# Robotmurlock/Deepwalk-and-Node2vec

Measured on AMD Instinct MI355X. Metric: positive-pairs/s + random-walks/s, 1M-node d=128 k=5, 1/2/4/8 MI355X, higher is better.
Workload: dtype fp32

## Files before the change

deepwalk-and-node2vec_amd/csrc/dw_abi.cpp:

```cpp
#include <stdarg.h>
#include <string.h>

#include "dw_common.h"

namespace dw {

static thread_local char g_err[512] = "";
static thread_local const dw_step_scalars *g_step = nullptr;
static thread_local bool g_step_has_host = false;
static thread_local int64_t g_step_host = 0;

const dw_step_scalars *bound_step_scalars() { return g_step; }

int bound_step_rel(int64_t step, const dw_step_scalars **dyn, int32_t *delta, const char *what) {
    *dyn = g_step;
    *delta = 0;
    if (!g_step) return DW_OK;
    if (!g_step_has_host) {
        set_error("%s: a dw_step_scalars block is bound without its host step "
                  "(dw_step_scalars_bind_at)", what);
        return DW_E_INVALID_ARG;
    }
    const int64_t d = step - g_step_host;
    if (d < -0x7FFFFFFF || d > 0x7FFFFFFF) {
        set_error("%s: step %lld is too far from the bound block's host step %lld", what,
                  (long long)step, (long long)g_step_host);
        return DW_E_INVALID_ARG;
    }
    *delta = static_cast<int32_t>(d);
    return DW_OK;
}

void set_error(const char *fmt, ...) {
    va_list ap;
    va_start(ap, fmt);
    vsnprintf(g_err, sizeof(g_err), fmt, ap);
    va_end(ap);
}

}

extern "C" {

const char *dw_last_error_string(void) { return dw::g_err; }

int dw_abi_version(void) { return 29; }

#ifndef DW_BUILD_ID
#define DW_BUILD_ID "unknown"
#endif
const char *dw_build_id(void) { return DW_BUILD_ID; }

int dw_step_scalars_bind(const dw_step_scalars *dev) {
    dw::g_step = dev;
    dw::g_step_has_host = false;
    return DW_OK;
}

int dw_step_scalars_bind_at(const dw_step_scalars *dev, int64_t host_step) {
    dw::g_step = dev;
    dw::g_step_has_host = dev != nullptr;
    dw::g_step_host = host_step;
    return DW_OK;
}

int dw_device_sync(void *stream) {
    hipError_t e = hipStreamSynchronize(dw::as_stream(stream));
    if (e != hipSuccess) {
        dw::set_error("hipStreamSynchronize: %s", hipGetErrorString(e));
        return DW_E_HIP;
    }
    return DW_OK;
}

}
```

deepwalk-and-node2vec_amd/csrc/dw_sgns.hip:

```cpp
#include <stdlib.h>

#include <cmath>
#include <mutex>
#include <unordered_map>
#include <vector>

#include <rocprim/block/block_radix_sort.hpp>
#include <rocprim/block/block_scan.hpp>
#include <rocprim/device/device_radix_sort.hpp>
#include <rocprim/device/device_scan.hpp>
#include <rocprim/device/device_select.hpp>

#include "dw_common.h"

namespace {

constexpr int WAVE = 64;
constexpr int WAVES_PER_BLOCK = 4;
constexpr int CHUNK = 12;
constexpr int TMAX = 256;
constexpr int GCH = 512;
constexpr int GU = 8;
constexpr uint32_t TAG_SGNS = 0x53470000u;

__device__ __forceinline__ float sigmoidf(float x) { return 1.0f / (1.0f + expf(-x)); }

using dw::row_coef;

__device__ void flush_loss(double *acc, float p, float n, float r, float pr) {
    __shared__ float s_loss[WAVES_PER_BLOCK][4];
    p = dw::wave_sum(p);
    n = dw::wave_sum(n);
    r = dw::wave_sum(r);
    pr = dw::wave_sum(pr);
    const int lane = threadIdx.x & (WAVE - 1), wv = threadIdx.x / WAVE;
    if (lane == 0) {
        s_loss[wv][0] = p;
        s_loss[wv][1] = n;
        s_loss[wv][2] = r;
        s_loss[wv][3] = pr;
    }
    __syncthreads();
    if (threadIdx.x < 4) {
        double t = 0.0;
        for (int w = 0; w < WAVES_PER_BLOCK; ++w) t += s_loss[w][threadIdx.x];
        if (t != 0.0) atomicAdd(acc + threadIdx.x, t);
    }
}

__device__ __forceinline__ float pooled(const int64_t *__restrict__ inputs, int64_t b, int32_t P,
                                        const float *__restrict__ w_in, int32_t d, int e) {
    if (P == 1) return w_in[inputs[b] * d + e];
    float h = 0.f;
    for (int p = 0; p < P; ++p) h += w_in[inputs[b * P + p] * d + e];
    return h / static_cast<float>(P);
}

__device__ __forceinline__ bool inputs_ok(const int64_t *__restrict__ inputs, int64_t b,
                                          int32_t P, int64_t V) {
    bool ok = true;
    for (int p = 0; p < P; ++p) {
        const int64_t c = inputs[b * P + p];
        ok = ok && c >= 0 && c < V;
    }
    return ok;
}

struct SgnsArgs {
    const int32_t *walks;
    int32_t L, R;
    const int64_t *inputs;
    int32_t n_in;
    const int64_t *targets;
    int64_t batch;
    int32_t C;
    int32_t K;
    int64_t V;
    int32_t d;
    const float *w_in, *w_out;
    float *g_in, *g_out;
    const int64_t *noise;
    uint32_t k0, k1;
    uint64_t noise_offset;
    float scale;
    double *loss_acc;
    int32_t *status;
    uint32_t *rec_key;
    uint64_t *rec_val;
    int32_t owner, n_owners;
    int32_t own_shift;
    uint32_t *rec_counts;
    uint32_t *count_out;
    int64_t region;
    const uint32_t *place_rank = nullptr, *place_off = nullptr;
    const uint32_t *occ;
    int64_t occ_per_wave;
    const dw_step_scalars *dyn;
    dw::Fixed fx_in{};
};

#ifndef DW_NOISE_ROUNDS
#define DW_NOISE_ROUNDS 10
#endif
__device__ __forceinline__ dw::U4 noise_pair(const SgnsArgs &a, int64_t b, int m) {
    const uint64_t g = (a.dyn ? a.dyn->noise_offset : a.noise_offset) + static_cast<uint64_t>(b);
    return dw::philox<DW_NOISE_ROUNDS>(
        dw::U4{static_cast<uint32_t>(g), static_cast<uint32_t>(g >> 32), static_cast<uint32_t>(m),
               TAG_SGNS},
        a.k0, a.k1);
}

__device__ __forceinline__ int64_t noise_id(const SgnsArgs &a, int64_t b, int j, int k) {
    if (a.noise) return a.noise[(b * a.C + j) * a.K + k];
    const int n = j * a.K + k;
    const dw::U4 r = noise_pair(a, b, n >> 1);
    const uint64_t V = static_cast<uint64_t>(a.V);
    return static_cast<int64_t>((n & 1) ? dw::bounded64(r.z, r.w, V) : dw::bounded64(r.x, r.y, V));
}

__device__ __forceinline__ uint64_t pack_record(float coef, int64_t centre) {
    return (static_cast<uint64_t>(__float_as_uint(coef)) << 32) |
           static_cast<uint32_t>(centre);
}

template <bool FROM_WALKS>
__device__ __forceinline__ int64_t row_id(const SgnsArgs &a, int64_t b, const int32_t *walk,
                                          int64_t i, int t) {
    const int rows_per_ctx = 1 + a.K;
    const int j = t / rows_per_ctx, k = t - j * rows_per_ctx - 1;
    if (k < 0) {
        if (FROM_WALKS) return walk[(j < a.R) ? (i - a.R + j) : (i + 1 + (j - a.R))];
        return a.targets[b * a.C + j];
    }
    return noise_id(a, b, j, k);
}

template <int VPL, bool MASKED, bool FROM_WALKS, bool RECORDS, int CH, bool EXACT = false>
__global__ void __launch_bounds__(WAVES_PER_BLOCK *WAVE) k_sgns(SgnsArgs a) {
    static_assert(!EXACT || RECORDS, "the exact form writes records");
    bool range = false;
    const int lane = threadIdx.x & (WAVE - 1);
    const int wv = threadIdx.x / WAVE;
    const int64_t n_waves = (int64_t)gridDim.x * WAVES_PER_BLOCK;
    const int rows_per_ctx = 1 + a.K;
    const int n_rows = a.C * rows_per_ctx;

    bool live[VPL];
#pragma unroll
    for (int m = 0; m < VPL; ++m) live[m] = !MASKED || (lane + WAVE * m < a.d);

    float acc_pos = 0.f, acc_neg = 0.f, acc_rec = 0.f, acc_prec = 0.f;

    for (int64_t b = (int64_t)blockIdx.x * WAVES_PER_BLOCK + wv; b < a.batch; b += n_waves) {
        const int32_t *walk = nullptr;
        int64_t i = 0, cid;
        if (FROM_WALKS) {
            const int64_t per = a.L - 2 * a.R;
            const int64_t w = b / per;
            i = a.R + (b - w * per);
            walk = a.walks + w * a.L;
            cid = walk[i];
        } else {
            cid = a.inputs[b * a.n_in];
        }
        const bool pool = !FROM_WALKS && a.n_in > 1;
        const bool centre_ok =
            pool ? inputs_ok(a.inputs, b, a.n_in, a.V) : (cid >= 0 && cid < a.V);
        if (!centre_ok) {
            if (lane == 0) dw::status_or(a.status, DW_S_BAD_INDEX);
            if (RECORDS) {
                for (int t = lane; t < n_rows; t += WAVE) {
                    a.rec_key[b * n_rows + t] = 0u;
                    a.rec_val[b * n_rows + t] = 0ull;
                }
            }
            continue;
        }
        float c[VPL], gc[VPL];
        int64_t gx[VPL];
        const float *crow = a.w_in + cid * a.d + lane;
#pragma unroll
        for (int m = 0; m < VPL; ++m) {
            c[m] = !live[m] ? 0.f
                   : pool   ? pooled(a.inputs, b, a.n_in, a.w_in, a.d, lane + WAVE * m)
                            : crow[WAVE * m];
            gc[m] = 0.f;
            gx[m] = 0;
        }
        for (int g0 = 0; g0 < n_rows; g0 += WAVE) {
            const int g_rows = (n_rows - g0 < WAVE) ? n_rows - g0 : WAVE;
            const int t = g0 + lane;
            int32_t my_id = 0;
            bool my_ok = false;
            const bool my_pos = (t % rows_per_ctx) == 0;
            if (lane < g_rows) {
                const int64_t id = row_id<FROM_WALKS>(a, b, walk, i, t);
                my_ok = id >= 0 && id < a.V;
                if (!my_ok) dw::status_or(a.status, DW_S_BAD_INDEX);
                my_id = my_ok ? static_cast<int32_t>(id) : 0;
            }
            float my_coef = 0.f;
            for (int r0 = 0; r0 < g_rows; r0 += CH) {
                int32_t id[CH];
                float o[CH][VPL], dot[CH];
#pragma unroll
                for (int u = 0; u < CH; ++u) {
                    const int src = (r0 + u < g_rows) ? r0 + u : 0;
                    id[u] = __builtin_amdgcn_readlane(my_id, src);
                }
#pragma unroll
                for (int u = 0; u < CH; ++u) {
                    const bool in = r0 + u < g_rows;
                    const float *row = a.w_out + static_cast<int64_t>(id[u]) * a.d + lane;
#pragma unroll
                    for (int m = 0; m < VPL; ++m) o[u][m] = (in && live[m]) ? row[WAVE * m] : 0.f;
                }
#pragma unroll
                for (int u = 0; u < CH; ++u) {
                    float s = 0.f;
#pragma unroll
                    for (int m = 0; m < VPL; ++m) s += c[m] * o[u][m];
                    dot[u] = s;
                }
#pragma unroll
                for (int off = 32; off >= 1; off >>= 1) {
#pragma unroll
                    for (int u = 0; u < CH; ++u) dot[u] += __shfl_xor(dot[u], off, WAVE);
                }
                float x = 0.f;
#pragma unroll
                for (int u = 0; u < CH; ++u)
                    if (lane == r0 + u) x = dot[u];
                const bool mine = lane >= r0 && lane < r0 + CH && lane < g_rows && my_ok;
                float coef = 0.f;
                if (mine) {
                    coef = row_coef(x, my_pos, a.scale, acc_pos, acc_neg, acc_rec, acc_prec);
                    my_coef = coef;
                }
#pragma unroll
                for (int u = 0; u < CH; ++u) {
                    if (r0 + u >= g_rows) continue;
                    const float gs =
                        __int_as_float(__builtin_amdgcn_readlane(__float_as_int(coef), r0 + u));
#pragma unroll
                    for (int m = 0; m < VPL; ++m) {
                        if constexpr (EXACT)
                            gx[m] += dw::to_fixed(gs * o[u][m], a.fx_in.fs, range);
                        else
                            gc[m] += gs * o[u][m];
                    }
                    if (!RECORDS && gs != 0.f) {
                        float *grow = a.g_out + static_cast<int64_t>(id[u]) * a.d + lane;
#pragma unroll
                        for (int m = 0; m < VPL; ++m)
                            if (live[m]) atomicAdd(grow + WAVE * m, gs * c[m]);
                    }
                }
            }
            if (RECORDS && lane < g_rows) {
                a.rec_key[b * n_rows + t] = static_cast<uint32_t>(my_id);
                a.rec_val[b * n_rows + t] = pack_record(my_ok ? my_coef : 0.f, cid);
            }
        }
        if (pool) {
            for (int p = 0; p < a.n_in; ++p) {
                float *grow = a.g_in + a.inputs[b * a.n_in + p] * a.d + lane;
#pragma unroll
                for (int m = 0; m < VPL; ++m)
                    if (live[m]) atomicAdd(grow + WAVE * m, gc[m] / static_cast<float>(a.n_in));
            }
        } else if constexpr (EXACT) {
            int64_t *gxrow = a.fx_in.acc + cid * a.d + lane;
#pragma unroll
            for (int m = 0; m < VPL; ++m)
                if (live[m]) dw::fixed_add(gxrow + WAVE * m, gx[m]);
        } else {
            float *gcrow = a.g_in + cid * a.d + lane;
#pragma unroll
            for (int m = 0; m < VPL; ++m)
                if (live[m]) atomicAdd(gcrow + WAVE * m, gc[m]);
        }
    }
    if constexpr (EXACT)
        if (__ballot(range) && lane == 0) dw::status_or(a.status, DW_S_FIXED_RANGE);

    if (a.loss_acc) flush_loss(a.loss_acc, acc_pos, acc_neg, acc_rec, acc_prec);
}

constexpr int G16_TMAX = 64;
#ifndef G16_MIN_WAVES
#define G16_MIN_WAVES 4
#endif

template <int N>
__device__ __forceinline__ float row_ror(float x) {
    return __int_as_float(
        __builtin_amdgcn_update_dpp(0, __float_as_int(x), 0x120 + N, 0xF, 0xF, false));
}

__device__ __forceinline__ float row_sum16(float x) {
    x += row_ror<8>(x);
    x += row_ror<4>(x);
    x += row_ror<2>(x);
    x += row_ror<1>(x);
    return x;
}

template <int F4, bool FROM_WALKS, int CHR, bool OWNER, bool EXACT = false, bool COEFIN = false>
__global__ void __launch_bounds__(WAVES_PER_BLOCK *WAVE, CHR >= 8 ? 3 : G16_MIN_WAVES)
    k_sgns_g16(SgnsArgs a) {
    static_assert(!COEFIN || OWNER, "the coefficients-in form is the owner path's");
    constexpr int D = 64 * F4;
    __shared__ int32_t s_id[WAVES_PER_BLOCK][4][G16_TMAX];
    __shared__ float s_coef[WAVES_PER_BLOCK][4][G16_TMAX];
    __shared__ uint8_t s_t[WAVES_PER_BLOCK][4][OWNER ? G16_TMAX : 1];
    __shared__ float4 s_g[WAVES_PER_BLOCK][4][EXACT ? 1 : 16 * F4];
    __shared__ int64_t s_gx[WAVES_PER_BLOCK][EXACT ? D : 1];
    bool range = false;
    uint32_t tmax = 0u;
    const int lane = threadIdx.x & (WAVE - 1);
    const int wv = threadIdx.x / WAVE;
    const int q = lane >> 4, gl = lane & 15;
    const int rows_per_ctx = 1 + a.K;
    const int T = a.C * rows_per_ctx;
    const int64_t n_slots = (int64_t)gridDim.x * WAVES_PER_BLOCK * 4;
    float acc_pos = 0.f, acc_neg = 0.f, acc_rec = 0.f, acc_prec = 0.f;
    int64_t filled = 0;
    const int64_t gw = (int64_t)blockIdx.x * WAVES_PER_BLOCK + wv;
    int64_t o_end = a.batch, step = n_slots, base0 = gw * 4;
    if constexpr (OWNER) {
        base0 = gw * a.occ_per_wave;
        o_end = base0 + a.occ_per_wave < a.batch ? base0 + a.occ_per_wave : a.batch;
        step = 4;
    }
    int32_t pend_c = -1;
    float pend[F4];
#pragma unroll
    for (int f = 0; f < F4; ++f) pend[f] = 0.f;

    for (int64_t base = base0; base < o_end; base += step) {
        const int64_t jb = base + q;
        const int64_t b0 =
            OWNER ? (jb < o_end ? (a.occ ? static_cast<int64_t>(a.occ[jb]) : jb) : 0) : jb;
        const bool bad_b = OWNER && jb < o_end && (b0 < 0 || b0 >= a.batch);
        if (bad_b && gl == 0) dw::status_or(a.status, DW_S_BAD_INDEX);
        const bool active = jb < o_end && !bad_b;
        const int64_t b = bad_b ? 0 : b0;
        const int32_t *walk = nullptr;
        int64_t i = 0, cid = -1;
        if (active) {
            if (FROM_WALKS) {
                const int64_t per = a.L - 2 * a.R;
                const int64_t w = b / per;
                i = a.R + (b - w * per);
                walk = a.walks + w * a.L;
                cid = walk[i];
            } else {
                cid = a.inputs[b];
            }
        }
        const bool ok_c = active && cid >= 0 && cid < a.V;
        if (active && !ok_c && gl == 0) dw::status_or(a.status, DW_S_BAD_INDEX);
        int n_own = T;
        if constexpr (OWNER) {
            int32_t *stage = reinterpret_cast<int32_t *>(&s_coef[wv][q][0]);
            for (int t = gl; t < T; t += 16) stage[t] = -1;
            if (ok_c) {
                const int n_neg = a.C * a.K;
                auto put = [&](int n, int64_t r) {
                    const int jn = n / a.K;
                    const int t = jn * rows_per_ctx + 1 + (n - jn * a.K);
                    if (r >= 0 && r < a.V)
                        stage[t] = static_cast<int32_t>(r);
                    else
                        dw::status_or(a.status, DW_S_BAD_INDEX);
                };
                for (int j = gl; j < a.C; j += 16) {
                    const int64_t r = row_id<FROM_WALKS>(a, b, walk, i, j * rows_per_ctx);
                    if (r >= 0 && r < a.V)
                        stage[j * rows_per_ctx] = static_cast<int32_t>(r);
                    else
                        dw::status_or(a.status, DW_S_BAD_INDEX);
                }
                if (a.noise) {
                    for (int n = gl; n < n_neg; n += 16) put(n, a.noise[b * n_neg + n]);
                } else {
                    const uint64_t Vu = static_cast<uint64_t>(a.V);
#pragma unroll 2
                    for (int m = gl; 2 * m < n_neg; m += 16) {
                        const dw::U4 r = noise_pair(a, b, m);
                        put(2 * m, static_cast<int64_t>(dw::bounded64(r.x, r.y, Vu)));
                        if (2 * m + 1 < n_neg)
                            put(2 * m + 1, static_cast<int64_t>(dw::bounded64(r.z, r.w, Vu)));
                    }
                }
            }
            dw::wave_lds_sync();
            n_own = 0;
#pragma unroll
            for (int k = 0; k < G16_TMAX / 16; ++k) {
                const int t = gl + 16 * k;
                const int32_t id = t < T ? stage[t] : -1;
                const int32_t lrow = a.own_shift >= 0 ? (id >> a.own_shift) : id / a.n_owners;
                const int32_t orow = id - lrow * a.n_owners;
                const bool own = (id >= 0 && orow == a.owner) ||
                                 (a.n_owners == 1 && active && t < T);
                const uint32_t grp =
                    static_cast<uint32_t>(__ballot(own) >> (16 * q)) & 0xFFFFu;
                if (own) {
                    const int pos = n_own + __popc(grp & ((1u << gl) - 1u));
                    s_id[wv][q][pos] = lrow;
                    s_t[wv][q][pos] = static_cast<uint8_t>(t);
                }
                n_own += __popc(grp);
            }
        } else {
#pragma unroll 2
            for (int k = 0; k < G16_TMAX / 16; ++k) {
                const int t = gl + 16 * k;
                int32_t id = -1;
                if (t < T && ok_c) {
                    const int64_t r = row_id<FROM_WALKS>(a, b, walk, i, t);
                    if (r >= 0 && r < a.V)
                        id = static_cast<int32_t>(r);
                    else
                        dw::status_or(a.status, DW_S_BAD_INDEX);
                }
                if (t < T) {
                    s_id[wv][q][t] = id;
                    s_coef[wv][q][t] = 0.f;
                }
            }
        }
        int n_loop = T;
        if constexpr (OWNER) {
            const int c0 = __builtin_amdgcn_readlane(n_own, 0);
            const int c1 = __builtin_amdgcn_readlane(n_own, 16);
            const int c2 = __builtin_amdgcn_readlane(n_own, 32);
            const int c3 = __builtin_amdgcn_readlane(n_own, 48);
            n_loop = max(max(c0, c1), max(c2, c3));
        }
        float4 c4[F4], g4[F4];
        int64_t gx[EXACT ? 4 * F4 : 1];
        const float *crow = a.w_in + (ok_c ? cid : 0) * D + 4 * gl;
#pragma unroll
        for (int f = 0; f < F4; ++f) {
            c4[f] = ok_c ? *reinterpret_cast<const float4 *>(crow + 64 * f)
                         : make_float4(0.f, 0.f, 0.f, 0.f);
            g4[f] = make_float4(0.f, 0.f, 0.f, 0.f);
        }
#pragma unroll
        for (int k = 0; k < (EXACT ? 4 * F4 : 1); ++k) gx[k] = 0;
        dw::wave_lds_sync();
        auto load_chunk = [&](float4(&o4)[CHR][F4], int32_t(&rid)[CHR], int t0) {
#pragma unroll
            for (int u = 0; u < CHR; ++u) {
                const int t = t0 + u;
                rid[u] = (t < n_own) ? s_id[wv][q][t] : -1;
                const int64_t at = rid[u] < 0 ? 0 : static_cast<int64_t>(rid[u]);
                const float *row = a.w_out + at * D + 4 * gl;
#pragma unroll
                for (int f = 0; f < F4; ++f)
                    o4[u][f] = rid[u] >= 0 ? *reinterpret_cast<const float4 *>(row + 64 * f)
                                           : make_float4(0.f, 0.f, 0.f, 0.f);
            }
        };
        auto compute_chunk = [&](const float4(&o4)[CHR][F4], const int32_t(&rid)[CHR],
                                 int t0) {
            float dot[CHR];
            if constexpr (!COEFIN) {
#pragma unroll
                for (int u = 0; u < CHR; ++u) {
                    float p = 0.f;
#pragma unroll
                    for (int f = 0; f < F4; ++f) {
                        p = fmaf(c4[f].x, o4[u][f].x, p);
                        p = fmaf(c4[f].y, o4[u][f].y, p);
                        p = fmaf(c4[f].z, o4[u][f].z, p);
                        p = fmaf(c4[f].w, o4[u][f].w, p);
                    }
                    dot[u] = row_sum16(p);
                }
            }
            float x = 0.f;
            int32_t xid = -1;
#pragma unroll
            for (int u = 0; u < CHR; ++u)
                if (gl == u) {
                    if constexpr (!COEFIN) x = dot[u];
                    xid = rid[u];
                }
            float coef = 0.f;
            const int t = t0 + gl;
            if (gl < CHR && t < n_own && xid >= 0) {
                const int slot = OWNER ? static_cast<int>(s_t[wv][q][t]) : t;
                if constexpr (COEFIN) {
                    coef = reinterpret_cast<const float *>(a.rec_val)[b * T + slot];
                } else {
                    coef = row_coef(x, (slot % rows_per_ctx) == 0, a.scale, acc_pos, acc_neg,
                                    acc_rec, acc_prec);
                    s_coef[wv][q][t] = coef;
                }
            }
#pragma unroll
            for (int u = 0; u < CHR; ++u) {
                const float cu = __shfl(coef, (q << 4) | u, WAVE);
                if constexpr (EXACT) {
                    const double fs = a.fx_in.fs;
#pragma unroll
                    for (int f = 0; f < F4; ++f) {
                        const float t0 = cu * o4[u][f].x, t1 = cu * o4[u][f].y;
                        const float t2 = cu * o4[u][f].z, t3 = cu * o4[u][f].w;
                        gx[4 * f + 0] += dw::fixed_bits(t0, fs);
                        gx[4 * f + 1] += dw::fixed_bits(t1, fs);
                        gx[4 * f + 2] += dw::fixed_bits(t2, fs);
                        gx[4 * f + 3] += dw::fixed_bits(t3, fs);
                        tmax = dw::fixed_track(dw::fixed_track(tmax, t0), t1);
                        tmax = dw::fixed_track(dw::fixed_track(tmax, t2), t3);
                    }
                    continue;
                }
#pragma unroll
                for (int f = 0; f < F4; ++f) {
                    g4[f].x = fmaf(cu, o4[u][f].x, g4[f].x);
                    g4[f].y = fmaf(cu, o4[u][f].y, g4[f].y);
                    g4[f].z = fmaf(cu, o4[u][f].z, g4[f].z);
                    g4[f].w = fmaf(cu, o4[u][f].w, g4[f].w);
                }
            }
        };
        for (int t0 = 0; t0 < n_loop; t0 += CHR) {
            float4 o4[CHR][F4];
            int32_t rid[CHR];
            load_chunk(o4, rid, t0);
            compute_chunk(o4, rid, t0);
        }
        if constexpr (EXACT) {
            const int64_t nt = static_cast<int64_t>((n_loop + CHR - 1) / CHR) * CHR;
#pragma unroll
            for (int k = 0; k < 4 * F4; ++k) gx[k] = dw::fixed_finish(gx[k], nt);
        }
        if constexpr (!EXACT) {
#pragma unroll
            for (int f = 0; f < F4; ++f) s_g[wv][q][gl + 16 * f] = g4[f];
        }
        dw::wave_lds_sync();
        if constexpr (COEFIN) {
        } else if constexpr (OWNER) {
            const int c0 = __builtin_amdgcn_readlane(n_own, 0);
            const int c1 = __builtin_amdgcn_readlane(n_own, 16);
            const int c2 = __builtin_amdgcn_readlane(n_own, 32);
            const int c3 = __builtin_amdgcn_readlane(n_own, 48);
            const int64_t at = ((int64_t)blockIdx.x * WAVES_PER_BLOCK + wv) * a.region + filled +
                               (q == 0 ? 0 : q == 1 ? c0 : q == 2 ? c0 + c1 : c0 + c1 + c2);
#pragma unroll
            for (int k = 0; k < G16_TMAX / 16; ++k) {
                const int tt = gl + 16 * k;
                if (tt < n_own) {
                    const int32_t id = s_id[wv][q][tt];
                    if (a.place_off) {
                        if (id >= 0) {
                            const uint32_t pos = a.place_off[id] +
                                                 a.place_rank[b * T + s_t[wv][q][tt]];
                            a.rec_key[pos] = static_cast<uint32_t>(id);
                            a.rec_val[pos] = pack_record(s_coef[wv][q][tt], ok_c ? cid : 0);
                        }
                    } else {
                        a.rec_key[at + tt] = static_cast<uint32_t>(id < 0 ? 0 : id);
                        a.rec_val[at + tt] = pack_record(id < 0 ? 0.f : s_coef[wv][q][tt],
                                                         ok_c ? cid : 0);
                    }
                }
            }
            filled += c0 + c1 + c2 + c3;
        } else if (active) {
#pragma unroll
            for (int k = 0; k < G16_TMAX / 16; ++k) {
                const int tt = gl + 16 * k;
                if (tt < T) {
                    const int32_t id = s_id[wv][q][tt];
                    a.rec_key[b * T + tt] = static_cast<uint32_t>(id < 0 ? 0 : id);
                    a.rec_val[b * T + tt] = pack_record(s_coef[wv][q][tt], ok_c ? cid : 0);
                }
            }
        }
        if constexpr (EXACT) {
            const int32_t cq_self = (ok_c && n_own > 0) ? static_cast<int32_t>(cid) : -1;
#pragma unroll
            for (int qq = 0; qq < 4; ++qq) {
                const int32_t cq = __builtin_amdgcn_readlane(cq_self, qq * 16);
                if (cq < 0) continue;
                if (q == qq) {
#pragma unroll
                    for (int f = 0; f < F4; ++f)
#pragma unroll
                        for (int k = 0; k < 4; ++k) s_gx[wv][64 * f + 4 * gl + k] = gx[4 * f + k];
                }
                dw::wave_lds_sync();
                int64_t *dst = a.fx_in.acc + static_cast<int64_t>(cq) * D + lane;
#pragma unroll
                for (int f = 0; f < F4; ++f) dw::fixed_add(dst + 64 * f, s_gx[wv][lane + 64 * f]);
                dw::wave_lds_sync();
            }
            dw::wave_lds_sync();
            continue;
        }
        const float *sg_flat = reinterpret_cast<const float *>(&s_g[wv][0][0]);
#pragma unroll
        for (int qq = 0; qq < 4; ++qq) {
            const int32_t cq = __builtin_amdgcn_readlane(
                ok_c && n_own > 0 ? static_cast<int32_t>(cid) : -1, qq * 16);
            if constexpr (OWNER) {
                if (cq < 0) continue;
                if (cq != pend_c) {
                    if (pend_c >= 0) {
                        float *dst = a.g_in + static_cast<int64_t>(pend_c) * D + lane;
#pragma unroll
                        for (int f = 0; f < F4; ++f) atomicAdd(dst + 64 * f, pend[f]);
                    }
                    pend_c = cq;
#pragma unroll
                    for (int f = 0; f < F4; ++f) pend[f] = 0.f;
                }
#pragma unroll
                for (int f = 0; f < F4; ++f)
                    pend[f] += sg_flat[qq * 16 * F4 * 4 + ((lane >> 2) + 16 * f) * 4 + (lane & 3)];
                continue;
            }
            if (cq >= 0) {
                float *dst = a.g_in + static_cast<int64_t>(cq) * D;
#pragma unroll
                for (int e0 = 0; e0 < D; e0 += WAVE) {
                    const int e = e0 + lane;
                    const int f = e >> 6, g = (e & 63) >> 2, comp = e & 3;
                    atomicAdd(dst + e, sg_flat[qq * 16 * F4 * 4 + (g + 16 * f) * 4 + comp]);
                }
            }
        }
        dw::wave_lds_sync();
    }
    if constexpr (EXACT) {
        range = range || dw::fixed_range(tmax, a.fx_in.fs);
        if (__ballot(range) && lane == 0) dw::status_or(a.status, DW_S_FIXED_RANGE);
    }
    if constexpr (OWNER) {
        if (!EXACT && pend_c >= 0) {
            float *dst = a.g_in + static_cast<int64_t>(pend_c) * D + lane;
#pragma unroll
            for (int f = 0; f < F4; ++f) atomicAdd(dst + 64 * f, pend[f]);
        }
        if (!COEFIN && lane == 0) a.rec_counts[gw] = static_cast<uint32_t>(filled);
        if (!COEFIN && a.count_out && blockIdx.x == 0 && threadIdx.x == 0)
            *a.count_out = static_cast<uint32_t>(a.batch * T);
    }
    if (a.loss_acc) flush_loss(a.loss_acc, acc_pos, acc_neg, acc_rec, acc_prec);
}

struct OutAdam {
    float *p, *m, *v;
    uint8_t *flags;
    dw::AdamScalars s;
    int32_t *last = nullptr;
    const float *hist = nullptr;
    int32_t step = 0;
    const dw_step_scalars *dyn = nullptr;
    int32_t step_delta = 0;
    bool p_current = false;
    bool betas_const = false;
    uint32_t *counts = nullptr;
    uint8_t *pend = nullptr;
};

template <int VPL, bool MASKED>
__device__ __forceinline__ void lazy_row_step(const OutAdam &oa, int32_t step, uint32_t row,
                                              int32_t d, int lane, const float (&g)[VPL]) {
    const int32_t from = __builtin_amdgcn_readfirstlane(oa.last[row]);
    const bool pd = oa.pend && __builtin_amdgcn_readfirstlane(oa.pend[row]) != 0;
    const int64_t o = static_cast<int64_t>(row) * d + lane;
    float pp[VPL], mm[VPL], vv[VPL], gg[VPL];
#pragma unroll
    for (int m = 0; m < VPL; ++m) {
        const bool live = !MASKED || lane + WAVE * m < d;
        const int64_t i = o + WAVE * m;
        pp[m] = live ? oa.p[i] : 0.f;
        mm[m] = live ? oa.m[i] : 0.f;
        vv[m] = live ? oa.v[i] : 0.f;
        gg[m] = g[m];
    }
    if (oa.p_current) {
        if (oa.betas_const) {
            const float *h = oa.hist + 8 * static_cast<int64_t>(step);
            const float w1 = h[0], b2 = h[1];
            for (int32_t t = from + 1; t < step; ++t) {
#pragma unroll
                for (int m = 0; m < VPL; ++m) {
#pragma clang fp contract(off)
                    mm[m] = fmaf(w1, -mm[m], mm[m]);
                    vv[m] = vv[m] * b2;
                }
            }
        } else {
            for (int32_t t = from + 1; t < step; ++t) {
                const float *h = oa.hist + 8 * static_cast<int64_t>(t);
                const float w1 = h[0], b2 = h[1];
#pragma unroll
                for (int m = 0; m < VPL; ++m) {
#pragma clang fp contract(off)
                    mm[m] = fmaf(w1, -mm[m], mm[m]);
                    vv[m] = vv[m] * b2;
                }
            }
        }
    } else {
        const int32_t box_from = dw::hist_box_from(oa.hist);
        if (pd) dw::settle_pending(pp, mm, vv, oa.hist, from, box_from);
        dw::replay_g0(pp, mm, vv, oa.hist, from, step - 1, box_from);
    }
    const dw::AdamScalars h = dw::hist_at(oa.hist, step);
#pragma unroll
    for (int m = 0; m < VPL; ++m) {
        if (MASKED && lane + WAVE * m >= d) continue;
        if (oa.pend)
            dw::adam_mv(pp[m], gg[m], mm[m], vv[m], h);
        else
            dw::adam_elem(pp[m], gg[m], mm[m], vv[m], h);
        const int64_t i = o + WAVE * m;
        oa.p[i] = pp[m];
        oa.m[i] = mm[m];
        oa.v[i] = vv[m];
    }
    if (lane == 0) {
        oa.last[row] = step;
        if (oa.counts) oa.counts[row] = 0u;
        if (oa.pend && !pd) oa.pend[row] = 1;
    }
}

template <int VPL, bool MASKED, bool ADAM, bool EXACT = false>
__global__ void __launch_bounds__(WAVES_PER_BLOCK *WAVE)
    k_rec_gather(const uint32_t *__restrict__ keys, const uint64_t *__restrict__ vals,
                 int64_t n_rec, const float *__restrict__ w_in, float *__restrict__ g_out,
                 int32_t d, OutAdam oa, const int64_t *__restrict__ range, int32_t gch,
                 dw::Fixed fo, int32_t *status) {
    bool fx_range = false;
    uint32_t fx_tmax = 0u;
    const int lane = threadIdx.x & (WAVE - 1);
    const int wv = __builtin_amdgcn_readfirstlane(threadIdx.x / WAVE);
    const int64_t lo = range ? range[0] : 0;
    const int64_t hi = range ? range[1] : n_rec;
    const int64_t n_chunks = (hi - lo + gch - 1) / gch;
    const dw::AdamScalars sc = ADAM ? dw::step_adam(oa.dyn, oa.s) : oa.s;
    const int32_t lstep = dw::eff_step(oa.dyn, oa.step_delta, oa.step);
    const int64_t n_waves = (int64_t)gridDim.x * WAVES_PER_BLOCK;
    bool live[VPL];
#pragma unroll
    for (int m = 0; m < VPL; ++m) live[m] = !MASKED || (lane + WAVE * m < d);

    for (int64_t ch = (int64_t)blockIdx.x * WAVES_PER_BLOCK + wv; ch < n_chunks; ch += n_waves) {
        const int64_t e0 = lo + ch * gch;
        const int64_t e1 = (e0 + gch < hi) ? e0 + gch : hi;
        const uint32_t before = e0 > lo ? keys[e0 - 1] : 0xFFFFFFFFu;
        const uint32_t after = e1 < hi ? keys[e1] : 0xFFFFFFFFu;
        const uint32_t last = keys[e1 - 1];
        uint32_t cur = keys[e0];
        float g[VPL];
        int64_t gx[VPL];
#pragma unroll
        for (int m = 0; m < VPL; ++m) {
            g[m] = 0.f;
            gx[m] = 0;
        }

        int64_t nt = 0;
        auto flush = [&](uint32_t row) {
            float *dst = g_out + static_cast<int64_t>(row) * d + lane;
            if constexpr (EXACT) {
#pragma unroll
                for (int m = 0; m < VPL; ++m) gx[m] = dw::fixed_finish(gx[m], nt);
                if (row == before || row == after) {
                    int64_t *acc = fo.acc + static_cast<int64_t>(row) * d + lane;
#pragma unroll
                    for (int m = 0; m < VPL; ++m)
                        if (live[m]) dw::fixed_add(acc + WAVE * m, gx[m]);
                    return;
                }
#pragma unroll
                for (int m = 0; m < VPL; ++m) g[m] = dw::from_fixed(gx[m], fo.fi);
            }
            if (row != before && row != after) {
                if (ADAM && oa.last) {
                    lazy_row_step<VPL, MASKED>(oa, lstep, row, d, lane, g);
                } else if (ADAM) {
                    const int64_t o = static_cast<int64_t>(row) * d + lane;
#pragma unroll
                    for (int m = 0; m < VPL; ++m) {
                        if (!live[m]) continue;
                        const int64_t i = o + WAVE * m;
                        float pp = oa.p[i], gg = g[m], mm = oa.m[i], vv = oa.v[i];
                        dw::adam_elem(pp, gg, mm, vv, sc);
                        oa.p[i] = pp;
                        oa.m[i] = mm;
                        oa.v[i] = vv;
                    }
                    if (lane == 0) oa.flags[row] = 1;
                } else {
#pragma unroll
                    for (int m = 0; m < VPL; ++m)
                        if (live[m]) dst[WAVE * m] += g[m];
                }
            } else {
#pragma unroll
                for (int m = 0; m < VPL; ++m)
                    if (live[m]) atomicAdd(dst + WAVE * m, g[m]);
            }
        };

        for (int64_t e = e0; e < e1; e += GU) {
            uint32_t k[GU];
            float coef[GU];
            float x[GU][VPL];
#pragma unroll
            for (int u = 0; u < GU; ++u) {
                const bool in = e + u < e1;
                const uint64_t v = in ? vals[e + u] : 0ull;
                k[u] = in ? keys[e + u] : last;
                coef[u] = in ? __uint_as_float(static_cast<uint32_t>(v >> 32)) : 0.f;
                const float *src = w_in + static_cast<int64_t>(static_cast<uint32_t>(v)) * d + lane;
#pragma unroll
                for (int m = 0; m < VPL; ++m) x[u][m] = (in && live[m]) ? src[WAVE * m] : 0.f;
            }
#pragma unroll
            for (int u = 0; u < GU; ++u) {
                if (k[u] != cur) {
                    flush(cur);
                    cur = k[u];
                    nt = 0;
#pragma unroll
                    for (int m = 0; m < VPL; ++m) {
                        g[m] = 0.f;
                        gx[m] = 0;
                    }
                }
                ++nt;
#pragma unroll
                for (int m = 0; m < VPL; ++m) {
                    if constexpr (EXACT) {
                        const float t = coef[u] * x[u][m];
                        gx[m] += dw::fixed_bits(t, fo.fs);
                        fx_tmax = dw::fixed_track(fx_tmax, t);
                    } else {
                        g[m] += coef[u] * x[u][m];
                    }
                }
            }
        }
        flush(cur);
    }
    if constexpr (EXACT) {
        fx_range = fx_range || dw::fixed_range(fx_tmax, fo.fs);
        if (__ballot(fx_range) && lane == 0) dw::status_or(status, DW_S_FIXED_RANGE);
    }
}

__global__ void __launch_bounds__(WAVES_PER_BLOCK *WAVE)
    k_fixed_boundary(const uint32_t *__restrict__ keys, int64_t n_rec, int32_t gch,
                     const int64_t *__restrict__ range, dw::Fixed fo, float *__restrict__ g_out,
                     int32_t d) {
    const int lane = threadIdx.x & (WAVE - 1);
    const int64_t lo = range ? range[0] : 0;
    const int64_t hi = range ? range[1] : n_rec;
    const int64_t n_chunks = (hi - lo + gch - 1) / gch;
    const int64_t n_waves = (int64_t)gridDim.x * WAVES_PER_BLOCK;
    for (int64_t ch = (int64_t)blockIdx.x * WAVES_PER_BLOCK + threadIdx.x / WAVE; ch < n_chunks;
         ch += n_waves) {
        const int64_t e0 = lo + ch * gch;
        const int64_t e1 = (e0 + gch < hi) ? e0 + gch : hi;
        const uint32_t first = keys[e0], last = keys[e1 - 1];
        const bool a = e0 > lo && keys[e0 - 1] == first;
        const bool b = e1 < hi && keys[e1] == last;
        for (int k = 0; k < 2; ++k) {
            if (!(k == 0 ? a : b)) continue;
            const int64_t o = static_cast<int64_t>(k == 0 ? first : last) * d;
            for (int e = lane; e < d; e += WAVE) {
                const unsigned long long v =
                    atomicExch(reinterpret_cast<unsigned long long *>(fo.acc + o + e), 0ull);
                if (v) atomicAdd(g_out + o + e, dw::from_fixed(static_cast<int64_t>(v), fo.fi));
            }
        }
    }
}

template <bool FROM_WALKS>
__global__ void __launch_bounds__(WAVES_PER_BLOCK *WAVE) k_fixed_centres(SgnsArgs a) {
    const int lane = threadIdx.x & (WAVE - 1);
    const int64_t n_waves = (int64_t)gridDim.x * WAVES_PER_BLOCK;
    for (int64_t b = (int64_t)blockIdx.x * WAVES_PER_BLOCK + threadIdx.x / WAVE; b < a.batch;
         b += n_waves) {
        int64_t cid;
        if (FROM_WALKS) {
            const int64_t per = a.L - 2 * a.R;
            const int64_t w = b / per;
            cid = a.walks[w * a.L + a.R + (b - w * per)];
        } else {
            cid = a.inputs[b];
        }
        if (cid < 0 || cid >= a.V) continue;
        const int64_t o = cid * a.d;
        for (int e = lane; e < a.d; e += WAVE) {
            const unsigned long long v =
                atomicExch(reinterpret_cast<unsigned long long *>(a.fx_in.acc + o + e), 0ull);
            if (v) atomicAdd(a.g_in + o + e, dw::from_fixed(static_cast<int64_t>(v), a.fx_in.fi));
        }
    }
}

__global__ void k_fixed_dense(int64_t *__restrict__ acc, float *__restrict__ g, int64_t n,
                              double fi, int32_t accumulate) {
    const int64_t stride = (int64_t)gridDim.x * blockDim.x;
    for (int64_t i = blockIdx.x * (int64_t)blockDim.x + threadIdx.x; i < n; i += stride) {
        const int64_t v = acc[i];
        if (v) acc[i] = 0;
        const float f = dw::from_fixed(v, fi);
        if (accumulate) {
            if (v) g[i] += f;
        } else {
            g[i] = f;
        }
    }
}

int end_bit_for(int64_t V) {
    int bits = 1;
    while (bits < 32 && (static_cast<uint64_t>(V - 1) >> bits) != 0) ++bits;
    return bits;
}

constexpr int MAX_PIECES = 1024;
constexpr int MAX_OWNER_WAVES = 1 << 16;

struct Workspace {
    uint32_t *k0, *k1;
    uint64_t *v0, *v1;
    int64_t *bounds;
    uint32_t *count;
    uint32_t *wave_counts;
    int64_t *wave_offsets;
    void *cub;
    size_t cub_bytes;
    size_t total;
};

inline size_t align256(size_t x) { return (x + 255) & ~size_t(255); }

using RecordSortConfig = rocprim::radix_sort_config<
    rocprim::default_config, rocprim::default_config,
    rocprim::radix_sort_onesweep_config<rocprim::kernel_config<1024, 16>,
                                        rocprim::kernel_config<1024, 16>, 11,
                                        rocprim::block_radix_rank_algorithm::match>,
    0>;
using SmallSortConfig = rocprim::radix_sort_config<
    rocprim::default_config, rocprim::default_config,
    rocprim::radix_sort_onesweep_config<rocprim::kernel_config<256, 8>,
                                        rocprim::kernel_config<256, 8>, 8,
                                        rocprim::block_radix_rank_algorithm::match>,
    128 * 1024>;
constexpr uint32_t SMALL_SORT_MAX = 4u << 20;
using Small11SortConfig = rocprim::radix_sort_config<
    rocprim::default_config, rocprim::default_config,
    rocprim::radix_sort_onesweep_config<rocprim::kernel_config<1024, 4>,
                                        rocprim::kernel_config<1024, 4>, 11,
                                        rocprim::block_radix_rank_algorithm::match>,
    0>;

template <class K, class Vt>
hipError_t sort_pairs(void *tmp, size_t &bytes, rocprim::double_buffer<K> &kb,
                      rocprim::double_buffer<Vt> &vb, uint32_t n, int end_bit, hipStream_t st) {
    if (tmp == nullptr) {
        size_t a = 0, b = 0, c = 0;
        hipError_t e = rocprim::radix_sort_pairs<RecordSortConfig>(nullptr, a, kb, vb, n, 0,
                                                                   end_bit, st);
// ... 23 lines not shown
        dw::set_error("dw_sgns: sort size query failed: %s", hipGetErrorString(e));
        return DW_E_HIP;
    }
    const size_t kbytes = align256((size_t)n_rec * 4), vbytes = align256((size_t)n_rec * 8);
    char *p = static_cast<char *>(base);
    ws->k0 = reinterpret_cast<uint32_t *>(p);
    ws->k1 = reinterpret_cast<uint32_t *>(p + kbytes);
    ws->v0 = reinterpret_cast<uint64_t *>(p + 2 * kbytes);
    ws->v1 = reinterpret_cast<uint64_t *>(p + 2 * kbytes + vbytes);
    const size_t wbytes = align256(sizeof(uint32_t) * MAX_OWNER_WAVES) +
                          align256(sizeof(int64_t) * MAX_OWNER_WAVES);
    const size_t bbytes = align256(sizeof(int64_t) * (MAX_PIECES + 1)) + 256 + wbytes;
    char *q = p + 2 * kbytes + 2 * vbytes;
    ws->bounds = reinterpret_cast<int64_t *>(q);
    q += align256(sizeof(int64_t) * (MAX_PIECES + 1));
    ws->count = reinterpret_cast<uint32_t *>(q);
    q += 256;
    ws->wave_counts = reinterpret_cast<uint32_t *>(q);
    q += align256(sizeof(uint32_t) * MAX_OWNER_WAVES);
    ws->wave_offsets = reinterpret_cast<int64_t *>(q);
    ws->cub = p + 2 * kbytes + 2 * vbytes + bbytes;
    ws->cub_bytes = cub_bytes;
    ws->total = 2 * kbytes + 2 * vbytes + bbytes + align256(cub_bytes);
    return DW_OK;
}

int64_t grid_cap(int per_cu) {
    static int n_cu[64] = {0};
    int dev = 0;
    if (hipGetDevice(&dev) != hipSuccess || dev < 0 || dev >= 64) return 65536;
    if (n_cu[dev] == 0) {
        int v = 0;
        if (hipDeviceGetAttribute(&v, hipDeviceAttributeMultiprocessorCount, dev) != hipSuccess ||
            v <= 0)
            v = 256;
        n_cu[dev] = v;
    }
    return (int64_t)n_cu[dev] * per_cu;
}

struct ExactEntry {
    int64_t *acc;
    int64_t n;
    int32_t frac, flags;
};
std::mutex g_exact_mu;
std::unordered_map<const float *, ExactEntry> g_exact;

int exact_of(const float *g, int64_t need, dw::Fixed *fx, int32_t *flags, const char *who) {
    *fx = dw::Fixed{};
    if (flags) *flags = 0;
    if (!g) return DW_OK;
    std::lock_guard<std::mutex> lk(g_exact_mu);
    const auto it = g_exact.find(g);
    if (it == g_exact.end()) return DW_OK;
    DW_REQUIRE(it->second.n >= need, "%s: the registered accumulator holds %lld elements, the "
               "launch needs %lld", who, (long long)it->second.n, (long long)need);
    *fx = dw::Fixed{it->second.acc, ldexp(1.0, it->second.frac), ldexp(1.0, -it->second.frac)};
    if (flags) *flags = it->second.flags;
    return DW_OK;
}

}

int dw::exact_lookup(const float *g, dw::Fixed *fx, int64_t *n, int32_t *flags) {
    *fx = dw::Fixed{};
    *n = 0;
    *flags = 0;
    if (!g) return 0;
    std::lock_guard<std::mutex> lk(g_exact_mu);
    const auto it = g_exact.find(g);
    if (it == g_exact.end()) return 0;
    *fx = dw::Fixed{it->second.acc, ldexp(1.0, it->second.frac), ldexp(1.0, -it->second.frac)};
    *n = it->second.n;
    *flags = it->second.flags;
    return 1;
}

namespace {

template <bool FROM_WALKS, bool RECORDS>
int launch_pass1(const SgnsArgs &a, hipStream_t st) {
    int64_t blocks = (a.batch + WAVES_PER_BLOCK - 1) / WAVES_PER_BLOCK;
    if (blocks > grid_cap(8)) blocks = grid_cap(8);
    if (blocks < 1) blocks = 1;
    const dim3 g((unsigned)blocks), bl(WAVES_PER_BLOCK * WAVE);
    const bool exact = a.fx_in.acc != nullptr;
    DW_REQUIRE(!exact || RECORDS, "dw_sgns: the deterministic mode needs the records (sorted) "
               "output-table path");
    DW_REQUIRE(!exact || FROM_WALKS || a.n_in == 1,
               "dw_sgns: the deterministic mode does not cover pooled (CBOW) inputs");
#define DW_SGNS_CASE(VPL)                                                                    \
    if (a.d <= 64 * VPL) {                                                                    \
        const bool full = a.d == 64 * VPL;                                                    \
        if (exact && RECORDS && full)                                                         \
            hipLaunchKernelGGL((k_sgns<VPL, false, FROM_WALKS, RECORDS, CHUNK, RECORDS>), g,  \
                               bl, 0, st, a);                                                 \
        else if (exact && RECORDS)                                                            \
            hipLaunchKernelGGL((k_sgns<VPL, true, FROM_WALKS, RECORDS, CHUNK, RECORDS>), g,   \
                               bl, 0, st, a);                                                 \
        else if (full)                                                                        \
            hipLaunchKernelGGL((k_sgns<VPL, false, FROM_WALKS, RECORDS, CHUNK>), g, bl, 0, st, \
                               a);                                                            \
        else                                                                                  \
            hipLaunchKernelGGL((k_sgns<VPL, true, FROM_WALKS, RECORDS, CHUNK>), g, bl, 0, st, \
                               a);                                                            \
        DW_LAUNCH_CHECK("dw_sgns");                                                           \
        return DW_OK;                                                                         \
    }
    DW_SGNS_CASE(1)
    DW_SGNS_CASE(2)
    DW_SGNS_CASE(4)
    DW_SGNS_CASE(8)
#undef DW_SGNS_CASE
    dw::set_error("dw_sgns: dim %d > 512 is not supported", a.d);
    return DW_E_UNSUPPORTED;
}

template <bool FROM_WALKS, bool OWNER = false, bool COEFIN = false>
int launch_pass1_g16(const SgnsArgs &a, hipStream_t st) {
    const int64_t T = (int64_t)a.C * (1 + a.K);
    if (a.d % 64 != 0 || a.d > 512 || T > G16_TMAX) return DW_E_UNSUPPORTED;
    int64_t blocks = (a.batch + 4 * WAVES_PER_BLOCK - 1) / (4 * WAVES_PER_BLOCK);
    if (blocks > grid_cap(8)) blocks = grid_cap(8);
    if (blocks < 1) blocks = 1;
    const dim3 g((unsigned)blocks), bl(WAVES_PER_BLOCK * WAVE);
    if constexpr (COEFIN) {
        switch ((a.d / 64) * 2 + (a.fx_in.acc ? 1 : 0)) {
            case 2: hipLaunchKernelGGL((k_sgns_g16<1, FROM_WALKS, 8, true, false, true>), g, bl, 0, st, a); break;
            case 3: hipLaunchKernelGGL((k_sgns_g16<1, FROM_WALKS, 8, true, true, true>), g, bl, 0, st, a); break;
            case 4: hipLaunchKernelGGL((k_sgns_g16<2, FROM_WALKS, 4, true, false, true>), g, bl, 0, st, a); break;
            case 5: hipLaunchKernelGGL((k_sgns_g16<2, FROM_WALKS, 4, true, true, true>), g, bl, 0, st, a); break;
            case 8: hipLaunchKernelGGL((k_sgns_g16<4, FROM_WALKS, 2, true, false, true>), g, bl, 0, st, a); break;
            case 9: hipLaunchKernelGGL((k_sgns_g16<4, FROM_WALKS, 2, true, true, true>), g, bl, 0, st, a); break;
            case 16: hipLaunchKernelGGL((k_sgns_g16<8, FROM_WALKS, 1, true, false, true>), g, bl, 0, st, a); break;
            case 17: hipLaunchKernelGGL((k_sgns_g16<8, FROM_WALKS, 1, true, true, true>), g, bl, 0, st, a); break;
            default:
                dw::set_error("dw_sgns: the coefficient-input pass 1 needs d in {64, 128, 256, 512}, got %d", a.d);
                return DW_E_UNSUPPORTED;
        }
        DW_LAUNCH_CHECK("dw_sgns/g16_coefin");
        return DW_OK;
    }
    if (a.fx_in.acc) {
        switch (a.d / 64) {
            case 1: hipLaunchKernelGGL((k_sgns_g16<1, FROM_WALKS, 8, OWNER, true>), g, bl, 0, st, a); break;
            case 2: hipLaunchKernelGGL((k_sgns_g16<2, FROM_WALKS, 4, OWNER, true>), g, bl, 0, st, a); break;
            case 4: hipLaunchKernelGGL((k_sgns_g16<4, FROM_WALKS, 2, OWNER, true>), g, bl, 0, st, a); break;
            case 8: hipLaunchKernelGGL((k_sgns_g16<8, FROM_WALKS, 1, OWNER, true>), g, bl, 0, st, a); break;
            default: return DW_E_UNSUPPORTED;
        }
        DW_LAUNCH_CHECK("dw_sgns/g16");
        return DW_OK;
    }
    switch (a.d / 64) {
        case 1: hipLaunchKernelGGL((k_sgns_g16<1, FROM_WALKS, 8, OWNER>), g, bl, 0, st, a); break;
        case 2: hipLaunchKernelGGL((k_sgns_g16<2, FROM_WALKS, 4, OWNER>), g, bl, 0, st, a); break;
        case 4: hipLaunchKernelGGL((k_sgns_g16<4, FROM_WALKS, 2, OWNER>), g, bl, 0, st, a); break;
        case 8: hipLaunchKernelGGL((k_sgns_g16<8, FROM_WALKS, 1, OWNER>), g, bl, 0, st, a); break;
        default: return DW_E_UNSUPPORTED;
    }
    DW_LAUNCH_CHECK("dw_sgns/g16");
    return DW_OK;
}

template <int VPL, bool MASKED>
__global__ void __launch_bounds__(256)
    k_adam_rest(int64_t n_rows, int32_t d, uint8_t *__restrict__ flags,
                float *__restrict__ g, OutAdam oa) {
    const int lane = threadIdx.x & (WAVE - 1);
    const int64_t n_waves = (int64_t)gridDim.x * (blockDim.x / WAVE);
    const dw::AdamScalars sc = dw::step_adam(oa.dyn, oa.s);
    for (int64_t base = (blockIdx.x * (int64_t)(blockDim.x / WAVE) + threadIdx.x / WAVE) * WAVE;
         base < n_rows; base += n_waves * WAVE) {
        const int64_t r = base + lane;
        const bool in = r < n_rows;
        const uint8_t f = in ? flags[r] : 1;
        if (in && f != 0) flags[r] = 0;
        unsigned long long todo = __ballot(in && f == 0);
        while (todo) {
            const int l0 = __ffsll(static_cast<long long>(todo)) - 1;
            todo &= todo - 1ull;
            const bool two = todo != 0ull;
            const int l1 = two ? __ffsll(static_cast<long long>(todo)) - 1 : l0;
            if (two) todo &= todo - 1ull;
            const int64_t o0 = (base + l0) * d + lane, o1 = (base + l1) * d + lane;
            float pp[2][VPL], gg[2][VPL], mm[2][VPL], vv[2][VPL];
#pragma unroll
            for (int m = 0; m < VPL; ++m) {
                if (MASKED && lane + WAVE * m >= d) continue;
                const int64_t i0 = o0 + WAVE * m, i1 = o1 + WAVE * m;
                pp[0][m] = oa.p[i0]; gg[0][m] = g[i0]; mm[0][m] = oa.m[i0]; vv[0][m] = oa.v[i0];
                pp[1][m] = oa.p[i1]; gg[1][m] = g[i1]; mm[1][m] = oa.m[i1]; vv[1][m] = oa.v[i1];
            }
#pragma unroll
            for (int k = 0; k < 2; ++k) {
                if (k == 1 && !two) break;
                const int64_t o = k ? o1 : o0;
#pragma unroll
                for (int m = 0; m < VPL; ++m) {
                    if (MASKED && lane + WAVE * m >= d) continue;
                    const int64_t i = o + WAVE * m;
                    dw::adam_elem(pp[k][m], gg[k][m], mm[k][m], vv[k][m], sc);
                    oa.p[i] = pp[k][m];
                    oa.m[i] = mm[k][m];
                    oa.v[i] = vv[k][m];
                    if (__float_as_uint(gg[k][m]) != 0u) g[i] = 0.f;
                }
            }
        }
    }
}

template <int VPL, bool MASKED>
__global__ void __launch_bounds__(WAVES_PER_BLOCK *WAVE)
    k_lazy_boundary(const uint32_t *__restrict__ keys, int64_t n_rec, int32_t gch,
                    float *__restrict__ g_out, int32_t d, OutAdam oa,
                    const int64_t *__restrict__ range) {
    const int lane = threadIdx.x & (WAVE - 1);
    if (range) n_rec = range[1];
    const int64_t n_chunks = (n_rec + gch - 1) / gch;
    const int64_t n_waves = (int64_t)gridDim.x * WAVES_PER_BLOCK;
    for (int64_t ch = (int64_t)blockIdx.x * WAVES_PER_BLOCK + threadIdx.x / WAVE; ch < n_chunks;
         ch += n_waves) {
        const int64_t e0 = ch * gch;
        const int64_t e1 = (e0 + gch < n_rec) ? e0 + gch : n_rec;
        const uint32_t row = keys[e1 - 1];
        if (e1 >= n_rec || keys[e1] != row) continue;
        if (keys[e0] == row && e0 > 0 && keys[e0 - 1] == row) continue;
        float g[VPL];
        const int64_t o = static_cast<int64_t>(row) * d + lane;
#pragma unroll
        for (int m = 0; m < VPL; ++m) {
            g[m] = 0.f;
            if (MASKED && lane + WAVE * m >= d) continue;
            g[m] = g_out[o + WAVE * m];
            g_out[o + WAVE * m] = 0.f;
        }
        lazy_row_step<VPL, MASKED>(oa, dw::eff_step(oa.dyn, oa.step_delta, oa.step), row, d,
                                   lane, g);
    }
}

template <int VPL>
void launch_boundary(hipStream_t st, const uint32_t *keys, int64_t n_rec, int32_t gch,
                     float *g_out, int32_t d, const OutAdam &oa, const int64_t *range) {
    int64_t blocks = ((n_rec + gch - 1) / gch + WAVES_PER_BLOCK - 1) / WAVES_PER_BLOCK;
    if (blocks < 1) blocks = 1;
    if (blocks > 65536) blocks = 65536;
    if (d == 64 * VPL)
        hipLaunchKernelGGL((k_lazy_boundary<VPL, false>), dim3((unsigned)blocks),
                           dim3(WAVES_PER_BLOCK * WAVE), 0, st, keys, n_rec, gch, g_out, d, oa,
                           range);
    else
        hipLaunchKernelGGL((k_lazy_boundary<VPL, true>), dim3((unsigned)blocks),
                           dim3(WAVES_PER_BLOCK * WAVE), 0, st, keys, n_rec, gch, g_out, d, oa,
                           range);
}

constexpr int OUT_ROWS_WAVES = 7;
template <int F4, bool EXACT = false>
__global__ void __launch_bounds__(WAVES_PER_BLOCK *WAVE, F4 <= 2 ? OUT_ROWS_WAVES : 2)
    k_out_rows(SgnsArgs a, const uint32_t *__restrict__ keys, const uint64_t *__restrict__ vals,
               const int64_t *__restrict__ range, int32_t gch, OutAdam oa,
               float *__restrict__ coef_slot, dw::Fixed fo, const uint32_t *__restrict__ off) {
    constexpr int D = 64 * F4;
    constexpr int BR = WAVES_PER_BLOCK * WAVE;
    bool fx_range = false;
    uint32_t fx_tmax = 0u;
    constexpr int RU = 4;
    __shared__ uint32_t s_key[BR], s_slot[BR];
    __shared__ int32_t s_cid[BR];
    __shared__ uint16_t s_rs[BR + 1];
    __shared__ int32_t s_wrows[WAVES_PER_BLOCK];
    __shared__ int32_t s_next;
    __shared__ float4 s_p[WAVES_PER_BLOCK][D / 4];
    __shared__ float4 s_c[WAVES_PER_BLOCK][RU][D / 4];
    __shared__ uint32_t s_ovs[WAVES_PER_BLOCK][WAVE];
    __shared__ int32_t s_ovc[WAVES_PER_BLOCK][WAVE];
    const int lane = threadIdx.x & (WAVE - 1);
    const int wv = __builtin_amdgcn_readfirstlane(threadIdx.x / WAVE);
    const int q = lane >> 4, gl = lane & 15;
    const uint64_t lt = (1ull << lane) - 1ull;
    const int64_t n_rec = range[1];
    const int32_t br_len = WAVES_PER_BLOCK * gch;
    const int64_t n_ranges = (n_rec + br_len - 1) / br_len;
    const int32_t step = dw::eff_step(oa.dyn, oa.step_delta, oa.step);
    const dw::AdamScalars hs = dw::hist_at(oa.hist, step);
    const int32_t box_from = dw::hist_box_from(oa.hist);
    const int T = a.C * (1 + a.K), rpc = 1 + a.K;
    const int64_t per = a.L - 2 * a.R;
    float *sp = reinterpret_cast<float *>(&s_p[wv][0]);
    float acc_pos = 0.f, acc_neg = 0.f, acc_rec = 0.f, acc_prec = 0.f;

    for (int64_t br = blockIdx.x; br < n_ranges; br += gridDim.x) {
        const int64_t r0 = br * br_len;
        const int n_blk = static_cast<int>(n_rec - r0 < br_len ? n_rec - r0 : br_len);
        const uint32_t after = r0 + n_blk < n_rec ? keys[r0 + n_blk] : 0xFFFFFFFFu;
        {
            const int i = WAVE * wv + lane;
            const bool in = i < n_blk;
            const uint32_t key = in ? keys[r0 + i] : 0xFFFFFFFFu;
            const uint32_t prev = lane > 0 ? 0u
                                  : i == 0 ? (r0 > 0 ? keys[r0 - 1] : 0xFFFFFFFFu)
                                           : (in ? keys[r0 + i - 1] : 0u);
            const uint64_t rec = in ? vals[r0 + i] : 0xFFFFFFFF00000000ull;
// ... 27 lines not shown
        float np[F4], nm[F4], nv[F4];
        int32_t nlast = 0;
        uint32_t npend = 0;
        auto prefetch = [&](int k) {
            const uint32_t r = s_key[s_rs[k]];
            const int64_t o = static_cast<int64_t>(r) * D + lane;
            nlast = oa.last[r];
            npend = oa.pend[r];
#pragma unroll
            for (int f = 0; f < F4; ++f) {
                np[f] = oa.p[o + 64 * f];
                nm[f] = oa.m[o + 64 * f];
                nv[f] = oa.v[o + 64 * f];
            }
        };
        int k = take();
        if (k < nrows) prefetch(k);
        while (k < nrows) {
            const int rs = s_rs[k], re = s_rs[k + 1];
            const uint32_t row = s_key[rs];
            const int64_t ro = static_cast<int64_t>(row) * D + lane;
            const bool glob = re == n_blk && after == row;
            const int cnt = glob ? static_cast<int>(off[row + 1] - static_cast<uint32_t>(r0 + rs))
                                 : re - rs;
            auto window = [&](int j) {
                const uint64_t rec = j + lane < cnt ? vals[r0 + rs + j + lane]
                                                    : 0xFFFFFFFF00000000ull;
                s_ovs[wv][lane] = static_cast<uint32_t>(rec);
                s_ovc[wv][lane] = static_cast<int32_t>(rec >> 32);
                dw::wave_lds_sync();
            };
            if (glob) window(0);
            const uint32_t *Ls = glob ? &s_ovs[wv][0] : &s_slot[rs];
            const int32_t *Lc = glob ? &s_ovc[wv][0] : &s_cid[rs];
            const int msk = glob ? WAVE - 1 : 0x7FFFFFFF;
            float p[F4], m[F4], v[F4], g[F4];
            int64_t gx[EXACT ? F4 : 1];
#pragma unroll
            for (int f = 0; f < F4; ++f) {
                p[f] = np[f];
                m[f] = nm[f];
                v[f] = nv[f];
                g[f] = 0.f;
            }
#pragma unroll
            for (int f = 0; f < (EXACT ? F4 : 1); ++f) gx[f] = 0;
            const int32_t from = __builtin_amdgcn_readfirstlane(nlast);
            const bool pd = __builtin_amdgcn_readfirstlane(npend) != 0;
            __builtin_amdgcn_s_waitcnt(0x0F70);
            float4 c4[F4];
            {
                const int32_t cid = q < cnt ? Lc[q] : -1;
                const bool ok = cid >= 0 && cid < a.V;
                const float *crow = a.w_in + static_cast<int64_t>(ok ? cid : 0) * D + 4 * gl;
#pragma unroll
                for (int f = 0; f < F4; ++f)
                    c4[f] = ok ? *reinterpret_cast<const float4 *>(crow + 64 * f)
                               : make_float4(0.f, 0.f, 0.f, 0.f);
            }
            const int kn = take();
            prefetch(kn < nrows ? kn : k);
            if (pd) dw::settle_pending(p, m, v, oa.hist, from, box_from);
            dw::replay_g0(p, m, v, oa.hist, from, step - 1, box_from);
#pragma unroll
            for (int f = 0; f < F4; ++f) sp[lane + 64 * f] = p[f];
            dw::wave_lds_sync();
            for (int j0 = 0; j0 < cnt; j0 += RU) {
                const bool in = j0 + q < cnt;
                if (glob && j0 > 0 && (j0 & (WAVE - 1)) == 0) window(j0);
                const int l = in ? (j0 & msk) + q : 0;
                const uint32_t spx = Ls[l];
                const uint32_t slot = spx & 0x7FFFFFFFu;
                const bool pos = (spx >> 31) != 0u;
                const int32_t cid = in ? Lc[l] : -1;
                const bool ok = in && cid >= 0 && cid < a.V;
                if (j0 > 0) {
                    const float *crow = a.w_in + static_cast<int64_t>(ok ? cid : 0) * D + 4 * gl;
#pragma unroll
                    for (int f = 0; f < F4; ++f)
                        c4[f] = ok ? *reinterpret_cast<const float4 *>(crow + 64 * f)
                                   : make_float4(0.f, 0.f, 0.f, 0.f);
                }
                float pr = 0.f;
#pragma unroll
                for (int f = 0; f < F4; ++f) {
                    const float4 of = s_p[wv][gl + 16 * f];
                    pr = fmaf(c4[f].x, of.x, pr);
                    pr = fmaf(c4[f].y, of.y, pr);
                    pr = fmaf(c4[f].z, of.z, pr);
                    pr = fmaf(c4[f].w, of.w, pr);
                    s_c[wv][q][gl + 16 * f] = c4[f];
                }
                const float x = row_sum16(pr);
                float coef = 0.f;
                if (ok && gl == 0)
                    coef = row_coef(x, pos, a.scale, acc_pos, acc_neg, acc_rec, acc_prec);
                if (in && gl == 0) coef_slot[slot] = coef;
                dw::wave_lds_sync();
#pragma unroll
                for (int u = 0; u < RU; ++u) {
                    if (j0 + u >= cnt) break;
                    const float cu = __shfl(coef, u << 4, WAVE);
                    const float *cr = reinterpret_cast<const float *>(&s_c[wv][u][0]);
                    if constexpr (EXACT) {
#pragma unroll
                        for (int f = 0; f < F4; ++f) {
                            const float t = cu * cr[lane + 64 * f];
                            gx[f] += dw::fixed_bits(t, fo.fs);
                            fx_tmax = dw::fixed_track(fx_tmax, t);
                        }
                    } else {
#pragma unroll
                        for (int f = 0; f < F4; ++f) g[f] += cu * cr[lane + 64 * f];
                    }
                }
                dw::wave_lds_sync();
            }
            if constexpr (EXACT) {
#pragma unroll
                for (int f = 0; f < F4; ++f) {
                    gx[f] = dw::fixed_finish(gx[f], cnt);
                    g[f] = dw::from_fixed(gx[f], fo.fi);
                }
            }
            {
#pragma unroll
                for (int f = 0; f < F4; ++f) {
                    dw::adam_mv(p[f], g[f], m[f], v[f], hs);
                    oa.p[ro + 64 * f] = p[f];
                    oa.m[ro + 64 * f] = m[f];
                    oa.v[ro + 64 * f] = v[f];
                }
                if (lane == 0) {
                    oa.last[row] = step;
                    if (!pd) oa.pend[row] = 1;
                    if (oa.counts) oa.counts[row] = 0u;
                }
            }
            k = kn;
        }
        __syncthreads();
    }
    if constexpr (EXACT) {
        fx_range = fx_range || dw::fixed_range(fx_tmax, fo.fs);
        if (__ballot(fx_range) && lane == 0) dw::status_or(a.status, DW_S_FIXED_RANGE);
    }
    if (a.loss_acc) flush_loss(a.loss_acc, acc_pos, acc_neg, acc_rec, acc_prec);
}

template <int VPL, bool EXACT>
void launch_gather_fx(dim3 g, dim3 bl, hipStream_t st, const uint32_t *keys,
                      const uint64_t *vals, int64_t n_rec, const float *w_in, float *g_out,
                      int32_t d, const OutAdam *oa, const int64_t *range, int32_t gch,
                      const dw::Fixed &fo, int32_t *status) {
    const bool full = d == 64 * VPL;
    if (oa) {
        if (full)
            hipLaunchKernelGGL((k_rec_gather<VPL, false, true, EXACT>), g, bl, 0, st, keys, vals,
                               n_rec, w_in, g_out, d, *oa, range, gch, fo, status);
        else
            hipLaunchKernelGGL((k_rec_gather<VPL, true, true, EXACT>), g, bl, 0, st, keys, vals,
                               n_rec, w_in, g_out, d, *oa, range, gch, fo, status);
    } else {
        if (full)
            hipLaunchKernelGGL((k_rec_gather<VPL, false, false, EXACT>), g, bl, 0, st, keys,
                               vals, n_rec, w_in, g_out, d, OutAdam{}, range, gch, fo, status);
        else
            hipLaunchKernelGGL((k_rec_gather<VPL, true, false, EXACT>), g, bl, 0, st, keys, vals,
                               n_rec, w_in, g_out, d, OutAdam{}, range, gch, fo, status);
    }
}

template <int VPL>
void launch_gather(dim3 g, dim3 bl, hipStream_t st, const uint32_t *keys, const uint64_t *vals,
                   int64_t n_rec, const float *w_in, float *g_out, int32_t d,
                   const OutAdam *oa, const int64_t *range, int32_t gch, const dw::Fixed &fo,
                   int32_t *status) {
    if (fo.acc)
        launch_gather_fx<VPL, true>(g, bl, st, keys, vals, n_rec, w_in, g_out, d, oa, range, gch,
                                    fo, status);
    else
        launch_gather_fx<VPL, false>(g, bl, st, keys, vals, n_rec, w_in, g_out, d, oa, range,
                                     gch, fo, status);
}

template <int VPL>
void launch_rest(hipStream_t st, int64_t V, int32_t d, float *g_out, const OutAdam &oa) {
    int64_t rb = (V + 255) / 256;
    if (rb > grid_cap(8)) rb = grid_cap(8);
    if (rb < 1) rb = 1;
    if (d == 64 * VPL)
        hipLaunchKernelGGL((k_adam_rest<VPL, false>), dim3((unsigned)rb), dim3(256), 0, st, V, d,
                           oa.flags, g_out, oa);
    else
        hipLaunchKernelGGL((k_adam_rest<VPL, true>), dim3((unsigned)rb), dim3(256), 0, st, V, d,
                           oa.flags, g_out, oa);
}

int launch_pass2(const uint32_t *keys, const uint64_t *vals, int64_t n_rec, const float *w_in,
                 float *g_out, int32_t d, const OutAdam *oa, int64_t V, hipStream_t st,
                 const int64_t *range = nullptr, double share = 1.0, int32_t *status = nullptr) {
    dw::Fixed fo;
    {
        const int rc = exact_of(g_out, V * d, &fo, nullptr, "dw_sgns pass 2");
        if (rc != DW_OK) return rc;
    }
    int32_t gch = GCH;
    {
        const int64_t want = grid_cap(16);
        while (gch > 32 && (n_rec + gch - 1) / gch < want) gch >>= 1;
    }
    const int64_t n_chunks = (n_rec + gch - 1) / gch;
    int64_t blocks = (int64_t)((double)(n_chunks + WAVES_PER_BLOCK - 1) / WAVES_PER_BLOCK * share);
    if (blocks < 1) blocks = 1;
    if (blocks > 65536) blocks = 65536;
    const dim3 g((unsigned)blocks), bl(WAVES_PER_BLOCK * WAVE);
    if (d <= 64) launch_gather<1>(g, bl, st, keys, vals, n_rec, w_in, g_out, d, oa, range, gch, fo, status);
    else if (d <= 128) launch_gather<2>(g, bl, st, keys, vals, n_rec, w_in, g_out, d, oa, range, gch, fo, status);
    else if (d <= 256) launch_gather<4>(g, bl, st, keys, vals, n_rec, w_in, g_out, d, oa, range, gch, fo, status);
    else if (d <= 512) launch_gather<8>(g, bl, st, keys, vals, n_rec, w_in, g_out, d, oa, range, gch, fo, status);
    else return DW_E_UNSUPPORTED;
    DW_LAUNCH_CHECK("dw_sgns/gather");
    if (fo.acc && n_rec > 0) {
        hipLaunchKernelGGL(k_fixed_boundary, g, bl, 0, st, keys, n_rec, gch, range, fo, g_out, d);
        DW_LAUNCH_CHECK("dw_sgns/fixed_boundary");
    }
    if (oa && oa->last) {
        if (n_rec > 0) {
            if (d <= 64) launch_boundary<1>(st, keys, n_rec, gch, g_out, d, *oa, range);
            else if (d <= 128) launch_boundary<2>(st, keys, n_rec, gch, g_out, d, *oa, range);
            else if (d <= 256) launch_boundary<4>(st, keys, n_rec, gch, g_out, d, *oa, range);
            else launch_boundary<8>(st, keys, n_rec, gch, g_out, d, *oa, range);
            DW_LAUNCH_CHECK("dw_sgns/lazy_boundary");
        }
    } else if (oa) {
        if (d <= 64) launch_rest<1>(st, V, d, g_out, *oa);
        else if (d <= 128) launch_rest<2>(st, V, d, g_out, *oa);
        else if (d <= 256) launch_rest<4>(st, V, d, g_out, *oa);
        else launch_rest<8>(st, V, d, g_out, *oa);
        DW_LAUNCH_CHECK("dw_sgns/adam_rest");
    }
    return DW_OK;
}

struct PhaseTimer {
    static constexpr size_t MAX_CALLS = 4096;
    bool on = false;
    size_t calls = 0;
    std::vector<hipEvent_t> ev;
    bool active() const { return on && calls < MAX_CALLS; }
    void mark(int slot, hipStream_t st) {
        if (!active()) return;
        const size_t i = 4 * calls + slot;
        while (ev.size() <= i) {
            hipEvent_t e;
            if (hipEventCreate(&e) != hipSuccess) {
                on = false;
                return;
            }
            ev.push_back(e);
        }
        (void)hipEventRecord(ev[i], st);
        if (slot == 3) ++calls;
    }
};
PhaseTimer g_timer;

template <bool FROM_WALKS>
int launch_sgns_impl(SgnsArgs a, void *workspace, size_t workspace_bytes, int phase,
                     hipStream_t st, const OutAdam *oa);

template <bool FROM_WALKS>
int launch_sgns(SgnsArgs a, void *workspace, size_t workspace_bytes, int phase, hipStream_t st,
                const OutAdam *oa = nullptr) {
    if (phase != 2) g_timer.mark(0, st);
    const int rc = launch_sgns_impl<FROM_WALKS>(a, workspace, workspace_bytes, phase, st, oa);
    if (rc != DW_OK) {
        if (g_timer.active()) g_timer.on = false;
        return rc;
    }
    if (phase != 1) g_timer.mark(3, st);
    return DW_OK;
}

template <bool FROM_WALKS>
int launch_sgns_impl(SgnsArgs a, void *workspace, size_t workspace_bytes, int phase,
                     hipStream_t st, const OutAdam *oa) {
    const bool do1 = phase != 2, do2 = phase != 1;
    if (a.batch == 0 && do2 && oa) {
        if (do1) g_timer.mark(1, st);
        g_timer.mark(2, st);
        return launch_pass2(nullptr, nullptr, 0, a.w_in, a.g_out, a.d, oa, a.V, st);
    }
    if (a.batch == 0 || workspace == nullptr) {
        if (do1 && a.batch > 0) {
            dw::Fixed f0;
            int rc0 = exact_of(a.g_in, 0, &f0, nullptr, "dw_sgns");
            if (rc0 == DW_OK) rc0 = exact_of(a.g_out, 0, &f0, nullptr, "dw_sgns");
            if (rc0 != DW_OK) return rc0;
            DW_REQUIRE(!f0.acc, "dw_sgns: the deterministic mode needs the records (sorted) "
                       "output-table path (a workspace)");
            const int rc = launch_pass1<FROM_WALKS, false>(a, st);
            if (rc != DW_OK) return rc;
        }
        if (do1) g_timer.mark(1, st);
        if (do2) g_timer.mark(2, st);
        return DW_OK;
    }
    const int64_t T = (int64_t)a.C * (1 + a.K);
    DW_REQUIRE(T <= TMAX, "dw_sgns: records mode needs 2R(1+K) <= %d (got %lld)", TMAX,
               (long long)T);
    DW_REQUIRE(a.V <= 0x7FFFFFFF, "dw_sgns: records mode needs vocab_size < 2^31");
    const int64_t n_rec = a.batch * T;
    DW_REQUIRE(n_rec < 0x7FFFFFFF, "dw_sgns: records mode needs batch*2R(1+K) < 2^31");
    Workspace ws;
    int rc = plan_workspace(n_rec, a.V, workspace, &ws, st);
    if (rc != DW_OK) return rc;
    DW_REQUIRE(workspace_bytes >= ws.total, "dw_sgns: workspace too small (%zu < %zu)",
               workspace_bytes, ws.total);
    if (do1) {
        a.rec_key = ws.k0;
        a.rec_val = ws.v0;
        int32_t fl = 0;
        rc = exact_of(a.g_in, a.V * a.d, &a.fx_in, &fl, "dw_sgns pass 1");
        if (rc != DW_OK) return rc;
        rc = launch_pass1_g16<FROM_WALKS>(a, st);
        if (rc == DW_E_UNSUPPORTED) rc = launch_pass1<FROM_WALKS, true>(a, st);
        if (rc != DW_OK) return rc;
        if (a.fx_in.acc && !(fl & (DW_EXACT_DEFER | DW_EXACT_ADAM))) {
            int64_t cb = (a.batch + WAVES_PER_BLOCK - 1) / WAVES_PER_BLOCK;
            if (cb > grid_cap(8)) cb = grid_cap(8);
            hipLaunchKernelGGL(k_fixed_centres<FROM_WALKS>, dim3((unsigned)cb),
                               dim3(WAVES_PER_BLOCK * WAVE), 0, st, a);
            DW_LAUNCH_CHECK("dw_sgns/fixed_centres");
        }
        g_timer.mark(1, st);
    }
    if (!do2) return DW_OK;
    rocprim::double_buffer<uint32_t> kb(ws.k0, ws.k1);
    rocprim::double_buffer<uint64_t> vb(ws.v0, ws.v1);
    size_t cub_bytes = ws.cub_bytes;
    hipError_t e = sort_pairs(ws.cub, cub_bytes, kb, vb, static_cast<uint32_t>(n_rec),
                              end_bit_for(a.V), st);
    if (e != hipSuccess) {
        dw::set_error("dw_sgns: records sort failed: %s", hipGetErrorString(e));
        return DW_E_HIP;
    }
    g_timer.mark(2, st);
    return launch_pass2(kb.current(), vb.current(), n_rec, a.w_in, a.g_out, a.d, oa, a.V, st,
                        nullptr, 1.0, a.status);
}

__global__ void k_piece_bounds(const uint32_t *__restrict__ keys, int64_t n_rec, int32_t n_pieces,
                               int64_t piece_rows, int64_t *__restrict__ bounds) {
    const int p = blockIdx.x * blockDim.x + threadIdx.x;
    if (p > n_pieces) return;
    if (p == n_pieces) {
        bounds[p] = n_rec;
        return;
    }
    const uint64_t target = static_cast<uint64_t>(p) * static_cast<uint64_t>(piece_rows);
    int64_t lo = 0, hi = n_rec;
    while (lo < hi) {
        const int64_t mid = (lo + hi) >> 1;
        if (static_cast<uint64_t>(keys[mid]) < target) lo = mid + 1;
        else hi = mid;
    }
    bounds[p] = lo;
}

std::mutex g_sorted_mu;
std::unordered_map<const void *, bool> g_sorted_in_k1;

int launch_pieces(SgnsArgs a, void *workspace, size_t workspace_bytes, int piece, int n_pieces,
                  int64_t piece_rows, hipStream_t st) {
    DW_REQUIRE(workspace != nullptr, "dw_sgns_walks_phase2_piece: needs the records workspace");
    DW_REQUIRE(n_pieces >= 1 && n_pieces <= MAX_PIECES && piece >= -1 && piece < n_pieces,
               "dw_sgns_walks_phase2_piece: piece %d of %d (at most %d pieces)", piece, n_pieces,
               MAX_PIECES);
    DW_REQUIRE(piece_rows >= 1 && piece_rows * (int64_t)n_pieces >= a.V,
               "dw_sgns_walks_phase2_piece: %d pieces of %lld rows do not cover %lld rows",
               n_pieces, (long long)piece_rows, (long long)a.V);
    const int64_t T = (int64_t)a.C * (1 + a.K);
    DW_REQUIRE(T <= TMAX && a.V <= 0x7FFFFFFF, "dw_sgns_walks_phase2_piece: records mode limits");
    const int64_t n_rec = a.batch * T;
    DW_REQUIRE(n_rec < 0x7FFFFFFF, "dw_sgns_walks_phase2_piece: too many records");
    Workspace ws;
    int rc = plan_workspace(n_rec > 0 ? n_rec : 1, a.V, workspace, &ws, st);
    if (rc != DW_OK) return rc;
    DW_REQUIRE(workspace_bytes >= ws.total, "dw_sgns: workspace too small (%zu < %zu)",
               workspace_bytes, ws.total);
    if (piece == -1) {
        bool in_k1 = false;
        if (n_rec > 0) {
            rocprim::double_buffer<uint32_t> kb(ws.k0, ws.k1);
            rocprim::double_buffer<uint64_t> vb(ws.v0, ws.v1);
            size_t cub_bytes = ws.cub_bytes;
            hipError_t e = sort_pairs(ws.cub, cub_bytes, kb, vb, static_cast<uint32_t>(n_rec),
                                      end_bit_for(a.V), st);
            if (e != hipSuccess) {
                dw::set_error("dw_sgns: records sort failed: %s", hipGetErrorString(e));
                return DW_E_HIP;
            }
            in_k1 = kb.current() == ws.k1;
        }
        {
            std::lock_guard<std::mutex> lk(g_sorted_mu);
            g_sorted_in_k1[workspace] = in_k1;
        }
        hipLaunchKernelGGL(k_piece_bounds, dim3((n_pieces + 256) / 256), dim3(256), 0, st,
                           in_k1 ? ws.k1 : ws.k0, n_rec, n_pieces, piece_rows, ws.bounds);
        DW_LAUNCH_CHECK("dw_sgns/piece_bounds");
        g_timer.mark(2, st);
        return DW_OK;
    }
    bool in_k1;
    {
        std::lock_guard<std::mutex> lk(g_sorted_mu);
        auto it = g_sorted_in_k1.find(workspace);
        DW_REQUIRE(it != g_sorted_in_k1.end(),
                   "dw_sgns_walks_phase2_piece: piece %d before the sort call (piece -1)", piece);
        in_k1 = it->second;
    }
    if (n_rec > 0) {
        rc = launch_pass2(in_k1 ? ws.k1 : ws.k0, in_k1 ? ws.v1 : ws.v0, n_rec, a.w_in, a.g_out,
                          a.d, nullptr, a.V, st, ws.bounds + piece, 2.0 / n_pieces);
        if (rc != DW_OK) return rc;
    }
    if (piece == n_pieces - 1) g_timer.mark(3, st);
    return DW_OK;
}

struct OwnerLayout {
    int64_t blocks, n_waves, region, total;
};

OwnerLayout owner_layout(int64_t n_centres, int64_t T) {
    OwnerLayout l;
    l.blocks = (n_centres + 4 * WAVES_PER_BLOCK - 1) / (4 * WAVES_PER_BLOCK);
    if (l.blocks > grid_cap(8)) l.blocks = grid_cap(8);
    if (l.blocks < 1) l.blocks = 1;
    l.n_waves = l.blocks * WAVES_PER_BLOCK;
    const int64_t per_sweep = l.n_waves * 4;
    const int64_t iters = (n_centres + per_sweep - 1) / per_sweep;
    l.region = iters * 4 * T;
    l.total = l.n_waves * l.region;
    return l;
}

__global__ void __launch_bounds__(1024)
    k_wave_scan(const uint32_t *__restrict__ counts, int64_t n, int64_t *__restrict__ offsets,
                uint32_t *__restrict__ count) {
    __shared__ int64_t part[1024];
    const int t = threadIdx.x;
    const int64_t per = (n + 1023) / 1024;
    const int64_t lo = t * per, hi = lo + per < n ? lo + per : n;
    int64_t sum = 0;
    for (int64_t i = lo; i < hi; ++i) sum += counts[i];
    part[t] = sum;
    __syncthreads();
    for (int off = 1; off < 1024; off <<= 1) {
        const int64_t v = t >= off ? part[t - off] : 0;
        __syncthreads();
        part[t] += v;
        __syncthreads();
    }
    int64_t run = part[t] - sum;
    for (int64_t i = lo; i < hi; ++i) {
        offsets[i] = run;
        run += counts[i];
    }
    if (t == 1023) *count = static_cast<uint32_t>(part[1023]);
}

__global__ void __launch_bounds__(256)
    k_rec_compact(const uint32_t *__restrict__ counts, const int64_t *__restrict__ offsets,
                  int64_t n_waves, int64_t region, const uint32_t *__restrict__ k_src,
                  const uint64_t *__restrict__ v_src, uint32_t *__restrict__ k_dst,
                  uint64_t *__restrict__ v_dst) {
    for (int64_t g = blockIdx.x; g < n_waves; g += gridDim.x) {
        const int64_t n = counts[g], src = g * region, dst = offsets[g];
        for (int64_t i = threadIdx.x; i < n; i += blockDim.x) {
            k_dst[dst + i] = k_src[src + i];
            v_dst[dst + i] = v_src[src + i];
        }
    }
}

__global__ void __launch_bounds__(256)
    k_rec_pad(const uint32_t *__restrict__ count, int64_t bound, uint32_t *__restrict__ keys,
              uint64_t *__restrict__ vals, int64_t *__restrict__ range) {
    const int64_t n = *count;
    if (blockIdx.x == 0 && threadIdx.x == 0) {
        range[0] = 0;
        range[1] = n < bound ? n : bound;
    }
    for (int64_t i = n + blockIdx.x * (int64_t)blockDim.x + threadIdx.x; i < bound;
         i += (int64_t)gridDim.x * blockDim.x) {
        keys[i] = 0xFFFFFFFFu;
        vals[i] = 0ull;
    }
}

__global__ void __launch_bounds__(256)
    k_occ_keys(const int32_t *__restrict__ walks, int64_t n_centres, int32_t L, int32_t R,
               uint32_t *__restrict__ keys, uint32_t *__restrict__ vals) {
    const int64_t per = L - 2 * R;
    for (int64_t b = blockIdx.x * (int64_t)blockDim.x + threadIdx.x; b < n_centres;
         b += (int64_t)gridDim.x * blockDim.x) {
        const int64_t w = b / per;
        keys[b] = static_cast<uint32_t>(walks[w * L + R + (b - w * per)]);
        vals[b] = static_cast<uint32_t>(b);
    }
}

constexpr int OCC_SMALL_THREADS = 1024, OCC_SMALL_IPT = 8;
constexpr int64_t OCC_SMALL_MAX = (int64_t)OCC_SMALL_THREADS * OCC_SMALL_IPT;

__global__ void __launch_bounds__(OCC_SMALL_THREADS)
    k_occ_small(const int32_t *__restrict__ walks, int64_t n_centres, int32_t L, int32_t R,
                int32_t end_bit, uint32_t *__restrict__ keys_out, uint32_t *__restrict__ vals_out,
                uint32_t *__restrict__ touched, int64_t *__restrict__ n_touched) {
    using Sort = rocprim::block_radix_sort<uint32_t, OCC_SMALL_THREADS, OCC_SMALL_IPT, uint32_t>;
    using Scan = rocprim::block_scan<uint32_t, OCC_SMALL_THREADS>;
    __shared__ typename Sort::storage_type s_sort;
    __shared__ typename Scan::storage_type s_scan;
    __shared__ uint32_t s_last[OCC_SMALL_THREADS];
    const int t = threadIdx.x;
    const int64_t per = L - 2 * R;
    uint32_t k[OCC_SMALL_IPT], v[OCC_SMALL_IPT];
#pragma unroll
    for (int i = 0; i < OCC_SMALL_IPT; ++i) {
        const int64_t b = (int64_t)t * OCC_SMALL_IPT + i;
        if (b < n_centres) {
            const int64_t w = b / per;
            k[i] = static_cast<uint32_t>(walks[w * L + R + (b - w * per)]);
            v[i] = static_cast<uint32_t>(b);
        } else {
            k[i] = 0xFFFFFFFFu;
            v[i] = 0xFFFFFFFFu;
        }
    }
    Sort().sort(k, v, s_sort, 0, end_bit);
#pragma unroll
    for (int i = 0; i < OCC_SMALL_IPT; ++i) {
        const int64_t b = (int64_t)t * OCC_SMALL_IPT + i;
        if (b < n_centres) {
            keys_out[b] = k[i];
            vals_out[b] = v[i];
        }
    }
    if (!touched) return;
    s_last[t] = k[OCC_SMALL_IPT - 1];
    __syncthreads();
    uint32_t prev = t > 0 ? s_last[t - 1] : 0u;
    bool f[OCC_SMALL_IPT];
    uint32_t cnt = 0;
#pragma unroll
    for (int i = 0; i < OCC_SMALL_IPT; ++i) {
        const int64_t b = (int64_t)t * OCC_SMALL_IPT + i;
        f[i] = b < n_centres && (b == 0 || k[i] != prev);
        prev = k[i];
        cnt += f[i] ? 1u : 0u;
    }
    uint32_t off = 0, total = 0;
    Scan().exclusive_scan(cnt, off, 0u, total, s_scan);
#pragma unroll
    for (int i = 0; i < OCC_SMALL_IPT; ++i)
        if (f[i]) touched[off++] = k[i];
    if (t == 0) *n_touched = static_cast<int64_t>(total);
}

struct OccSpace {
    uint32_t *k0, *k1, *v0, *v1;
    void *tmp;
    size_t tmp_bytes, total;
};

int plan_occ(int64_t n_centres, int64_t V, void *base, OccSpace *o, hipStream_t st) {
// ... 635 lines not shown
                   n_rows && hist && status,
               "dw_sgns_owner_out_catch_up: null pointer");
    DW_REQUIRE((flags & ~7) == 0, "dw_sgns_owner_out_catch_up: flags must be a set of 1 | 2 | 4");
    const bool place = (flags & 1) != 0, p_only = (flags & 2) != 0;
    const bool rows_major = (flags & 4) != 0;
    DW_REQUIRE(!place || counts, "dw_sgns_owner_out_catch_up: placing needs the row counts");
    DW_REQUIRE(!rows_major || place, "dw_sgns_owner_out_catch_up: the rows-major step places "
               "the records (flags & 1)");
    hipStream_t st = dw::as_stream(stream);
    const dw_step_scalars *dyn = nullptr;
    int32_t delta = 0;
    int rc = dw::bound_step_rel(step, &dyn, &delta, "dw_sgns_owner_out_catch_up");
    if (rc != DW_OK) return rc;
    SgnsArgs a = base_args(vocab_size, dim, neg_samples, nullptr, w_out_local, nullptr, nullptr,
                           noise, seed, noise_offset, 0.f, nullptr, status);
    a.walks = walks;
    a.L = walk_length;
    a.R = context_radius;
    a.batch = n_walks * (walk_length - 2 * context_radius);
    a.C = 2 * context_radius;
    a.owner = owner;
    a.n_owners = n_owners;
    if (!(flags & 4) && hipMemsetAsync(n_rows, 0, sizeof(int64_t), st) != hipSuccess) {
        dw::set_error("dw_sgns_owner_out_catch_up: counter reset failed");
        return DW_E_HIP;
    }
    const int64_t T = (int64_t)a.C * (1 + a.K);
    Workspace ws;
    OwnerLayout lay;
    PlaceSpace pl{};
    if (place) {
        rc = owner_workspace(a.batch, T, local_rows, workspace, workspace_bytes, &ws, &lay, st,
                             "dw_sgns_owner_out_catch_up", vocab_size, nullptr, &pl);
        if (rc != DW_OK) return rc;
    }
    const int64_t ctile = (int64_t)WAVES_PER_BLOCK * (rows_major ? 1 : CLAIM_TRIPS);
    int64_t blocks = (a.batch + ctile - 1) / ctile;
    if (blocks > grid_cap(8)) blocks = grid_cap(8);
    if (blocks < 1) blocks = 1;
    if (rows_major)
        hipLaunchKernelGGL(k_out_claim<false>, dim3((unsigned)blocks),
                           dim3(WAVES_PER_BLOCK * WAVE), 0, st, a, claim, step, delta, rows_buf,
                           reinterpret_cast<unsigned long long *>(n_rows), counts, pl.rank,
                           ws.k0);
    else
        hipLaunchKernelGGL(k_out_claim<true>, dim3((unsigned)blocks),
                           dim3(WAVES_PER_BLOCK * WAVE), 0, st, a, claim, step, delta, rows_buf,
                           reinterpret_cast<unsigned long long *>(n_rows),
                           place ? counts : nullptr, place ? pl.rank : nullptr, nullptr);
    DW_LAUNCH_CHECK("dw_sgns_owner_out_catch_up/claim");
    if (place) {
        const int64_t nb = (local_rows + PLACE_TILE - 1) / PLACE_TILE;
        DW_REQUIRE(pl.tmp_bytes >= (size_t)nb * 4, "dw_sgns_owner_out_catch_up: scan scratch");
        uint32_t *sums = static_cast<uint32_t *>(pl.tmp);
        hipLaunchKernelGGL(k_place_sums, dim3((unsigned)nb), dim3(256), 0, st, counts, local_rows,
                           sums);
        hipLaunchKernelGGL(k_place_scan, dim3((unsigned)nb), dim3(256), 0, st, counts, local_rows,
                           sums, pl.off, ws.bounds);
        DW_LAUNCH_CHECK("dw_sgns_owner_out_catch_up/place");
    }
    if (rows_major) {
        int64_t pb = (a.batch * T + 255) / 256;
        if (pb > grid_cap(8)) pb = grid_cap(8);
        if (pb < 1) pb = 1;
        hipLaunchKernelGGL(k_place_slots, dim3((unsigned)pb), dim3(256), 0, st, a.batch * T,
                           ws.k0, pl.rank, pl.off, ws.k1, ws.v1, walks, walk_length,
                           context_radius, static_cast<int32_t>(T), 1 + neg_samples);
        DW_LAUNCH_CHECK("dw_sgns_owner_out_catch_up/place_slots");
        return DW_OK;
    }
    const int64_t n_max = std::min<int64_t>(local_rows, a.batch * T);
    return dw::adam_rows_launch(w_out_local, m_out, v_out, last_step, nullptr, local_rows, dim,
                                rows_buf,
                                n_rows, n_max, nullptr, hist, step - 1, p_only, st);
}

int dw_exact_register(const float *grad, int64_t *acc, int64_t n_elems, int32_t frac,
                      int32_t flags) {
    DW_REQUIRE(grad && acc && n_elems >= 0, "dw_exact_register: bad arguments");
    DW_REQUIRE(frac >= 0 && frac <= 62, "dw_exact_register: frac %d outside [0, 62]", frac);
    DW_REQUIRE((flags & ~(DW_EXACT_DEFER | DW_EXACT_ADAM)) == 0,
               "dw_exact_register: unknown flags %d", flags);
    std::lock_guard<std::mutex> lk(g_exact_mu);
    g_exact[grad] = ExactEntry{acc, n_elems, frac, flags};
    return DW_OK;
}

int dw_exact_unregister(const float *grad) {
    std::lock_guard<std::mutex> lk(g_exact_mu);
    g_exact.erase(grad);
    return DW_OK;
}

int32_t dw_exact_frac_bits(double scale) {
    const double a = fabs(scale);
    if (!(a > 0.0) || !std::isfinite(a)) return 40;
    int f = 32 + static_cast<int>(ceil(-log2(a)));
    return f < 16 ? 16 : (f > 62 ? 62 : f);
}

int dw_fixed_to_float(int64_t *acc, float *grad, int64_t n, int32_t frac, int32_t accumulate,
                      void *stream) {
    DW_REQUIRE(n >= 0 && frac >= 0 && frac <= 62, "dw_fixed_to_float: bad arguments");
    if (n == 0) return DW_OK;
    DW_REQUIRE(acc && grad, "dw_fixed_to_float: null pointer");
    int64_t blocks = (n + 255) / 256;
    if (blocks > grid_cap(8)) blocks = grid_cap(8);
    hipLaunchKernelGGL(k_fixed_dense, dim3((unsigned)blocks), dim3(256), 0, dw::as_stream(stream),
                       acc, grad, n, ldexp(1.0, -frac), accumulate);
    DW_LAUNCH_CHECK("dw_fixed_to_float");
    return DW_OK;
}

int dw_sgns_timing(int32_t enable) {
    g_timer.on = enable != 0;
    if (enable) g_timer.calls = 0;
    return DW_OK;
}

int dw_sgns_phase_ms(double *ms, int64_t *n_calls) {
    DW_REQUIRE(ms && n_calls, "dw_sgns_phase_ms: null pointer");
    ms[0] = ms[1] = ms[2] = 0.0;
    *n_calls = static_cast<int64_t>(g_timer.calls);
    if (g_timer.calls == 0) return DW_OK;
    hipError_t e = hipEventSynchronize(g_timer.ev[4 * g_timer.calls - 1]);
    for (size_t c = 0; c < g_timer.calls && e == hipSuccess; ++c) {
        for (int k = 0; k < 3 && e == hipSuccess; ++k) {
            float t = 0.f;
            e = hipEventElapsedTime(&t, g_timer.ev[4 * c + k], g_timer.ev[4 * c + k + 1]);
            ms[k] += t;
        }
    }
    if (e != hipSuccess) {
        dw::set_error("dw_sgns_phase_ms: %s", hipGetErrorString(e));
        return DW_E_HIP;
    }
    for (int k = 0; k < 3; ++k) ms[k] /= static_cast<double>(g_timer.calls);
    return DW_OK;
}

int dw_sgns_workspace_bytes(int64_t n_centres, int32_t n_ctx, int32_t neg_samples,
                            int64_t vocab_size, size_t *bytes) {
    DW_REQUIRE(bytes, "dw_sgns_workspace_bytes: bytes is null");
    DW_REQUIRE(n_centres >= 0 && n_ctx >= 1 && neg_samples >= 0 && vocab_size >= 1,
               "dw_sgns_workspace_bytes: bad sizes");
    const int64_t n_rec = n_centres * n_ctx * (1 + (int64_t)neg_samples);
    DW_REQUIRE(n_rec < 0x7FFFFFFF, "dw_sgns_workspace_bytes: too many records");
    Workspace ws;
    char dummy;
    int rc = plan_workspace(n_rec > 0 ? n_rec : 1, vocab_size, &dummy, &ws, nullptr);
    if (rc != DW_OK) return rc;
    *bytes = ws.total;
    return DW_OK;
}

namespace {
int sgns_walks(int phase, const int32_t *walks, int64_t n_walks, int32_t walk_length,
               int32_t context_radius, int32_t neg_samples, int64_t vocab_size, int32_t dim,
               const float *w_in, const float *w_out, float *g_in, float *g_out,
               const int64_t *noise, uint64_t seed, uint64_t noise_offset, float grad_scale,
               double *loss_acc, int32_t *status, void *workspace, size_t workspace_bytes,
               void *stream) {
    DW_REQUIRE(phase >= 0 && phase <= 2, "dw_sgns_walks_phase: phase must be 0, 1 or 2");
    DW_REQUIRE(context_radius >= 1, "dw_sgns_walks: context_radius must be >= 1");
    DW_REQUIRE(walk_length >= 2 * context_radius + 1,
               "dw_sgns_walks: walk_length %d < 2R+1 (Text is too short!)", walk_length);
    DW_REQUIRE(neg_samples >= 0 && dim >= 1 && vocab_size >= 1 && n_walks >= 0,
               "dw_sgns_walks: bad sizes");
    DW_REQUIRE(walks && w_in && w_out && g_in && g_out && status, "dw_sgns_walks: null pointer");
    SgnsArgs a = base_args(vocab_size, dim, neg_samples, w_in, w_out, g_in, g_out, noise, seed,
                           noise_offset, grad_scale, loss_acc, status);
    a.walks = walks;
    a.L = walk_length;
    a.R = context_radius;
    a.batch = n_walks * (walk_length - 2 * context_radius);
    a.C = 2 * context_radius;
    return launch_sgns<true>(a, workspace, workspace_bytes, phase, dw::as_stream(stream));
}
}

int dw_sgns_walks(const int32_t *walks, int64_t n_walks, int32_t walk_length,
                  int32_t context_radius, int32_t neg_samples, int64_t vocab_size, int32_t dim,
                  const float *w_in, const float *w_out, float *g_in, float *g_out,
                  const int64_t *noise, uint64_t seed, uint64_t noise_offset, float grad_scale,
                  double *loss_acc, int32_t *status, void *workspace, size_t workspace_bytes,
                  void *stream) {
    return sgns_walks(0, walks, n_walks, walk_length, context_radius, neg_samples, vocab_size,
                      dim, w_in, w_out, g_in, g_out, noise, seed, noise_offset, grad_scale,
                      loss_acc, status, workspace, workspace_bytes, stream);
}

int dw_sgns_walks_phase2_adam(const int32_t *walks, int64_t n_walks, int32_t walk_length,
                              int32_t context_radius, int32_t neg_samples, int64_t vocab_size,
                              int32_t dim, const float *w_in, float *w_out, float *g_out,
                              float *m_out, float *v_out, uint8_t *row_flags,
                              float one_minus_beta1, float beta2, float one_minus_beta2,
                              float bias_correction2_sqrt, float neg_step_size, float eps,
                              float weight_decay, int32_t *status, void *workspace,
                              size_t workspace_bytes, void *stream) {
    DW_REQUIRE(workspace && m_out && v_out && row_flags && w_out && g_out,
               "dw_sgns_walks_phase2_adam: needs the records workspace and the Adam state");
    DW_REQUIRE(bias_correction2_sqrt > 0.f, "dw_sgns_walks_phase2_adam: bad Adam scalars");
    DW_REQUIRE(context_radius >= 1 && walk_length >= 2 * context_radius + 1 && n_walks >= 0 &&
                   dim >= 1 && vocab_size >= 1 && neg_samples >= 0,
               "dw_sgns_walks_phase2_adam: bad sizes");
    DW_REQUIRE(walks && w_in && status, "dw_sgns_walks_phase2_adam: null pointer");
    SgnsArgs a = base_args(vocab_size, dim, neg_samples, w_in, w_out, nullptr, g_out, nullptr,
                           0, 0, 1.f, nullptr, status);
    a.walks = walks;
    a.L = walk_length;
    a.R = context_radius;
    a.batch = n_walks * (walk_length - 2 * context_radius);
    a.C = 2 * context_radius;
    OutAdam oa{w_out, m_out, v_out, row_flags,
               dw::AdamScalars{one_minus_beta1, beta2, one_minus_beta2, bias_correction2_sqrt,
                               neg_step_size, eps, weight_decay,
                               bias_correction2_sqrt > 0.f ? 1.0f / bias_correction2_sqrt : 0.f}};
    oa.dyn = dw::bound_step_scalars();
    return launch_sgns<true>(a, workspace, workspace_bytes, 2, dw::as_stream(stream), &oa);
}

int dw_sgns_walks_phase2_piece(int32_t piece, int32_t n_pieces, int64_t piece_rows,
                               const int32_t *walks, int64_t n_walks, int32_t walk_length,
                               int32_t context_radius, int32_t neg_samples, int64_t vocab_size,
                               int32_t dim, const float *w_in, float *g_out, int32_t *status,
                               void *workspace, size_t workspace_bytes, void *stream) {
    DW_REQUIRE(context_radius >= 1 && walk_length >= 2 * context_radius + 1 && n_walks >= 0 &&
                   dim >= 1 && vocab_size >= 1 && neg_samples >= 0,
               "dw_sgns_walks_phase2_piece: bad sizes");
    DW_REQUIRE(walks && w_in && g_out && status, "dw_sgns_walks_phase2_piece: null pointer");
    SgnsArgs a = base_args(vocab_size, dim, neg_samples, w_in, nullptr, nullptr, g_out, nullptr,
                           0, 0, 1.f, nullptr, status);
    a.walks = walks;
    a.L = walk_length;
    a.R = context_radius;
    a.batch = n_walks * (walk_length - 2 * context_radius);
    a.C = 2 * context_radius;
    return launch_pieces(a, workspace, workspace_bytes, piece, n_pieces, piece_rows,
                         dw::as_stream(stream));
}

int dw_sgns_walks_phase(int32_t phase, const int32_t *walks, int64_t n_walks,
                        int32_t walk_length, int32_t context_radius, int32_t neg_samples,
                        int64_t vocab_size, int32_t dim, const float *w_in, const float *w_out,
                        float *g_in, float *g_out, const int64_t *noise, uint64_t seed,
                        uint64_t noise_offset, float grad_scale, double *loss_acc,
                        int32_t *status, void *workspace, size_t workspace_bytes,
                        void *stream) {
    return sgns_walks(phase, walks, n_walks, walk_length, context_radius, neg_samples,
                      vocab_size, dim, w_in, w_out, g_in, g_out, noise, seed, noise_offset,
                      grad_scale, loss_acc, status, workspace, workspace_bytes, stream);
}

int dw_sgns_owner_workspace_bytes(int64_t n_centres, int32_t n_ctx, int32_t neg_samples,
                                  int64_t vocab_size, int64_t local_rows, size_t *bytes) {
    DW_REQUIRE(bytes, "dw_sgns_owner_workspace_bytes: bytes is null");
    DW_REQUIRE(n_centres >= 0 && n_ctx >= 1 && neg_samples >= 0 && local_rows >= 1 &&
                   vocab_size >= 1,
               "dw_sgns_owner_workspace_bytes: bad sizes");
    const OwnerLayout lay = owner_layout(n_centres, (int64_t)n_ctx * (1 + neg_samples));
    DW_REQUIRE(lay.total < 0x7FFFFFFF, "dw_sgns_owner_workspace_bytes: too many records");
    Workspace ws;
    OccSpace occ;
    PlaceSpace pl;
    char dummy;
    int rc = plan_workspace(lay.total > 0 ? lay.total : 1, local_rows, &dummy, &ws, nullptr);
    if (rc != DW_OK) return rc;
    rc = plan_place(n_centres * (int64_t)n_ctx * (1 + neg_samples), local_rows, &dummy, &pl,
                    nullptr);
    if (rc != DW_OK) return rc;
    rc = plan_occ(n_centres > 0 ? n_centres : 1, vocab_size, &dummy, &occ, nullptr);
    if (rc != DW_OK) return rc;
    *bytes = ws.total + pl.total + occ.total;
    return DW_OK;
}

int dw_sgns_owner_prepare(const int32_t *walks, int64_t n_walks, int32_t walk_length,
                          int32_t context_radius, int32_t neg_samples, int64_t vocab_size,
                          int64_t local_rows, uint32_t *touched, int64_t *n_touched,
                          void *workspace, size_t workspace_bytes, void *stream) {
    DW_REQUIRE(context_radius >= 1 && walk_length >= 2 * context_radius + 1 && n_walks >= 0 &&
                   vocab_size >= 1 && local_rows >= 1 && neg_samples >= 0,
               "dw_sgns_owner_prepare: bad sizes");
    DW_REQUIRE((walks || n_walks == 0) && (!touched || n_touched),
               "dw_sgns_owner_prepare: null pointer");
    SgnsArgs a = base_args(vocab_size, 64, neg_samples, nullptr, nullptr, nullptr, nullptr,
                           nullptr, 0, 0, 1.f, nullptr, nullptr);
    a.walks = walks;
    a.L = walk_length;
    a.R = context_radius;
    a.batch = n_walks * (walk_length - 2 * context_radius);
    a.C = 2 * context_radius;
    return launch_owner_prepare(a, local_rows, touched, n_touched, workspace, workspace_bytes,
                                dw::as_stream(stream));
}

int dw_sgns_owner_touch_claim(const int32_t *walks, int64_t n_walks, int32_t walk_length,
                              int32_t context_radius, int64_t vocab_size, int32_t *claim,
                              int32_t step, uint32_t *touched, int64_t *n_touched,
                              uint32_t *fresh, int64_t *n_fresh, int32_t flags, void *stream) {
    DW_REQUIRE(context_radius >= 1 && walk_length >= 2 * context_radius + 1 && n_walks >= 0 &&
                   vocab_size >= 1 && step >= 1,
               "dw_sgns_owner_touch_claim: bad sizes");
    DW_REQUIRE(claim && touched && n_touched && (walks || n_walks == 0) && (!fresh || n_fresh),
               "dw_sgns_owner_touch_claim: null pointer");
    const hipStream_t st = dw::as_stream(stream);
// ... 348 lines not shown
```

deepwalk-and-node2vec_amd/shallow_encoders/_native.py:

```python
import ctypes
import os
import threading
from typing import Optional

import torch

LIB_PATH = os.environ.get(
    'DW_LIB_PATH', os.path.join(os.path.dirname(os.path.abspath(__file__)), '_lib', 'libdw_hip.so'))

DW_OK = 0
DW_E_INVALID_ARG = -1
DW_E_HIP = -2
DW_E_UNSUPPORTED = -3

DW_S_ISOLATED_NODE = 1
DW_S_ZERO_WEIGHT = 2
DW_S_REJECTION_CAP = 4
DW_S_BAD_CSR = 8
DW_S_BAD_INDEX = 16
DW_S_RECORDS_FULL = 32
DW_S_DUP_NEIGHBOR = 64
DW_S_FIXED_RANGE = 128
DW_S_BAD_TEXT = 256
DW_EXACT_DEFER = 1
DW_EXACT_ADAM = 2

DW_METHOD_DEEPWALK = 0
DW_METHOD_NODE2VEC = 1

ABI_VERSION = 29

_p = ctypes.c_void_p
_i32 = ctypes.c_int32
_i64 = ctypes.c_int64
_u64 = ctypes.c_uint64
_f32 = ctypes.c_float
_f64 = ctypes.c_double
_szp = ctypes.POINTER(ctypes.c_size_t)

SIGNATURES = {
    'dw_last_error_string': (ctypes.c_char_p, []),
    'dw_abi_version': (ctypes.c_int, []),
    'dw_build_id': (ctypes.c_char_p, []),
    'dw_device_sync': (ctypes.c_int, [_p]),
    'dw_stream_copy': (ctypes.c_int, [_p, _p, _i64, _p]),
    'dw_host_shuffle': (ctypes.c_int, [_p, _p, _i64]),
    'dw_mt_jump_table': (ctypes.c_int, [_i64, _i64, _p, _p, _i64]),
    'dw_mt_uniforms': (ctypes.c_int, [_p, _i32, _i64, _p, _p, _i64, _p, _p, _i64, _p, _i64,
                                      _p]),
    'dw_mt_workspace_words': (ctypes.c_int64, [_i64]),
    'dw_mt_draw': (ctypes.c_int, [_i32, _p, _i32, _i64, _p, _u64, _p, _i64, _p, _p, _i64, _p,
                                  _i64, _p]),
    'dw_csr_validate': (ctypes.c_int, [_p, _p, _i64, _i64, _p, _p]),
    'dw_csr_sort_copy': (ctypes.c_int, [_p, _p, _i64, _i64, _p, _p, _szp, _p]),
    'dw_csr_check_simple': (ctypes.c_int, [_p, _p, _i64, _i64, _p, _p]),
    'dw_adj_hash_offsets': (ctypes.c_int, [_p, _i64, _p, _p, _szp, _p]),
    'dw_adj_hash_build': (ctypes.c_int, [_p, _p, _i64, _p, _i64, _p, _p, _p]),
    'dw_alias_build': (ctypes.c_int, [_p, _p, _i64, _i64, _p, _p, _p, _p, _p, _p]),
    'dw_ingest_workspace_bytes': (ctypes.c_int, [_i32, _i64, _i64, _szp]),
    'dw_rmat_edges': (ctypes.c_int, [_i32, _i64, _p, _p, _u64, _u64, _f64, _f64, _f64, _p, _p, _p,
                                     ctypes.c_size_t, _p]),
    'dw_graph_isolated': (ctypes.c_int, [_p, _i64, _i64, _p, _p, _p, _p, ctypes.c_size_t, _p]),
    'dw_csr_from_edges': (ctypes.c_int, [_p, _i64, _i64, _p, _p, _p, _p, ctypes.c_size_t, _p]),
    'dw_edgelist_workspace_bytes': (ctypes.c_int, [_i64, _i64, _szp]),
    'dw_edgelist_parse': (ctypes.c_int, [_p, _i64, _i64, _p, _p, _i64, _p, _p, _p, _p,
                                         ctypes.c_size_t, _p]),
    'dw_edges_canonical': (ctypes.c_int, [_p, _p, _p, _i64, _i32, _p, _p, _p, _p, _p, _p,
                                          ctypes.c_size_t, _p]),
    'dw_csr_from_edges_loops': (ctypes.c_int, [_p, _p, _i64, _i64, _p, _p, _p, _p, _p,
                                               ctypes.c_size_t, _p]),
    'dw_walk_replay': (ctypes.c_int, [_p, _p, _p, _p, _i64, _p, _i64, _i32, _i32, _f64, _f64,
                                      _p, _p, _p, _p]),
    'dw_walk_fast': (ctypes.c_int, [_p, _p, _p, _p, _p, _i64, _p, _i64, _i32, _i32, _f64, _f64,
                                    _u64, _u64, _p, _p, _p]),
    'dw_walk_fast_indexed': (ctypes.c_int, [_p, _p, _p, _p, _p, _p, _p, _i64, _p, _i64, _i32,
                                            _i32, _f64, _f64, _u64, _u64, _p, _p, _p]),
    'dw_walk_fast_counted': (ctypes.c_int, [_p, _p, _p, _p, _p, _p, _i64, _p, _i64, _i32, _f64,
                                            _f64, _u64, _u64, _p, _p, _p, _p]),
    'dw_walk_fast_positions': (ctypes.c_int, [_p, _p, _p, _i64, _p, _i64, _i32, _f64, _f64,
                                              _u64, _u64, _p, _p, _p, _p]),
    'dw_edges_inline_build': (ctypes.c_int, [_p, _p, _i64, _i64, _p, _p]),
    'dw_sgns_walks': (ctypes.c_int, [_p, _i64, _i32, _i32, _i32, _i64, _i32, _p, _p, _p, _p,
                                     _p, _u64, _u64, _f32, _p, _p, _p, ctypes.c_size_t, _p]),
    'dw_sgns_walks_phase': (ctypes.c_int, [_i32, _p, _i64, _i32, _i32, _i32, _i64, _i32, _p, _p,
                                           _p, _p, _p, _u64, _u64, _f32, _p, _p, _p,
                                           ctypes.c_size_t, _p]),
    'dw_sgns_walks_phase2_piece': (ctypes.c_int, [_i32, _i32, _i64, _p, _i64, _i32, _i32, _i32,
                                                   _i64, _i32, _p, _p, _p, _p, ctypes.c_size_t,
                                                   _p]),
    'dw_sgns_owner_workspace_bytes': (ctypes.c_int, [_i64, _i32, _i32, _i64, _i64, _szp]),
    'dw_sgns_owner_prepare': (ctypes.c_int, [_p, _i64, _i32, _i32, _i32, _i64, _i64, _p, _p,
                                             _p, ctypes.c_size_t, _p]),
    'dw_sgns_owner_pass1': (ctypes.c_int, [_p, _i64, _i32, _i32, _i32, _i64, _i32, _i32, _i32,
                                           _i64, _i32, _p, _p, _p, _p, _u64, _u64, _f32, _p, _p,
                                           _p, ctypes.c_size_t, _p]),
    'dw_sgns_owner_touch_claim': (ctypes.c_int, [_p, _i64, _i32, _i32, _i64, _p, _i32, _p, _p,
                                                 _p, _p, _i32, _p]),
    'dw_adam_rows': (ctypes.c_int, [_p, _p, _p, _p, _p, _i64, _i32, _p, _p, _i64, _p, _i32, _p,
                                    _i32, _p]),
    'dw_rows_gather': (ctypes.c_int, [_p, _i64, _i32, _p, _p, _i64, _p, _i32, _p]),
    'dw_sgns_owner_pass2': (ctypes.c_int, [_i64, _i32, _i32, _i32, _i64, _i32, _p, _p, _p, _p, _p,
                                           _p, _f32, _f32, _f32, _f32, _f32, _f32, _f32, _p, _p,
                                           ctypes.c_size_t, _p, _p]),
    'dw_sgns_owner_out_catch_up': (ctypes.c_int, [_p, _i64, _i32, _i32, _i32, _i64, _i32, _i32,
                                                  _i32, _i64, _p, _u64, _u64, _p, _p, _p, _p, _p,
                                                  _p, _p, _p, _p, _i32, _i32, _p, _p,
                                                  ctypes.c_size_t, _p]),
    'dw_sgns_owner_pass2_lazy': (ctypes.c_int, [_i64, _i32, _i32, _i32, _i64, _i32, _p, _p, _p,
                                                _p, _p, _p, _p, _i32, _i32, _p, _p, _p,
                                                ctypes.c_size_t, _p, _p]),
    'dw_sgns_owner_out_rows': (ctypes.c_int, [_p, _i64, _i32, _i32, _i32, _i64, _i32, _i32, _i32,
                                              _i64, _p, _u64, _u64, _f32, _p, _p, _p, _p, _p, _p,
                                              _p, _p, _p, _i32, _p, _p, _p,
                                              ctypes.c_size_t, _p]),
    'dw_sgns_walks_phase2_adam': (ctypes.c_int, [_p, _i64, _i32, _i32, _i32, _i64, _i32, _p, _p,
                                                 _p, _p, _p, _p, _f32, _f32, _f32, _f32, _f32,
                                                 _f32, _f32, _p, _p, ctypes.c_size_t, _p]),
    'dw_sgns_walks_shared': (ctypes.c_int, [_p, _i64, _i32, _i32, _i32, _i32, _i64, _i32, _p, _p,
                                            _p, _p, _p, _f32, _p, _p, _p]),
    'dw_sgns_pairs': (ctypes.c_int, [_p, _p, _i64, _i32, _i32, _i64, _i32, _p, _p, _p, _p,
                                     _p, _u64, _u64, _f32, _p, _p, _p, ctypes.c_size_t, _p]),
    'dw_sgns_workspace_bytes': (ctypes.c_int, [_i64, _i32, _i32, _i64, _szp]),
    'dw_sgns_pooled_pairs': (ctypes.c_int, [_p, _i32, _p, _i64, _i32, _i32, _i64, _i32, _p, _p,
                                            _p, _p, _p, _u64, _u64, _f32, _p, _p, _p]),
    'dw_sgns_noise': (ctypes.c_int, [_i64, _i32, _i32, _i64, _u64, _u64, _p, _p]),
    'dw_noise_alias_build': (ctypes.c_int, [_p, _i64, _p]),
    'dw_sgns_noise_alias': (ctypes.c_int, [_i64, _i32, _i32, _i64, _p, _u64, _u64, _p, _p]),
    'dw_negative_edges': (ctypes.c_int, [_p, _p, _i64, _i64, _i64, _u64, _u64, _p, _p, _p]),
    'dw_edge_features': (ctypes.c_int, [_p, _i64, _i32, _i32, _p, _i64, _p, _p, _p]),
    'dw_edge_logreg_workspace_bytes': (ctypes.c_int, [_i64, _i32, _szp]),
    'dw_edge_logreg': (ctypes.c_int, [_p, _i64, _i32, _i32, _p, _p, _i64, _p, _p, _p,
                                      ctypes.c_size_t, _p, _p]),
    'dw_embedding_renorm_workspace_bytes': (ctypes.c_int, [_i64, _i64, _szp]),
    'dw_embedding_renorm': (ctypes.c_int, [_p, _i64, _i32, _p, _i64, _f64, _p, ctypes.c_size_t,
                                           _p, _p]),
    'dw_pooled_logits': (ctypes.c_int, [_p, _i32, _p, _i64, _i32, _i64, _i32, _p, _p, _i32, _p,
                                        _p, _p]),
    'dw_pooled_logits_backward': (ctypes.c_int, [_p, _i32, _p, _i64, _i32, _i64, _i32, _p, _p,
                                                 _p, _p, _p, _p, _p]),
    'dw_sgns_timing': (ctypes.c_int, [_i32]),
    'dw_sgns_phase_ms': (ctypes.c_int, [ctypes.POINTER(ctypes.c_double),
                                        ctypes.POINTER(ctypes.c_int64)]),
    'dw_skipgram_logits': (ctypes.c_int, [_p, _p, _i64, _i32, _i64, _i32, _p, _p, _i32, _p, _p,
                                          _p]),
    'dw_skipgram_logits_backward': (ctypes.c_int, [_p, _p, _i64, _i32, _i64, _i32, _p, _p, _p,
                                                   _p, _p, _p, _p]),
    'dw_adam_dense': (ctypes.c_int, [_p, _p, _p, _p, _i64, _f32, _f32, _f32, _f32, _f32, _f32,
                                     _f32, _i32, _p]),
    'dw_adam_dense_to': (ctypes.c_int, [_p, _p, _p, _p, _p, _i64, _f32, _f32, _f32, _f32, _f32,
                                         _f32, _f32, _i32, _i64, _p]),
    'dw_sgd_dense': (ctypes.c_int, [_p, _p, _p, _i64, _f32, _f32, _f32, _f32, _i32, _i32, _i32,
                                    _p]),
    'dw_sgd_rows': (ctypes.c_int, [_p, _p, _i64, _i32, _p, _i32, _i64, _p, _f32, _p, _p]),
    'dw_scale': (ctypes.c_int, [_p, _i64, _f32, _p, _p]),
    'dw_step_scalars_bind': (ctypes.c_int, [_p]),
    'dw_step_scalars_bind_at': (ctypes.c_int, [_p, _i64]),
    'dw_step_scalars_advance': (ctypes.c_int, [_p, _p, _i64, _u64, _u64, _p, _p, _i64, _p,
                                               _i64, _p]),
    'dw_step_starts': (ctypes.c_int, [_p, _p, _i64, _p, _i64, _p]),
    'dw_walk_replay_inline': (ctypes.c_int, [_p, _p, _i64, _p, _i64, _i32, _p, _p, _p, _p]),
    'dw_walk_replay_indexed': (ctypes.c_int, [_p, _p, _p, _p, _p, _p, _p, _p, _i64, _p, _i64,
                                              _p, _i64, _i32, _f64, _f64, _p, _p, _p, _p, _p]),
    'dw_edge_common_counts': (ctypes.c_int, [_p, _p, _p, _p, _p, _p, _p, _i64, _i64, _i64, _p,
                                             _p]),
    'dw_hub_bitmaps': (ctypes.c_int, [_p, _p, _i64, _p, _i64, _i64, _p, _p]),
    'dw_n2v_edge_offsets': (ctypes.c_int, [_p, _p, _p, _i64, _p, _p, _p, _szp, _p]),
    'dw_n2v_edge_index_build': (ctypes.c_int, [_p, _p, _p, _p, _p, _p, _p, _i64, _p, _p, _p,
                                               _i64, _i64, _i64, _i64, _i64, _i64, _p, _p, _p,
                                               _p, _szp, _p, _p]),
    'dw_n2v_edge_records': (ctypes.c_int, [_p, _p, _p, _p, _p, _i64, _p, _p]),
    'dw_exact_register': (ctypes.c_int, [_p, _p, _i64, _i32, _i32]),
    'dw_exact_unregister': (ctypes.c_int, [_p]),
    'dw_exact_frac_bits': (ctypes.c_int32, [_f64]),
    'dw_fixed_to_float': (ctypes.c_int, [_p, _p, _i64, _i32, _i32, _p]),
    'dw_walk_replay_positions': (ctypes.c_int, [_p, _p, _p, _i64, _p, _i64, _i32, _f64, _f64,
                                                _p, _p, _p, _p, _p]),
    'dw_adj_hash_positions': (ctypes.c_int, [_p, _p, _i64, _p, _p, _i64, _p, _p, _p]),
    'dw_step_scalars_expand': (ctypes.c_int, [_p, _p, _i64, _p, _i64, _u64, _u64, _p, _p, _i64,
                                              _p, _i64, _p]),
}


class NativeLibraryError(RuntimeError):
    """libdw_hip.so is missing or failed to load (build it with __graft_entry__.build())."""


class DWError(RuntimeError):
    """A libdw_hip entry point returned a negative DW_E_* code."""


_lock = threading.Lock()
_lib: Optional[ctypes.CDLL] = None


def load() -> ctypes.CDLL:
    global _lib
    if _lib is not None:
        return _lib
    with _lock:
        if _lib is not None:
            return _lib
        if not os.path.exists(LIB_PATH):
            raise NativeLibraryError(
                f'HIP library not found at {LIB_PATH}; build it with '
                f'`python -c "import __graft_entry__ as g; g.build()"` (hipcc, gfx950)')
        try:
            lib = ctypes.CDLL(LIB_PATH)
        except OSError as exc:
            raise NativeLibraryError(f'cannot load {LIB_PATH}: {exc}') from exc
        for name, (res, args) in SIGNATURES.items():
            fn = getattr(lib, name)
            fn.restype = res
            fn.argtypes = args
        if lib.dw_abi_version() != ABI_VERSION:
            raise NativeLibraryError(
                f'ABI mismatch: library {lib.dw_abi_version()} != host {ABI_VERSION}; rebuild')
        _lib = lib
        return lib


def call(name: str, *args) -> None:
    lib = load()
    rc = getattr(lib, name)(*args)
    if rc != DW_OK:
        msg = lib.dw_last_error_string().decode(errors='replace')
        raise DWError(f'{name} failed ({rc}): {msg}')


def ptr(t: Optional[torch.Tensor]) -> Optional[int]:
    if t is None:
        return None
    if t.device.type != 'cuda':
        raise ValueError(f'libdw_hip needs device tensors, got a {t.device} tensor')
    if not t.is_contiguous():
        raise ValueError('libdw_hip needs contiguous tensors')
    return t.data_ptr()


def stream(device: Optional[torch.device] = None) -> int:
    return torch.cuda.current_stream(device).cuda_stream


def require_device(device) -> torch.device:
    if not torch.cuda.is_available():
        raise NativeLibraryError('no HIP device visible: the hot path runs only on MI355X '
                                 '(the CPU restatement lives in oracle/, used by tests only)')
    load()
    dev = torch.device(device) if device is not None else torch.device('cuda',
                                                                       torch.cuda.current_device())
    if dev.type != 'cuda':
        raise ValueError(f'expected a HIP device, got {dev}')
    return dev


def check_status(status: torch.Tensor, what: str) -> None:
    s = int(status.item())
    if s == 0:
        return
    if s & DW_S_ISOLATED_NODE:
        raise IndexError(f'{what}: Cannot choose from an empty sequence (walk reached a node '
                         f'without neighbours)')
    if s & DW_S_ZERO_WEIGHT:
        raise ZeroDivisionError(f'{what}: neighbour weights sum to zero')
    if s & DW_S_REJECTION_CAP:
        raise RuntimeError(f'{what}: node2vec rejection sampling exceeded its round cap')
    if s & DW_S_BAD_CSR:
        raise ValueError(f'{what}: malformed CSR graph')
    if s & DW_S_BAD_INDEX:
        raise IndexError(f'{what}: index out of range [0, vocab_size)')
    if s & DW_S_RECORDS_FULL:
        raise RuntimeError(f'{what}: SGNS records exceeded the workspace')
    if s & DW_S_DUP_NEIGHBOR:
        raise ValueError(f'{what}: a CSR row lists the same neighbour twice (the reference\'s '
                         f'networkx.Graph cannot hold a repeated edge)')
    if s & DW_S_FIXED_RANGE:
# ... 6 lines not shown
```

deepwalk-and-node2vec_amd/shallow_encoders/word2vec/graphed.py:

```python
from typing import Optional

import numpy as np
import torch

from shallow_encoders import _native
from shallow_encoders.word2vec.sharding import (OwnerLazyTables, ShardedTables, adam_scalars,
                                                hist_header, hist_row,
                                                owner_lazy_step, owner_lazy_steps,
                                                replicated_step)

_STEP_DTYPE = np.dtype([('walk_id0', '<u8'), ('noise_offset', '<u8'), ('step', '<i8'),
                        ('adam', '<f4', (8,))])


def adam_history(n_steps: int, lr: float, betas, eps: float, weight_decay: float) -> np.ndarray:
    h = np.zeros((n_steps + 1, 8), dtype=np.float32)
    for s in range(1, n_steps + 1):
        h[s] = hist_row(s, lr, betas, eps, weight_decay)
    h[0] = hist_header(h, n_steps)
    return h


class GraphedStep:

    def __init__(self, tables: ShardedTables, walker, epoch_starts: torch.Tensor, B: int,
                 context_radius: int, neg_samples: int, *, seed: int, grad_scale: float,
                 loss_acc: torch.Tensor, status: torch.Tensor, first_walk_id: int,
                 n_steps: int, noise_offset: Optional[int] = None, scatter: str = 'sorted',
                 unroll: int = 1):
        if tables.world != 1 or not tables.can_fuse_out_adam():
            raise ValueError('GraphedStep: one GPU, HIP Adam')
        if epoch_starts.dtype != torch.int32 or epoch_starts.device != tables.device:
            raise ValueError('GraphedStep: epoch_starts must be int32 on the tables\' device')
        if unroll < 1:
            raise ValueError('GraphedStep: unroll must be >= 1')
        if getattr(walker, '_rng', None) != 'philox':
            raise ValueError("GraphedStep: the walker must be a Philox walker (rng='philox'); "
                             "rng='python' draws its uniforms on the host")
        self.unroll = int(unroll)
        self.t, self.walker = tables, walker
        dev = tables.device
        L = walker.length
        R, K = int(context_radius), int(neg_samples)
        self.B, self.centres = int(B), int(B) * (L - 2 * R)
        self.status, self.loss_acc = status, loss_acc
        self.epoch_starts = epoch_starts
        self.walks = torch.empty((self.unroll * self.B, L), dtype=torch.int32, device=dev)
        self.starts = torch.empty(self.unroll * self.B, dtype=torch.int32, device=dev)
        s1 = tables.step_count + 1
        hist = adam_history(s1 + n_steps + 2, tables.lr, tables.betas, tables.eps,
                            tables.weight_decay)
        self.hist = torch.from_numpy(hist).to(dev)
        blk = np.zeros(1, dtype=_STEP_DTYPE)
        blk['walk_id0'] = first_walk_id
        blk['noise_offset'] = (first_walk_id * (L - 2 * R) if noise_offset is None
                               else noise_offset)
        blk['step'] = s1
        blk['adam'][0] = hist[s1]
        self.block = torch.from_numpy(np.frombuffer(blk.tobytes(), dtype=np.uint8).copy()).to(dev)
        self.step_blocks = torch.zeros(self.unroll * _STEP_DTYPE.itemsize, dtype=torch.uint8,
                                       device=dev)
        self._args = dict(seed=seed, grad_scale=grad_scale, scatter=scatter,
                          fuse_out_adam=scatter == 'sorted')
        self.R, self.K = R, K
        self.graphs = {}
        self._hist_rows = int(hist.shape[0])
        next_wid = walker._next_walk_id
        n_warm = min(self.B, int(epoch_starts.numel()))
        walker.walk_batch(epoch_starts[:n_warm], walk_id0=int(first_walk_id),
                          out=torch.empty((n_warm, L), dtype=torch.int32, device=dev),
                          check=False, status=torch.zeros(1, dtype=torch.int32, device=dev))
        walker._next_walk_id = next_wid
        from shallow_encoders.word2vec.sgns import _use_records, workspace_for
        if scatter == 'sorted' and _use_records(scatter, 2 * R, K, tables.V):
            workspace_for(self.centres, 2 * R, K, tables.V, dev)
        torch.cuda.synchronize(dev)
        self._flips = tables.overlap_in and self.unroll % 2 == 1
        n_graphs = 2 if self._flips else 1
        for _ in range(n_graphs):
            parity = tables._cur_in
            g = torch.cuda.CUDAGraph()
            try:
                with torch.cuda.graph(g, capture_error_mode='relaxed'):
                    self._body()
            finally:
                _native.call('dw_step_scalars_bind', None)
            self.graphs[parity] = g
        tables.step_count -= n_graphs * self.unroll
        walker._next_walk_id = next_wid
        torch.cuda.synchronize(dev)

    def _step_blk(self, k: int) -> int:
        return self.step_blocks.data_ptr() + k * _STEP_DTYPE.itemsize

    def _body(self) -> None:
        t, dev, B = self.t, self.t.device, self.B
        with torch.cuda.device(dev):
            _native.call('dw_step_scalars_expand', _native.ptr(self.block), self._step_blk(0),
                         self.unroll, _native.ptr(self.hist), self.hist.shape[0], B,
                         self.centres, _native.ptr(self.status), _native.ptr(self.epoch_starts),
                         self.epoch_starts.numel(), _native.ptr(self.starts), self.starts.numel(),
                         _native.stream(dev))
        _native.call('dw_step_scalars_bind', self._step_blk(0))
        self.walker.walk_batch(self.starts, walk_id0=0, out=self.walks, check=False,
                               status=self.status)
        for k in range(self.unroll):
            _native.call('dw_step_scalars_bind', self._step_blk(k))
            replicated_step(t, self.walks[k * B:(k + 1) * B], self.R, self.K, noise_offset=0,
                            loss_acc=self.loss_acc, status=self.status, **self._args)

    def replay(self) -> None:
        t = self.t
        if t.step_count + 1 + self.unroll >= self._hist_rows:
            raise RuntimeError(f'GraphedStep: the Adam-scalar history covers steps up to '
                               f'{self._hist_rows - 2}; build a new GraphedStep (n_steps) to go on')
        self.graphs[t._cur_in].replay()
        t.step_count += self.unroll
        if self._flips:
            t._next_in = 2 - t._cur_in
            t._cur_in = t._next_in

    def scalars(self) -> dict:
        b = np.frombuffer(self.block.cpu().numpy().tobytes(), dtype=_STEP_DTYPE)[0]
        return {'walk_id0': int(b['walk_id0']), 'noise_offset': int(b['noise_offset']),
                'step': int(b['step'])}


SIDE_FIRST_FROM = 2000


class GraphedOwnerStep:

    def __init__(self, tables: OwnerLazyTables, walker, epoch_starts: torch.Tensor, B: int,
                 context_radius: int, neg_samples: int, *, seed: int, grad_scale: float,
                 loss_acc: torch.Tensor, status: torch.Tensor, first_walk_id: int,
                 n_steps: int, unroll: int = 1):
        if not isinstance(tables, OwnerLazyTables) or tables.multi or tables.world != 1 \
                or not tables._hip():
            raise ValueError('GraphedOwnerStep: one GPU, OwnerLazyTables with the HIP Adam')
        if tables._touched is None or tables._G is None or tables.step_count < 1:
            raise ValueError('GraphedOwnerStep: run one eager owner_lazy_step at this batch shape '
                             'first (it allocates the buffers the capture reuses)')
        if epoch_starts.dtype != torch.int32 or epoch_starts.device != tables.device:
            raise ValueError('GraphedOwnerStep: epoch_starts must be int32 on the tables\' device')
        if unroll < 1:
            raise ValueError('GraphedOwnerStep: unroll must be >= 1')
        if getattr(walker, '_rng', None) != 'philox':
            raise ValueError("GraphedOwnerStep: the walker must be a Philox walker (rng='philox')")
        self.unroll = int(unroll)
        self.t, self.walker = tables, walker
        dev = tables.device
        L = walker.length
        R, K = int(context_radius), int(neg_samples)
        self.R, self.K = R, K
        self.B, self.centres = int(B), int(B) * (L - 2 * R)
        self.status, self.loss_acc, self.epoch_starts = status, loss_acc, epoch_starts
        self.seed, self.grad_scale = int(seed), float(grad_scale)
        self.walks = torch.empty((self.unroll * self.B, L), dtype=torch.int32, device=dev)
        self.starts = torch.empty(self.unroll * self.B, dtype=torch.int32, device=dev)
        s1 = tables.step_count + 1
        self._last = s1 + int(n_steps) + self.unroll
        tables.reserve_history(self._last)
        self._key = tables._hist_key
        hist = tables._hist
        self._hist_ptr = hist.data_ptr()
        blk = np.zeros(1, dtype=_STEP_DTYPE)
        blk['walk_id0'] = first_walk_id
        blk['noise_offset'] = first_walk_id * (L - 2 * R)
        blk['step'] = s1
        blk['adam'][0] = hist[s1].cpu().numpy()
        self.block = torch.from_numpy(np.frombuffer(blk.tobytes(), dtype=np.uint8).copy()).to(dev)
        self.step_blocks = torch.zeros(self.unroll * _STEP_DTYPE.itemsize, dtype=torch.uint8,
                                       device=dev)
        next_wid = walker._next_walk_id
        n_warm = min(self.B, int(epoch_starts.numel()))
        walker.walk_batch(epoch_starts[:n_warm], walk_id0=int(first_walk_id),
                          out=torch.empty((n_warm, L), dtype=torch.int32, device=dev),
                          check=False, status=torch.zeros(1, dtype=torch.int32, device=dev))
        walker._next_walk_id = next_wid
        torch.cuda.synchronize(dev)
        if tables.pipeline_ok(R, K):
            tables._pipe_alloc(self.B, L, R, K)
        steps0, lr0 = tables.step_count, len(tables._lr_hist)
        self.graph = torch.cuda.CUDAGraph()
        self.graph_late = None
        for late in ((False, True) if tables.pipeline_ok(R, K) else (False,)):
            g = torch.cuda.CUDAGraph() if late else self.graph
            try:
                with torch.cuda.graph(g, capture_error_mode='relaxed'):
                    self._body(side_first=late)
            finally:
                _native.call('dw_step_scalars_bind', None)
                tables.step_count = steps0
                del tables._lr_hist[lr0:]
                walker._next_walk_id = next_wid
            if late:
                self.graph_late = g
        torch.cuda.synchronize(dev)

    def _step_blk(self, k: int) -> int:
        return self.step_blocks.data_ptr() + k * _STEP_DTYPE.itemsize

    def _body(self, side_first: bool = False) -> None:
        t, dev, B = self.t, self.t.device, self.B
        with torch.cuda.device(dev):
            _native.call('dw_step_scalars_expand', _native.ptr(self.block), self._step_blk(0),
                         self.unroll, _native.ptr(t._hist), self._last + 1, B, self.centres,
                         _native.ptr(self.status), _native.ptr(self.epoch_starts),
                         self.epoch_starts.numel(), _native.ptr(self.starts), self.starts.numel(),
                         _native.stream(dev))
        _native.call('dw_step_scalars_bind', self._step_blk(0))
        self.walker.walk_batch(self.starts, walk_id0=0, out=self.walks, check=False,
                               status=self.status)
        steps0 = t.step_count

        def bind(k):
            _native.call('dw_step_scalars_bind_at', self._step_blk(k), steps0 + k + 1)
        owner_lazy_steps(t, [self.walks[k * B:(k + 1) * B] for k in range(self.unroll)], self.R,
                         self.K, seed=self.seed, noise_offsets=[0] * self.unroll,
                         grad_scale=self.grad_scale, loss_acc=self.loss_acc, status=self.status,
                         bind=bind, side_first=side_first)

    def replay(self) -> None:
        t = self.t
        if (t.lr, tuple(t.betas), t.eps, t.weight_decay) != self._key:
            raise RuntimeError('GraphedOwnerStep: the Adam hyper-parameters changed since the '
                               'capture; build a new GraphedOwnerStep')
        if t._hist.data_ptr() != self._hist_ptr:
# ... 191 lines not shown
```

deepwalk-and-node2vec_amd/shallow_encoders/word2vec/sgns.py:

```python
import math
from typing import Callable, Dict, Optional

import torch

RECORDS_MAX_ROWS = 256

from shallow_encoders import _native


def loss_terms(acc: torch.Tensor, n_terms: int, neg_samples: int) -> Dict[str, torch.Tensor]:
    m = float(max(n_terms, 1))
    pos = (acc[0] / m).float()
    neg = (acc[1] / m).float()
    out = {
        'loss': pos + neg,
        'positive-loss': pos,
        'negative-loss': neg,
        'recall': (acc[2] / m).float(),
        'precision': (1.0 - acc[3] / (m * max(neg_samples, 1))).float(),
    }
    return out


_WORKSPACES: Dict[torch.device, torch.Tensor] = {}


def _use_records(scatter: str, n_ctx: int, neg_samples: int, vocab_size: int) -> bool:
    return (scatter == 'sorted' and n_ctx * (1 + neg_samples) <= RECORDS_MAX_ROWS
            and vocab_size < 2 ** 31)


def workspace_for(n_centres: int, n_ctx: int, neg_samples: int, vocab_size: int,
                  device: torch.device, local_rows: Optional[int] = None,
                  slot: int = 0) -> torch.Tensor:
    import ctypes
    nbytes = ctypes.c_size_t(0)
    if local_rows is None:
        _native.call('dw_sgns_workspace_bytes', int(n_centres), int(n_ctx), int(neg_samples),
                     int(vocab_size), ctypes.byref(nbytes))
    else:
        _native.call('dw_sgns_owner_workspace_bytes', int(n_centres), int(n_ctx),
                     int(neg_samples), int(vocab_size), int(local_rows), ctypes.byref(nbytes))
    key = device if slot == 0 else (device, int(slot))
    ws = _WORKSPACES.get(key)
    if ws is None or ws.numel() < nbytes.value:
        _WORKSPACES.pop(key, None)
        ws = torch.empty(int(nbytes.value), dtype=torch.uint8, device=device)
        _WORKSPACES[key] = ws
    return ws


def sgns_accumulate(w_in: torch.Tensor, w_out: torch.Tensor, g_in: torch.Tensor,
                    g_out: torch.Tensor, neg_samples: int, *, walks: Optional[torch.Tensor] = None,
                    context_radius: int = 0, inputs: Optional[torch.Tensor] = None,
                    targets: Optional[torch.Tensor] = None, noise: Optional[torch.Tensor] = None,
                    seed: int = 0, noise_offset: int = 0, grad_scale: Optional[float] = None,
                    loss_acc: Optional[torch.Tensor] = None,
                    status: Optional[torch.Tensor] = None, scatter: str = 'sorted',
                    phase: int = 0, out_adam: Optional[dict] = None) -> torch.Tensor:
    dev = w_in.device
    V, d = w_in.shape
    if w_out.shape != (V, d) or g_in.shape != (V, d) or g_out.shape != (V, d):
        raise ValueError('embedding tables and gradients must all be (V, d)')
    for t in (w_in, w_out, g_in, g_out):
        if t.dtype != torch.float32:
            raise TypeError('embedding tables and gradients must be float32')
    if scatter not in ('sorted', 'atomic'):
        raise ValueError('scatter must be "sorted" or "atomic"')
    if loss_acc is None:
        loss_acc = torch.zeros(4, dtype=torch.float64, device=dev)
    if status is None:
        status = torch.zeros(1, dtype=torch.int32, device=dev)
    K = int(neg_samples)
    with torch.cuda.device(dev):
        s = _native.stream(dev)
        if walks is not None:
            if walks.dtype != torch.int32 or walks.dim() != 2:
                raise TypeError('walks must be int32 [n_walks, L]')
            n, L = walks.shape
            R = int(context_radius)
            n_centres = n * (L - 2 * R)
            C = 2 * R
            if noise is not None and noise.numel() != n_centres * C * K:
                raise ValueError('noise must have B\' * 2R * K entries')
            scale = 1.0 / max(n_centres * C, 1) if grad_scale is None else grad_scale
            ws = workspace_for(n_centres, C, K, V, dev) \
                if _use_records(scatter, C, K, V) else None
            if out_adam is not None:
                if phase != 2 or ws is None:
                    raise ValueError('out_adam fuses the output-table Adam into phase 2 of the '
                                     'records (sorted) path')
                _native.call('dw_sgns_walks_phase2_adam', _native.ptr(walks), n, L, R, K, V, d,
                             _native.ptr(w_in), _native.ptr(w_out), _native.ptr(g_out),
                             _native.ptr(out_adam['m']), _native.ptr(out_adam['v']),
                             _native.ptr(out_adam['flags']), *out_adam['scalars'],
                             _native.ptr(status), _native.ptr(ws), ws.numel(), s)
                return loss_acc
            _native.call('dw_sgns_walks_phase', int(phase), _native.ptr(walks), n, L, R, K, V, d,
                         _native.ptr(w_in), _native.ptr(w_out), _native.ptr(g_in),
                         _native.ptr(g_out), _native.ptr(noise), seed & 0xFFFFFFFFFFFFFFFF,
                         int(noise_offset), float(scale), _native.ptr(loss_acc),
                         _native.ptr(status), _native.ptr(ws), 0 if ws is None else ws.numel(), s)
        else:
            if inputs is None or targets is None:
                raise ValueError('give walks, or inputs and targets')
            if phase != 0:
                raise ValueError('the two-phase form takes walks')
            B, C = targets.shape
            P = 1 if inputs.dim() == 1 else inputs.shape[1]
            if inputs.numel() != B * P:
                raise ValueError('inputs and targets disagree on the batch size')
            if noise is not None and noise.numel() != B * C * K:
                raise ValueError('noise must have B * C * K entries')
            scale = 1.0 / max(B * C, 1) if grad_scale is None else grad_scale
            if P > 1:
                _native.call('dw_sgns_pooled_pairs', _native.ptr(inputs.contiguous()), P,
                             _native.ptr(targets.contiguous()), B, C, K, V, d, _native.ptr(w_in),
                             _native.ptr(w_out), _native.ptr(g_in), _native.ptr(g_out),
                             _native.ptr(noise), seed & 0xFFFFFFFFFFFFFFFF, int(noise_offset),
                             float(scale), _native.ptr(loss_acc), _native.ptr(status), s)
                return loss_acc
            inputs = inputs.reshape(-1)
            ws = workspace_for(B, C, K, V, dev) if _use_records(scatter, C, K, V) else None
            _native.call('dw_sgns_pairs', _native.ptr(inputs.contiguous()),
                         _native.ptr(targets.contiguous()), B, C, K, V, d, _native.ptr(w_in),
                         _native.ptr(w_out), _native.ptr(g_in), _native.ptr(g_out),
                         _native.ptr(noise), seed & 0xFFFFFFFFFFFFFFFF, int(noise_offset),
                         float(scale), _native.ptr(loss_acc), _native.ptr(status),
                         _native.ptr(ws), 0 if ws is None else ws.numel(), s)
    return loss_acc


def sgns_phase2_pieces(w_in: torch.Tensor, g_out: torch.Tensor, neg_samples: int, *,
                       walks: torch.Tensor, context_radius: int, n_pieces: int,
                       piece_rows: int, on_piece: Optional[Callable[[int], None]] = None,
                       status: Optional[torch.Tensor] = None, scatter: str = 'sorted') -> None:
    dev = w_in.device
    V, d = w_in.shape
    if g_out.shape != (V, d):
        raise ValueError('w_in and g_out must both be (V, d)')
    if walks.dtype != torch.int32 or walks.dim() != 2:
        raise TypeError('walks must be int32 [n_walks, L]')
    if n_pieces * piece_rows < V:
        raise ValueError('the pieces must cover every output row')
    n, L = walks.shape
    R, K = int(context_radius), int(neg_samples)
    C = 2 * R
    if not _use_records(scatter, C, K, V):
        for p in range(n_pieces):
            if on_piece is not None:
                on_piece(p)
        return
    if status is None:
        status = torch.zeros(1, dtype=torch.int32, device=dev)
    ws = workspace_for(n * (L - 2 * R), C, K, V, dev)
    with torch.cuda.device(dev):
        for p in range(-1, n_pieces):
            _native.call('dw_sgns_walks_phase2_piece', p, int(n_pieces), int(piece_rows),
                         _native.ptr(walks), n, L, R, K, V, d, _native.ptr(w_in),
                         _native.ptr(g_out), _native.ptr(status), _native.ptr(ws), ws.numel(),
                         _native.stream(dev))
            if p >= 0 and on_piece is not None:
                on_piece(p)


def device_noise(n_centres: int, n_ctx: int, neg_samples: int, vocab_size: int, seed: int,
                 noise_offset: int, device, out: Optional[torch.Tensor] = None) -> torch.Tensor:
    n = int(n_centres) * int(n_ctx) * int(neg_samples)
    if out is None:
        out = torch.empty((n_centres, n_ctx, neg_samples), dtype=torch.int64, device=device)
    elif out.dtype != torch.int64 or out.numel() != n or out.device.type != 'cuda':
        raise ValueError('device_noise: out must be an int64 device tensor of B * C * K elements')
    else:
        device = out.device
        out = out.view(n_centres, n_ctx, neg_samples)
    with torch.cuda.device(device):
        _native.call('dw_sgns_noise', int(n_centres), int(n_ctx), int(neg_samples),
                     int(vocab_size), seed & 0xFFFFFFFFFFFFFFFF, int(noise_offset),
                     _native.ptr(out), _native.stream(device))
    return out


SHARED_DIMS = (64, 128, 256)
SHARED_MAX_L = 128
SHARED_MAX_S = 128


def shared_shape_error(L: int, R: int, S: int, d: int, V: int) -> Optional[str]:
    if R < 1 or L < 2 * R + 1:
        return f'walk_length {L} < 2R+1 (R = {R})'
    if L > SHARED_MAX_L:
        return f'walk_length {L} > {SHARED_MAX_L}'
    if d not in SHARED_DIMS:
        return f'dim must be one of {SHARED_DIMS}, got {d}'
    if S % 32 or not 32 <= S <= SHARED_MAX_S:
        return f'shared_negatives must be a multiple of 32 in [32, {SHARED_MAX_S}], got {S}'
    if V >= 2 ** 31:
        return 'vocab_size must be < 2^31'
    return None


def sgns_shared_accumulate(w_in: torch.Tensor, w_out: torch.Tensor, g_in: torch.Tensor,
                           g_out: torch.Tensor, neg_samples: int, *, walks: torch.Tensor,
                           context_radius: int, shared_ids: torch.Tensor,
                           grad_scale: Optional[float] = None,
                           loss_acc: Optional[torch.Tensor] = None,
                           status: Optional[torch.Tensor] = None) -> torch.Tensor:
    dev = w_in.device
    V, d = w_in.shape
    if w_out.shape != (V, d) or g_in.shape != (V, d) or g_out.shape != (V, d):
        raise ValueError('embedding tables and gradients must all be (V, d)')
    for t in (w_in, w_out, g_in, g_out):
        if t.dtype != torch.float32:
            raise TypeError('embedding tables and gradients must be float32')
    if walks.dtype != torch.int32 or walks.dim() != 2:
        raise TypeError('walks must be int32 [n_walks, L]')
    n, L = walks.shape
    if shared_ids.dtype != torch.int64 or n == 0 or shared_ids.numel() % n:
        raise ValueError('shared_ids must be int64 with n_walks * S entries')
    S = shared_ids.numel() // n
    R, K = int(context_radius), int(neg_samples)
    scale = 1.0 / max(n * (L - 2 * R) * 2 * R, 1) if grad_scale is None else grad_scale
    if loss_acc is None:
        loss_acc = torch.zeros(4, dtype=torch.float64, device=dev)
    if status is None:
        status = torch.zeros(1, dtype=torch.int32, device=dev)
    with torch.cuda.device(dev):
        _native.call('dw_sgns_walks_shared', _native.ptr(walks), n, L, R, K, S, V, d,
                     _native.ptr(w_in), _native.ptr(w_out), _native.ptr(g_in), _native.ptr(g_out),
                     _native.ptr(shared_ids), float(scale), _native.ptr(loss_acc),
                     _native.ptr(status), _native.stream(dev))
    return loss_acc


def sgns_shared_bytes(n_walks: int, L: int, R: int, S: int, d: int) -> Dict[str, float]:
    rows = n_walks * ((L - 2 * R) + (L + S))
    return {'reads': rows * 4 * d + n_walks * (4 * L + 8 * S), 'l2_reads': rows * 4 * d,
            'atomics': rows * 8 * d, 'atomic_rows': rows * 4 * d}


def unigram_table_host(weights: torch.Tensor, power: float = 0.75) -> torch.Tensor:
    w = torch.as_tensor(weights).detach().double().cpu().reshape(-1).pow(float(power)).contiguous()
    table = torch.empty(w.numel(), dtype=torch.uint64)
    _native.call('dw_noise_alias_build', w.data_ptr(), int(w.numel()), table.data_ptr())
    return table


def unigram_table(weights: torch.Tensor, power: float = 0.75, device=None) -> torch.Tensor:
    if device is None and isinstance(weights, torch.Tensor) and weights.device.type == 'cuda':
        device = weights.device
    dev = _native.require_device(device)
    return unigram_table_host(weights, power).to(dev)


def unigram_noise(n_centres: int, n_ctx: int, neg_samples: int, table: torch.Tensor, seed: int,
                  noise_offset: int, device, out: Optional[torch.Tensor] = None) -> torch.Tensor:
    dev = table.device
    want = torch.device(device) if device is not None else dev
    if table.dtype != torch.uint64 or dev.type != 'cuda' or want.type != 'cuda' or \
            (want.index is not None and want.index != dev.index):
        raise ValueError('unigram_noise: table must be a uint64 tensor on the noise device')
    n = int(n_centres) * int(n_ctx) * int(neg_samples)
    if out is None:
        out = torch.empty((n_centres, n_ctx, neg_samples), dtype=torch.int64, device=dev)
    elif out.dtype != torch.int64 or out.numel() != n or out.device != dev:
        raise ValueError('unigram_noise: out must be an int64 device tensor of B * C * K elements')
    with torch.cuda.device(dev):
        _native.call('dw_sgns_noise_alias', int(n_centres), int(n_ctx), int(neg_samples),
                     int(table.numel()), _native.ptr(table), seed & 0xFFFFFFFFFFFFFFFF,
                     int(noise_offset), _native.ptr(out), _native.stream(dev))
    return out.view(n_centres, n_ctx, neg_samples)


_RENORM_WS: Dict[torch.device, torch.Tensor] = {}


def renorm_(weight: torch.Tensor, ids: torch.Tensor, max_norm: float,
            status: Optional[torch.Tensor] = None) -> None:
    import ctypes
    V, d = weight.shape
    ids = ids.reshape(-1).to(weight.device, torch.long).contiguous()
    n = ids.numel()
    if n == 0:
        return
    nbytes = ctypes.c_size_t(0)
    _native.call('dw_embedding_renorm_workspace_bytes', n, V, ctypes.byref(nbytes))
    ws = _RENORM_WS.get(weight.device)
    if ws is None or ws.numel() < nbytes.value:
        ws = torch.empty(int(nbytes.value), dtype=torch.uint8, device=weight.device)
        _RENORM_WS[weight.device] = ws
    st = torch.zeros(1, dtype=torch.int32, device=weight.device) if status is None else status
    with torch.cuda.device(weight.device):
        _native.call('dw_embedding_renorm', _native.ptr(weight.detach()), V, d, _native.ptr(ids),
                     n, float(max_norm), _native.ptr(ws), ws.numel(), _native.ptr(st),
                     _native.stream(weight.device))
    if status is None:
        _native.check_status(st, 'embedding renorm')


def sgns_phase_bytes(n_walks: int, L: int, R: int, K: int, d: int, V: int, scatter: str,
                     fused: bool = False) -> Dict[str, float]:
    centres = n_walks * (L - 2 * R)
    T = 2 * R * (1 + K)
    n_rec = centres * T
    if scatter != 'sorted':
        return {'pass1': centres * (4 * d * (1 + T) + 8 * d + 8 * d * T) + n_walks * L * 4,
                'sort': 0, 'pass2': 0}
    bits = max(1, math.ceil(math.log2(V)))
    touched = V * (1.0 - math.exp(-n_rec / V))
    return {'pass1': centres * (4 * d * (1 + T) + 8 * d + 12 * T) + n_walks * L * 4,
            'sort': n_rec * (4 + 24 * math.ceil(bits / 11)),
            'pass2': n_rec * (12 + 4 * d) + (V * d * 24 if fused else touched * 8 * d)}


def phase_timing(enable: bool) -> None:
    _native.call('dw_sgns_timing', 1 if enable else 0)


def phase_ms() -> Dict[str, float]:
    import ctypes
    ms = (ctypes.c_double * 3)()
    n = ctypes.c_int64(0)
    _native.call('dw_sgns_phase_ms', ms, ctypes.byref(n))
    return {'pass1': ms[0], 'sort': ms[1], 'pass2': ms[2], 'calls': int(n.value)}


class SGNSLoss(torch.autograd.Function):

    @staticmethod
    def forward(ctx, w_in, w_out, src, targets, noise, context_radius, neg_samples, seed,
                noise_offset):
        g_in = torch.zeros_like(w_in)
        g_out = torch.zeros_like(w_out)
        if targets is None:
            acc = sgns_accumulate(w_in.detach(), w_out.detach(), g_in, g_out, neg_samples,
                                  walks=src, context_radius=context_radius, noise=noise,
                                  seed=seed, noise_offset=noise_offset)
            n, L = src.shape
            n_terms = n * (L - 2 * context_radius) * 2 * context_radius
        else:
            acc = sgns_accumulate(w_in.detach(), w_out.detach(), g_in, g_out, neg_samples,
                                  inputs=src, targets=targets, noise=noise, seed=seed,
                                  noise_offset=noise_offset)
            n_terms = targets.numel()
        t = loss_terms(acc, n_terms, neg_samples)
        ctx.save_for_backward(g_in, g_out)
        others = (t['positive-loss'], t['negative-loss'], t['recall'], t['precision'])
        ctx.mark_non_differentiable(*others)
        return (t['loss'],) + others

    @staticmethod
    def backward(ctx, grad_loss, *unused):
        g_in, g_out = ctx.saved_tensors
        if grad_loss is not None:
            go = grad_loss.detach().float().contiguous()
            with torch.cuda.device(g_in.device):
                s = _native.stream(g_in.device)
                _native.call('dw_scale', _native.ptr(g_in), g_in.numel(), 1.0, _native.ptr(go), s)
                _native.call('dw_scale', _native.ptr(g_out), g_out.numel(), 1.0, _native.ptr(go),
                             s)
        return g_in, g_out, None, None, None, None, None, None, None


def sgns_owner_pass1(w_in: torch.Tensor, w_out_local: torch.Tensor, g_in: torch.Tensor,
                     neg_samples: int, *, walks: torch.Tensor, context_radius: int, owner: int,
                     n_owners: int, vocab_size: int, noise: Optional[torch.Tensor] = None,
                     seed: int = 0, noise_offset: int = 0, grad_scale: Optional[float] = None,
                     loss_acc: Optional[torch.Tensor] = None,
                     status: Optional[torch.Tensor] = None,
                     order_ready: bool = False, placed: bool = False,
                     coefficients_in: bool = False,
                     walk_order: bool = False,
                     workspace_slot: int = 0) -> Optional[torch.Tensor]:
    dev = w_in.device
    d = w_in.shape[1]
    local_rows = w_out_local.shape[0]
    if w_out_local.shape[1] != d or g_in.shape[1] != d or g_in.shape[0] < vocab_size \
            or w_in.shape[0] < vocab_size:
        raise ValueError('w_in / g_in must be (>= V, d) and w_out_local (local_rows, d)')
    if local_rows * n_owners < vocab_size:
        raise ValueError('the owners\' local rows do not cover the vocabulary')
    for t in (w_in, w_out_local, g_in):
        if t.dtype != torch.float32:
            raise TypeError('embedding tables and gradients must be float32')
    if walks.dtype != torch.int32 or walks.dim() != 2:
        raise TypeError('walks must be int32 [n_walks, L]')
    n, L = walks.shape
    R, K = int(context_radius), int(neg_samples)
    n_centres = n * (L - 2 * R)
    if noise is not None and noise.numel() != n_centres * 2 * R * K:
        raise ValueError('noise must have B\' * 2R * K entries')
    scale = 1.0 / max(n_centres * 2 * R, 1) if grad_scale is None else grad_scale
    if coefficients_in:
        if not placed:
            raise ValueError('coefficients_in needs the placed records (placed=True)')
        loss_acc = None
    elif walk_order:
        raise ValueError('walk_order is the coefficients_in form\'s')
    elif loss_acc is None:
        loss_acc = torch.zeros(4, dtype=torch.float64, device=dev)
    if status is None:
        status = torch.zeros(1, dtype=torch.int32, device=dev)
    ws = workspace_for(n_centres, 2 * R, K, vocab_size, dev, local_rows=local_rows,
                       slot=workspace_slot)
    with torch.cuda.device(dev):
        _native.call('dw_sgns_owner_pass1', _native.ptr(walks), n, L, R, K, int(vocab_size), d,
                     int(owner), int(n_owners), local_rows,
                     (1 if order_ready else 0) | (2 if placed else 0)
                     | (4 if coefficients_in else 0) | (8 if walk_order else 0),
                     _native.ptr(w_in), _native.ptr(w_out_local), _native.ptr(g_in),
                     _native.ptr(noise),
                     seed & 0xFFFFFFFFFFFFFFFF, int(noise_offset), float(scale),
                     _native.ptr(loss_acc), _native.ptr(status), _native.ptr(ws), ws.numel(),
                     _native.stream(dev))
    return loss_acc


def sgns_owner_prepare(walks: torch.Tensor, context_radius: int, neg_samples: int,
                       vocab_size: int, local_rows: int, *,
                       touched: Optional[torch.Tensor] = None,
                       n_touched: Optional[torch.Tensor] = None) -> None:
    dev = walks.device
    if walks.dtype != torch.int32 or walks.dim() != 2:
        raise TypeError('walks must be int32 [n_walks, L]')
    n, L = walks.shape
    R, K = int(context_radius), int(neg_samples)
    n_centres = n * (L - 2 * R)
    if touched is not None and (touched.numel() < n_centres or touched.dtype != torch.int32
                                or n_touched is None or n_touched.dtype != torch.int64):
        raise ValueError('touched must be int32 [>= n_centres] with an int64 n_touched')
    ws = workspace_for(n_centres, 2 * R, K, vocab_size, dev, local_rows=local_rows)
    with torch.cuda.device(dev):
        _native.call('dw_sgns_owner_prepare', _native.ptr(walks), n, L, R, K, int(vocab_size),
                     int(local_rows), _native.ptr(touched), _native.ptr(n_touched),
                     _native.ptr(ws), ws.numel(), _native.stream(dev))


def sgns_owner_pass2(w_in: torch.Tensor, w_out_local: torch.Tensor, g_out_local: torch.Tensor,
                     neg_samples: int, *, walks: torch.Tensor, context_radius: int,
                     out_adam: Optional[dict] = None,
                     status: Optional[torch.Tensor] = None,
                     read_count: bool = True) -> Optional[int]:
    import ctypes
    dev = w_in.device
    d = w_in.shape[1]
    local_rows = w_out_local.shape[0]
    if g_out_local.shape != w_out_local.shape or w_out_local.shape[1] != d:
        raise ValueError('w_out_local and g_out_local must both be (local_rows, d)')
    n, L = walks.shape
    R, K = int(context_radius), int(neg_samples)
    if status is None:
        status = torch.zeros(1, dtype=torch.int32, device=dev)
    ws = workspace_for(n * (L - 2 * R), 2 * R, K, w_in.shape[0], dev, local_rows=local_rows)
    n_rec = ctypes.c_int64(0)
    n_rec_p = ctypes.byref(n_rec) if read_count else None
    if out_adam is not None and 'last' in out_adam:
        with torch.cuda.device(dev):
            _native.call('dw_sgns_owner_pass2_lazy', n, L, R, K, local_rows, d, _native.ptr(w_in),
                         _native.ptr(w_out_local), _native.ptr(g_out_local),
                         _native.ptr(out_adam['m']), _native.ptr(out_adam['v']),
                         _native.ptr(out_adam['last']), _native.ptr(out_adam['hist']),
                         int(out_adam['step']), int(out_adam.get('flags', 0)),
# ... 18 lines not shown
```

include/dw_hip.h:

```cpp
#ifndef DW_HIP_H
#define DW_HIP_H

#include <stddef.h>
#include <stdint.h>

#ifdef __cplusplus
extern "C" {
#endif

#define DW_OK                0
#define DW_E_INVALID_ARG    -1
#define DW_E_HIP            -2
#define DW_E_UNSUPPORTED    -3

#define DW_S_ISOLATED_NODE   1
#define DW_S_ZERO_WEIGHT     2
#define DW_S_REJECTION_CAP   4
#define DW_S_BAD_CSR         8
#define DW_S_BAD_INDEX      16
#define DW_S_RECORDS_FULL   32
#define DW_S_DUP_NEIGHBOR   64
#define DW_S_FIXED_RANGE   128
#define DW_S_BAD_TEXT      256

// ... 152 lines not shown
                         int32_t *out, int32_t *status, void *stream);

int dw_walk_fast_counted(const int64_t *row_ptr, const int32_t *col, const int64_t *adj_off,
                         const int32_t *adj_hash, const uint32_t *prob_thr, const int32_t *alias,
                         int64_t n_rows, const int32_t *starts, int64_t n_walks,
                         int32_t walk_length, double p, double q, uint64_t seed,
                         uint64_t walk_id0, int32_t *out, int32_t *status,
                         uint64_t *counters, void *stream);

int dw_walk_fast_positions(const int64_t *row_ptr, const int32_t *n2v_rec, const uint8_t *n2v_pos,
                           int64_t n_rows, const int32_t *starts, int64_t n_walks,
                           int32_t walk_length, double p, double q, uint64_t seed,
                           uint64_t walk_id0, int32_t *out, int32_t *status, uint64_t *counters,
                           void *stream);

int dw_edges_inline_build(const int64_t *row_ptr, const int32_t *col, int64_t n_rows, int64_t nnz,
                          int32_t *edges, void *stream);


int dw_sgns_walks(const int32_t *walks, int64_t n_walks, int32_t walk_length,
                  int32_t context_radius, int32_t neg_samples, int64_t vocab_size, int32_t dim,
                  const float *w_in, const float *w_out, float *g_in, float *g_out,
                  const int64_t *noise, uint64_t seed, uint64_t noise_offset, float grad_scale,
                  double *loss_acc, int32_t *status, void *workspace, size_t workspace_bytes,
                  void *stream);

int dw_sgns_walks_phase(int32_t phase, const int32_t *walks, int64_t n_walks,
                        int32_t walk_length, int32_t context_radius, int32_t neg_samples,
                        int64_t vocab_size, int32_t dim, const float *w_in, const float *w_out,
                        float *g_in, float *g_out, const int64_t *noise, uint64_t seed,
                        uint64_t noise_offset, float grad_scale, double *loss_acc,
                        int32_t *status, void *workspace, size_t workspace_bytes,
                        void *stream);

int dw_sgns_walks_phase2_piece(int32_t piece, int32_t n_pieces, int64_t piece_rows,
                               const int32_t *walks, int64_t n_walks, int32_t walk_length,
                               int32_t context_radius, int32_t neg_samples, int64_t vocab_size,
                               int32_t dim, const float *w_in, float *g_out, int32_t *status,
                               void *workspace, size_t workspace_bytes, void *stream);

int dw_sgns_walks_phase2_adam(const int32_t *walks, int64_t n_walks, int32_t walk_length,
                              int32_t context_radius, int32_t neg_samples, int64_t vocab_size,
                              int32_t dim, const float *w_in, float *w_out, float *g_out,
                              float *m_out, float *v_out, uint8_t *row_flags,
                              float one_minus_beta1, float beta2, float one_minus_beta2,
                              float bias_correction2_sqrt, float neg_step_size, float eps,
                              float weight_decay, int32_t *status, void *workspace,
                              size_t workspace_bytes, void *stream);

int dw_sgns_owner_workspace_bytes(int64_t n_centres, int32_t n_ctx, int32_t neg_samples,
                                  int64_t vocab_size, int64_t local_rows, size_t *bytes);
int dw_sgns_owner_prepare(const int32_t *walks, int64_t n_walks, int32_t walk_length,
                          int32_t context_radius, int32_t neg_samples, int64_t vocab_size,
                          int64_t local_rows, uint32_t *touched, int64_t *n_touched,
                          void *workspace, size_t workspace_bytes, void *stream);
int dw_sgns_owner_pass1(const int32_t *walks, int64_t n_walks, int32_t walk_length,
                        int32_t context_radius, int32_t neg_samples, int64_t vocab_size,
                        int32_t dim, int32_t owner, int32_t n_owners, int64_t local_rows,
                        int32_t order_ready, const float *w_in, const float *w_out_local,
                        float *g_in,
                        const int64_t *noise, uint64_t seed, uint64_t noise_offset,
                        float grad_scale, double *loss_acc, int32_t *status, void *workspace,
                        size_t workspace_bytes, void *stream);
int dw_sgns_owner_pass2(int64_t n_walks, int32_t walk_length, int32_t context_radius,
                        int32_t neg_samples, int64_t local_rows, int32_t dim, const float *w_in,
                        float *w_out_local, float *g_out_local, float *m_out, float *v_out,
                        uint8_t *row_flags, float one_minus_beta1, float beta2,
                        float one_minus_beta2, float bias_correction2_sqrt, float neg_step_size,
                        float eps, float weight_decay, int32_t *status, void *workspace,
                        size_t workspace_bytes, int64_t *n_records, void *stream);

int dw_sgns_owner_out_catch_up(const int32_t *walks, int64_t n_walks, int32_t walk_length,
                               int32_t context_radius, int32_t neg_samples, int64_t vocab_size,
                               int32_t dim, int32_t owner, int32_t n_owners, int64_t local_rows,
                               const int64_t *noise, uint64_t seed, uint64_t noise_offset,
                               float *w_out_local, float *m_out, float *v_out,
                               int32_t *last_step, int32_t *claim, uint32_t *counts,
                               uint32_t *rows_buf, int64_t *n_rows, const float *hist,
                               int32_t step, int32_t flags, int32_t *status, void *workspace,
                               size_t workspace_bytes, void *stream);

int dw_sgns_owner_pass2_lazy(int64_t n_walks, int32_t walk_length, int32_t context_radius,
                             int32_t neg_samples, int64_t local_rows, int32_t dim,
                             const float *w_in, float *w_out_local, float *g_out_local,
                             float *m_out, float *v_out, int32_t *last_step, const float *hist,
                             int32_t step, int32_t flags, uint32_t *counts, int32_t *status,
                             void *workspace, size_t workspace_bytes, int64_t *n_records,
                             void *stream);

int dw_sgns_owner_touch_claim(const int32_t *walks, int64_t n_walks, int32_t walk_length,
                              int32_t context_radius, int64_t vocab_size, int32_t *claim,
                              int32_t step, uint32_t *touched, int64_t *n_touched,
                              uint32_t *fresh, int64_t *n_fresh, int32_t flags, void *stream);

int dw_sgns_owner_out_rows(const int32_t *walks, int64_t n_walks, int32_t walk_length,
                           int32_t context_radius, int32_t neg_samples, int64_t vocab_size,
                           int32_t dim, int32_t owner, int32_t n_owners, int64_t local_rows,
                           const int64_t *noise, uint64_t seed, uint64_t noise_offset,
                           float grad_scale, const float *w_in, float *w_out_local,
                           float *g_out_local, float *m_out, float *v_out, int32_t *last_step,
                           uint32_t *counts, uint8_t *pending, const float *hist,
                           int32_t step, double *loss_acc, int32_t *status,
                           void *workspace, size_t workspace_bytes, void *stream);

int dw_sgns_pairs(const int64_t *inputs, const int64_t *targets, int64_t batch, int32_t n_ctx,
                  int32_t neg_samples, int64_t vocab_size, int32_t dim,
                  const float *w_in, const float *w_out, float *g_in, float *g_out,
                  const int64_t *noise, uint64_t seed, uint64_t noise_offset, float grad_scale,
                  double *loss_acc, int32_t *status, void *workspace, size_t workspace_bytes,
                  void *stream);

int dw_sgns_pooled_pairs(const int64_t *inputs, int32_t n_in, const int64_t *targets,
                         int64_t batch, int32_t n_ctx, int32_t neg_samples, int64_t vocab_size,
                         int32_t dim, const float *w_in, const float *w_out, float *g_in,
                         float *g_out, const int64_t *noise, uint64_t seed,
                         uint64_t noise_offset, float grad_scale, double *loss_acc,
                         int32_t *status, void *stream);

int dw_sgns_walks_shared(const int32_t *walks, int64_t n_walks, int32_t walk_length,
                         int32_t context_radius, int32_t neg_samples, int32_t n_shared,
                         int64_t vocab_size, int32_t dim, const float *w_in, const float *w_out,
                         float *g_in, float *g_out, const int64_t *shared_ids, float grad_scale,
                         double *loss_acc, int32_t *status, void *stream);

int dw_sgns_noise(int64_t batch, int32_t n_ctx, int32_t neg_samples, int64_t vocab_size,
                  uint64_t seed, uint64_t noise_offset, int64_t *noise, void *stream);

int dw_noise_alias_build(const double *weights, int64_t V, uint64_t *table);
int dw_sgns_noise_alias(int64_t batch, int32_t n_ctx, int32_t neg_samples, int64_t vocab_size,
                        const uint64_t *table, uint64_t seed, uint64_t noise_offset,
                        int64_t *noise, void *stream);

int dw_negative_edges(const int64_t *row_ptr, const int32_t *col_sorted, int64_t n_rows,
                      int64_t first_node, int64_t n, uint64_t seed, uint64_t offset,
                      int64_t *pairs, int32_t *status, void *stream);

int dw_edge_features(const float *table, int64_t vocab_size, int32_t dim, int32_t op,
                     const int64_t *pairs, int64_t n, float *out, int32_t *status, void *stream);

int dw_edge_logreg_workspace_bytes(int64_t n, int32_t dim, size_t *bytes);
int dw_edge_logreg(const float *table, int64_t vocab_size, int32_t dim, int32_t op,
                   const int64_t *pairs, const uint8_t *labels, int64_t n, const double *coef,
                   double *out, void *workspace, size_t workspace_bytes, int32_t *status,
                   void *stream);

int dw_embedding_renorm_workspace_bytes(int64_t n_ids, int64_t vocab_size, size_t *bytes);
int dw_embedding_renorm(float *weight, int64_t vocab_size, int32_t dim, const int64_t *ids,
                        int64_t n_ids, double max_norm, void *workspace, size_t workspace_bytes,
                        int32_t *status, void *stream);

int dw_sgns_workspace_bytes(int64_t n_centres, int32_t n_ctx, int32_t neg_samples,
                            int64_t vocab_size, size_t *bytes);

int dw_sgns_timing(int32_t enable);
int dw_sgns_phase_ms(double *ms, int64_t *n_calls);

int dw_pooled_logits(const int64_t *inputs, int32_t n_in, const int64_t *outputs,
                     int64_t batch, int32_t n_out, int64_t vocab_size, int32_t dim,
                     const float *w_in, const float *w_out, int32_t proba, float *logits,
                     int32_t *status, void *stream);
int dw_pooled_logits_backward(const int64_t *inputs, int32_t n_in, const int64_t *outputs,
                              int64_t batch, int32_t n_out, int64_t vocab_size, int32_t dim,
                              const float *w_in, const float *w_out, const float *dlogits,
                              float *g_in, float *g_out, int32_t *status, void *stream);

int dw_skipgram_logits(const int64_t *inputs, const int64_t *outputs, int64_t batch,
                       int32_t n_out, int64_t vocab_size, int32_t dim, const float *w_in,
                       const float *w_out, int32_t proba, float *logits, int32_t *status,
                       void *stream);

int dw_skipgram_logits_backward(const int64_t *inputs, const int64_t *outputs, int64_t batch,
                                int32_t n_out, int64_t vocab_size, int32_t dim,
                                const float *w_in, const float *w_out, const float *dlogits,
                                float *g_in, float *g_out, int32_t *status, void *stream);

int dw_adam_dense(float *param, float *grad, float *exp_avg, float *exp_avg_sq, int64_t n_elem,
                  float one_minus_beta1, float beta2, float one_minus_beta2,
                  float bias_correction2_sqrt, float neg_step_size, float eps,
                  float weight_decay, int32_t zero_grad, void *stream);

int dw_adam_dense_to(const float *param_src, float *param_dst, float *grad, float *exp_avg,
                     float *exp_avg_sq, int64_t n_elem, float one_minus_beta1, float beta2,
                     float one_minus_beta2, float bias_correction2_sqrt, float neg_step_size,
                     float eps, float weight_decay, int32_t zero_grad, int64_t max_blocks,
                     void *stream);

int dw_sgd_dense(float *param, float *grad, float *momentum_buf, int64_t n_elem, float neg_lr,
                 float weight_decay, float momentum, float one_minus_dampening, int32_t nesterov,
                 int32_t first_step, int32_t zero_grad, void *stream);

int dw_sgd_rows(float *param, float *grad, int64_t n_table_rows, int32_t dim, const void *ids,
                int32_t id_bytes, int64_t n_ids, uint32_t *claim, float neg_lr, int32_t *status,
                void *stream);

int dw_adam_rows(float *param, float *exp_avg, float *exp_avg_sq, int32_t *last_step,
                 uint8_t *pending, int64_t n_table_rows, int32_t dim, const uint32_t *rows,
                 const int64_t *n_rows_dev, int64_t n_rows_max, float *grad_rows,
                 int32_t grad_by_row, const float *hist, int32_t step, void *stream);

int dw_rows_gather(float *table, int64_t n_table_rows, int32_t dim, const uint32_t *rows,
                   const int64_t *n_rows_dev, int64_t n_rows_max, float *out,
                   int32_t zero_source, void *stream);

int dw_scale(float *x, int64_t n_elem, float alpha, const float *alpha_dev, void *stream);

typedef struct dw_step_scalars {
    uint64_t walk_id0;
    uint64_t noise_offset;
    int64_t step;
    float adam[8];
} dw_step_scalars;

int dw_step_scalars_bind(const dw_step_scalars *dev);

int dw_step_scalars_bind_at(const dw_step_scalars *dev, int64_t host_step);

int dw_step_scalars_advance(dw_step_scalars *dev, const float *hist, int64_t hist_rows,
                            uint64_t walks_per_step, uint64_t centres_per_step, int32_t *status,
                            const int32_t *epoch_starts, int64_t n_epoch, int32_t *starts_out,
                            int64_t n, void *stream);

int dw_step_scalars_expand(dw_step_scalars *base, dw_step_scalars *steps, int64_t n_steps,
                           const float *hist, int64_t hist_rows, uint64_t walks_per_step,
                           uint64_t centres_per_step, int32_t *status,
                           const int32_t *epoch_starts, int64_t n_epoch, int32_t *starts_out,
                           int64_t n, void *stream);

int dw_step_starts(const dw_step_scalars *dev, const int32_t *epoch_starts, int64_t n_epoch,
                   int32_t *starts_out, int64_t n, void *stream);

#ifdef __cplusplus
}
#endif

#endif
```

Measured before the change: 849.6 million.

## Aggregate positive-pair gradients per walk position before the sorted scatter

In the from-walks records path, positive-pair coefficients are no longer emitted as one record per (centre, context) pair. A new per-walk kernel sums the coefficient-weighted input rows for every walk position into an aggregate buffer and emits a single record per position, flagged so the gather pass reads from that buffer. Negative samples still produce per-pair records. This cuts the number of records to sort and gather by roughly the 2R-fold positive pairs. The cost is an extra kernel, a walk-sized aggregate buffer of dimension d, and a larger workspace. It is enabled by default when 2R(L-2R) >= 2L, and disabled for exact-accumulation mode or via an env var.

Result: faster. 888.1 million (median of 6 runs) (+4.5%).

```diff
diff --git a/deepwalk-and-node2vec_amd/csrc/dw_abi.cpp b/deepwalk-and-node2vec_amd/csrc/dw_abi.cpp
--- a/deepwalk-and-node2vec_amd/csrc/dw_abi.cpp
+++ b/deepwalk-and-node2vec_amd/csrc/dw_abi.cpp
@@ -44,7 +44,7 @@
 
 const char *dw_last_error_string(void) { return dw::g_err; }
 
-int dw_abi_version(void) { return 29; }
+int dw_abi_version(void) { return 30; }
 
 #ifndef DW_BUILD_ID
 #define DW_BUILD_ID "unknown"
diff --git a/deepwalk-and-node2vec_amd/csrc/dw_sgns.hip b/deepwalk-and-node2vec_amd/csrc/dw_sgns.hip
--- a/deepwalk-and-node2vec_amd/csrc/dw_sgns.hip
+++ b/deepwalk-and-node2vec_amd/csrc/dw_sgns.hip
@@ -1,5 +1,6 @@
 #include <stdlib.h>
 
+#include <atomic>
 #include <cmath>
 #include <mutex>
 #include <unordered_map>
@@ -97,7 +98,11 @@
     int64_t occ_per_wave;
     const dw_step_scalars *dyn;
     dw::Fixed fx_in{};
+    float *coef_pos = nullptr;
+    float *agg = nullptr;
 };
+
+constexpr uint32_t AGG_BIT = 1u << 31;
 
 #ifndef DW_NOISE_ROUNDS
 #define DW_NOISE_ROUNDS 10
@@ -306,10 +311,12 @@
     return x;
 }
 
-template <int F4, bool FROM_WALKS, int CHR, bool OWNER, bool EXACT = false, bool COEFIN = false>
+template <int F4, bool FROM_WALKS, int CHR, bool OWNER, bool EXACT = false, bool COEFIN = false,
+          bool AGG = false>
 __global__ void __launch_bounds__(WAVES_PER_BLOCK *WAVE, CHR >= 8 ? 3 : G16_MIN_WAVES)
     k_sgns_g16(SgnsArgs a) {
     static_assert(!COEFIN || OWNER, "the coefficients-in form is the owner path's");
+    static_assert(!AGG || (FROM_WALKS && !OWNER && !EXACT), "aggregation: the float walks form");
     constexpr int D = 64 * F4;
     __shared__ int32_t s_id[WAVES_PER_BLOCK][4][G16_TMAX];
     __shared__ float s_coef[WAVES_PER_BLOCK][4][G16_TMAX];
@@ -579,6 +586,17 @@
                 const int tt = gl + 16 * k;
                 if (tt < T) {
                     const int32_t id = s_id[wv][q][tt];
+                    if constexpr (AGG) {
+                        const int j = tt / rows_per_ctx, k = tt - j * rows_per_ctx - 1;
+                        if (k < 0) {
+                            a.coef_pos[b * a.C + j] = s_coef[wv][q][tt];
+                        } else {
+                            const int64_t at = (b * a.C + j) * a.K + k;
+                            a.rec_key[at] = static_cast<uint32_t>(id < 0 ? 0 : id);
+                            a.rec_val[at] = pack_record(s_coef[wv][q][tt], ok_c ? cid : 0);
+                        }
+                        continue;
+                    }
                     a.rec_key[b * T + tt] = static_cast<uint32_t>(id < 0 ? 0 : id);
                     a.rec_val[b * T + tt] = pack_record(s_coef[wv][q][tt], ok_c ? cid : 0);
                 }
@@ -654,6 +672,74 @@
             *a.count_out = static_cast<uint32_t>(a.batch * T);
     }
     if (a.loss_acc) flush_loss(a.loss_acc, acc_pos, acc_neg, acc_rec, acc_prec);
+}
+
+template <int SL>
+__global__ void __launch_bounds__(256) k_walk_agg(SgnsArgs a, int64_t n_neg) {
+    extern __shared__ float4 s_agg[];
+    constexpr int LPR = SL / 4;
+    constexpr int RPP = 256 / LPR;
+    const int per = a.L - 2 * a.R;
+    float4 *s_row = s_agg;
+    float *s_cf = reinterpret_cast<float *>(s_row + per * LPR);
+    int32_t *s_pos = reinterpret_cast<int32_t *>(s_cf + per * a.C);
+    const int64_t w = blockIdx.x;
+    const int col = blockIdx.y * SL + 4 * (threadIdx.x % LPR);
+    const int r = threadIdx.x / LPR, c = threadIdx.x % LPR;
+    const int32_t *walk = a.walks + w * a.L;
+    for (int j = threadIdx.x; j < a.L; j += 256) s_pos[j] = walk[j];
+    constexpr int UC = 4, UR = 8;
+    const float *cf_in = a.coef_pos + w * per * a.C;
+    for (int k0 = threadIdx.x; k0 < per * a.C; k0 += UC * 256) {
+        float x[UC];
+#pragma unroll
+        for (int u = 0; u < UC; ++u) x[u] = k0 + u * 256 < per * a.C ? cf_in[k0 + u * 256] : 0.f;
+#pragma unroll
+        for (int u = 0; u < UC; ++u)
+            if (k0 + u * 256 < per * a.C) s_cf[k0 + u * 256] = x[u];
+    }
+    __syncthreads();
+    for (int c0 = r; c0 < per; c0 += UR * RPP) {
+        float4 x[UR];
+#pragma unroll
+        for (int u = 0; u < UR; ++u) {
+            const int ci = c0 + u * RPP;
+            const int64_t id = ci < per ? s_pos[a.R + ci] : -1;
+            x[u] = (id >= 0 && id < a.V)
+                       ? *reinterpret_cast<const float4 *>(a.w_in + id * a.d + col)
+                       : make_float4(0.f, 0.f, 0.f, 0.f);
+        }
+#pragma unroll
+        for (int u = 0; u < UR; ++u)
+            if (c0 + u * RPP < per) s_row[(c0 + u * RPP) * LPR + c] = x[u];
+    }
+    __syncthreads();
+    for (int j = r; j < a.L; j += RPP) {
+        const int lo = j - 2 * a.R > 0 ? j - 2 * a.R : 0;
+        const int hi = j < per - 1 ? j : per - 1;
+        float4 g = make_float4(0.f, 0.f, 0.f, 0.f);
+        for (int ci = lo; ci <= hi; ++ci) {
+            const int i = ci + a.R;
+            if (i == j) continue;
+            const float cf = s_cf[ci * a.C + (j < i ? j - i + a.R : j - i - 1 + a.R)];
+            const float4 x = s_row[ci * LPR + c];
+            g.x = fmaf(cf, x.x, g.x);
+            g.y = fmaf(cf, x.y, g.y);
+            g.z = fmaf(cf, x.z, g.z);
+            g.w = fmaf(cf, x.w, g.w);
+        }
+        *reinterpret_cast<float4 *>(a.agg + (w * a.L + j) * a.d + col) = g;
+    }
+    if (blockIdx.y == 0) {
+        for (int j = threadIdx.x; j < a.L; j += 256) {
+            const int32_t id = s_pos[j];
+            const bool ok = id >= 0 && id < a.V;
+            if (!ok) dw::status_or(a.status, DW_S_BAD_INDEX);
+            const int64_t at = n_neg + w * a.L + j;
+            a.rec_key[at] = static_cast<uint32_t>(ok ? id : 0);
+            a.rec_val[at] = pack_record(ok ? 1.f : 0.f, AGG_BIT | static_cast<uint32_t>(w * a.L + j));
+        }
+    }
 }
 
 struct OutAdam {
@@ -741,7 +827,7 @@
     k_rec_gather(const uint32_t *__restrict__ keys, const uint64_t *__restrict__ vals,
                  int64_t n_rec, const float *__restrict__ w_in, float *__restrict__ g_out,
                  int32_t d, OutAdam oa, const int64_t *__restrict__ range, int32_t gch,
-                 dw::Fixed fo, int32_t *status) {
+                 dw::Fixed fo, int32_t *status, const float *__restrict__ agg) {
     bool fx_range = false;
     uint32_t fx_tmax = 0u;
     const int lane = threadIdx.x & (WAVE - 1);
@@ -825,7 +911,9 @@
                 const uint64_t v = in ? vals[e + u] : 0ull;
                 k[u] = in ? keys[e + u] : last;
                 coef[u] = in ? __uint_as_float(static_cast<uint32_t>(v >> 32)) : 0.f;
-                const float *src = w_in + static_cast<int64_t>(static_cast<uint32_t>(v)) * d + lane;
+                const uint32_t ci = static_cast<uint32_t>(v);
+                const float *src = ((ci & AGG_BIT) ? agg : w_in) +
+                                   static_cast<int64_t>(ci & ~AGG_BIT) * d + lane;
 #pragma unroll
                 for (int m = 0; m < VPL; ++m) x[u][m] = (in && live[m]) ? src[WAVE * m] : 0.f;
             }
@@ -1155,6 +1243,19 @@
         }
         DW_LAUNCH_CHECK("dw_sgns/g16");
         return DW_OK;
+    }
+    if constexpr (FROM_WALKS && !OWNER) {
+        if (a.coef_pos) {
+            switch (a.d / 64) {
+                case 1: hipLaunchKernelGGL((k_sgns_g16<1, true, 8, false, false, false, true>), g, bl, 0, st, a); break;
+                case 2: hipLaunchKernelGGL((k_sgns_g16<2, true, 4, false, false, false, true>), g, bl, 0, st, a); break;
+                case 4: hipLaunchKernelGGL((k_sgns_g16<4, true, 2, false, false, false, true>), g, bl, 0, st, a); break;
+                case 8: hipLaunchKernelGGL((k_sgns_g16<8, true, 1, false, false, false, true>), g, bl, 0, st, a); break;
+                default: return DW_E_UNSUPPORTED;
+            }
+            DW_LAUNCH_CHECK("dw_sgns/g16_agg");
+            return DW_OK;
+        }
     }
     switch (a.d / 64) {
         case 1: hipLaunchKernelGGL((k_sgns_g16<1, FROM_WALKS, 8, OWNER>), g, bl, 0, st, a); break;
@@ -1488,22 +1589,23 @@
 void launch_gather_fx(dim3 g, dim3 bl, hipStream_t st, const uint32_t *keys,
                       const uint64_t *vals, int64_t n_rec, const float *w_in, float *g_out,
                       int32_t d, const OutAdam *oa, const int64_t *range, int32_t gch,
-                      const dw::Fixed &fo, int32_t *status) {
+                      const dw::Fixed &fo, int32_t *status, const float *agg) {
     const bool full = d == 64 * VPL;
     if (oa) {
         if (full)
             hipLaunchKernelGGL((k_rec_gather<VPL, false, true, EXACT>), g, bl, 0, st, keys, vals,
-                               n_rec, w_in, g_out, d, *oa, range, gch, fo, status);
+                               n_rec, w_in, g_out, d, *oa, range, gch, fo, status, agg);
         else
             hipLaunchKernelGGL((k_rec_gather<VPL, true, true, EXACT>), g, bl, 0, st, keys, vals,
-                               n_rec, w_in, g_out, d, *oa, range, gch, fo, status);
+                               n_rec, w_in, g_out, d, *oa, range, gch, fo, status, agg);
     } else {
         if (full)
             hipLaunchKernelGGL((k_rec_gather<VPL, false, false, EXACT>), g, bl, 0, st, keys,
-                               vals, n_rec, w_in, g_out, d, OutAdam{}, range, gch, fo, status);
+                               vals, n_rec, w_in, g_out, d, OutAdam{}, range, gch, fo, status,
+                               agg);
         else
             hipLaunchKernelGGL((k_rec_gather<VPL, true, false, EXACT>), g, bl, 0, st, keys, vals,
-                               n_rec, w_in, g_out, d, OutAdam{}, range, gch, fo, status);
+                               n_rec, w_in, g_out, d, OutAdam{}, range, gch, fo, status, agg);
     }
 }
 
@@ -1511,13 +1613,13 @@
 void launch_gather(dim3 g, dim3 bl, hipStream_t st, const uint32_t *keys, const uint64_t *vals,
                    int64_t n_rec, const float *w_in, float *g_out, int32_t d,
                    const OutAdam *oa, const int64_t *range, int32_t gch, const dw::Fixed &fo,
-                   int32_t *status) {
+                   int32_t *status, const float *agg) {
     if (fo.acc)
         launch_gather_fx<VPL, true>(g, bl, st, keys, vals, n_rec, w_in, g_out, d, oa, range, gch,
-                                    fo, status);
+                                    fo, status, agg);
     else
         launch_gather_fx<VPL, false>(g, bl, st, keys, vals, n_rec, w_in, g_out, d, oa, range,
-                                     gch, fo, status);
+                                     gch, fo, status, agg);
 }
 
 template <int VPL>
@@ -1535,7 +1637,8 @@
 
 int launch_pass2(const uint32_t *keys, const uint64_t *vals, int64_t n_rec, const float *w_in,
                  float *g_out, int32_t d, const OutAdam *oa, int64_t V, hipStream_t st,
-                 const int64_t *range = nullptr, double share = 1.0, int32_t *status = nullptr) {
+                 const int64_t *range = nullptr, double share = 1.0, int32_t *status = nullptr,
+                 const float *agg = nullptr) {
     dw::Fixed fo;
     {
         const int rc = exact_of(g_out, V * d, &fo, nullptr, "dw_sgns pass 2");
@@ -1551,10 +1654,10 @@
     if (blocks < 1) blocks = 1;
     if (blocks > 65536) blocks = 65536;
     const dim3 g((unsigned)blocks), bl(WAVES_PER_BLOCK * WAVE);
-    if (d <= 64) launch_gather<1>(g, bl, st, keys, vals, n_rec, w_in, g_out, d, oa, range, gch, fo, status);
-    else if (d <= 128) launch_gather<2>(g, bl, st, keys, vals, n_rec, w_in, g_out, d, oa, range, gch, fo, status);
-    else if (d <= 256) launch_gather<4>(g, bl, st, keys, vals, n_rec, w_in, g_out, d, oa, range, gch, fo, status);
-    else if (d <= 512) launch_gather<8>(g, bl, st, keys, vals, n_rec, w_in, g_out, d, oa, range, gch, fo, status);
+    if (d <= 64) launch_gather<1>(g, bl, st, keys, vals, n_rec, w_in, g_out, d, oa, range, gch, fo, status, agg);
+    else if (d <= 128) launch_gather<2>(g, bl, st, keys, vals, n_rec, w_in, g_out, d, oa, range, gch, fo, status, agg);
+    else if (d <= 256) launch_gather<4>(g, bl, st, keys, vals, n_rec, w_in, g_out, d, oa, range, gch, fo, status, agg);
+    else if (d <= 512) launch_gather<8>(g, bl, st, keys, vals, n_rec, w_in, g_out, d, oa, range, gch, fo, status, agg);
     else return DW_E_UNSUPPORTED;
     DW_LAUNCH_CHECK("dw_sgns/gather");
     if (fo.acc && n_rec > 0) {
@@ -1602,6 +1705,91 @@
 };
 PhaseTimer g_timer;
 
+int walk_agg_env() {
+    const char *e = getenv("DW_SGNS_WALK_AGG");
+    if (e && e[0] == '0' && e[1] == '\0') return 0;
+    if (e && e[0] == '1' && e[1] == '\0') return 1;
+    return -1;
+}
+std::atomic<int> g_walk_agg_mode{walk_agg_env()};
+
+constexpr size_t AGG_LDS_MAX = 64 * 1024;
+
+inline int walk_agg_slice(int32_t d) { return d == 64 ? 64 : 128; }
+
+size_t walk_agg_lds(int32_t L, int32_t R, int32_t d) {
+    const size_t per = static_cast<size_t>(L - 2 * R);
+    return per * walk_agg_slice(d) * 4 + per * 2 * R * 4 + static_cast<size_t>(L) * 4;
+}
+
+bool walk_agg_shape_ok(int64_t n_walks, int32_t L, int32_t R, int32_t K, int32_t d) {
+    if (!(d == 64 || d == 128 || d == 256 || d == 512)) return false;
+    if (2 * (int64_t)R * (1 + (int64_t)K) > G16_TMAX) return false;
+    if (n_walks < 1 || n_walks * L >= 0x7FFFFFFF) return false;
+    return walk_agg_lds(L, R, d) <= AGG_LDS_MAX;
+}
+
+bool walk_agg_active(int64_t n_walks, int32_t L, int32_t R, int32_t K, int32_t d, bool exact) {
+    const int mode = g_walk_agg_mode.load();
+    if (mode == 0 || exact || !walk_agg_shape_ok(n_walks, L, R, K, d)) return false;
+    return mode == 1 || 2 * (int64_t)R * (L - 2 * R) >= 2 * (int64_t)L;
+}
+
+bool exact_registered(const float *g) {
+    if (!g) return false;
+    std::lock_guard<std::mutex> lk(g_exact_mu);
+    return g_exact.find(g) != g_exact.end();
+}
+
+struct WalkPlan {
+    bool agg;
+    int64_t n_neg, n_rec;
+    Workspace ws;
+    float *coef_pos, *agg_rows;
+    size_t total;
+};
+
+int plan_walks(int64_t n_walks, int32_t L, int32_t R, int32_t K, int64_t V, int32_t d, bool agg,
+               void *base, WalkPlan *p, hipStream_t st) {
+    const int64_t batch = n_walks * (L - 2 * R), C = 2 * R;
+    p->agg = agg;
+    p->n_neg = agg ? batch * C * K : 0;
+    p->n_rec = agg ? p->n_neg + n_walks * L : batch * C * (1 + (int64_t)K);
+    DW_REQUIRE(p->n_rec < 0x7FFFFFFF, "dw_sgns: records mode needs fewer than 2^31 records");
+    const int rc = plan_workspace(p->n_rec > 0 ? p->n_rec : 1, V, base, &p->ws, st);
+    if (rc != DW_OK) return rc;
+    p->total = p->ws.total;
+    p->coef_pos = p->agg_rows = nullptr;
+    if (agg) {
+        char *b = static_cast<char *>(base);
+        p->coef_pos = reinterpret_cast<float *>(b + p->total);
+        p->total += align256(static_cast<size_t>(batch * C) * 4);
+        p->agg_rows = reinterpret_cast<float *>(b + p->total);
+        p->total += align256(static_cast<size_t>(n_walks * L) * d * 4);
+    }
+    return DW_OK;
+}
+
+int plan_walks_for(const SgnsArgs &a, void *base, WalkPlan *p, hipStream_t st) {
+    const int64_t n_walks = a.batch / (a.L - 2 * a.R);
+    const bool exact = exact_registered(a.g_out) || exact_registered(a.g_in);
+    return plan_walks(n_walks, a.L, a.R, a.K, a.V, a.d,
+                      walk_agg_active(n_walks, a.L, a.R, a.K, a.d, exact), base, p, st);
+}
+
+int launch_walk_agg(const SgnsArgs &a, const WalkPlan &p, hipStream_t st) {
+    const int64_t n_walks = a.batch / (a.L - 2 * a.R);
+    const int sl = walk_agg_slice(a.d);
+    const dim3 g((unsigned)n_walks, (unsigned)(a.d / sl)), bl(256);
+    const size_t lds = walk_agg_lds(a.L, a.R, a.d);
+    if (sl == 64)
+        hipLaunchKernelGGL(k_walk_agg<64>, g, bl, lds, st, a, p.n_neg);
+    else
+        hipLaunchKernelGGL(k_walk_agg<128>, g, bl, lds, st, a, p.n_neg);
+    DW_LAUNCH_CHECK("dw_sgns/walk_agg");
+    return DW_OK;
+}
+
 template <bool FROM_WALKS>
 int launch_sgns_impl(SgnsArgs a, void *workspace, size_t workspace_bytes, int phase,
                      hipStream_t st, const OutAdam *oa);
@@ -1647,22 +1835,40 @@
     DW_REQUIRE(T <= TMAX, "dw_sgns: records mode needs 2R(1+K) <= %d (got %lld)", TMAX,
                (long long)T);
     DW_REQUIRE(a.V <= 0x7FFFFFFF, "dw_sgns: records mode needs vocab_size < 2^31");
-    const int64_t n_rec = a.batch * T;
-    DW_REQUIRE(n_rec < 0x7FFFFFFF, "dw_sgns: records mode needs batch*2R(1+K) < 2^31");
-    Workspace ws;
-    int rc = plan_workspace(n_rec, a.V, workspace, &ws, st);
+    DW_REQUIRE(a.batch * T < 0x7FFFFFFF, "dw_sgns: records mode needs batch*2R(1+K) < 2^31");
+    WalkPlan plan;
+    int rc;
+    if constexpr (FROM_WALKS) {
+        rc = plan_walks_for(a, workspace, &plan, st);
+    } else {
+        plan.agg = false;
+        plan.n_neg = 0;
+        plan.n_rec = a.batch * T;
+        plan.coef_pos = plan.agg_rows = nullptr;
+        rc = plan_workspace(plan.n_rec, a.V, workspace, &plan.ws, st);
+        plan.total = plan.ws.total;
+    }
     if (rc != DW_OK) return rc;
-    DW_REQUIRE(workspace_bytes >= ws.total, "dw_sgns: workspace too small (%zu < %zu)",
-               workspace_bytes, ws.total);
+    const Workspace &ws = plan.ws;
+    const int64_t n_rec = plan.n_rec;
+    DW_REQUIRE(workspace_bytes >= plan.total, "dw_sgns: workspace too small (%zu < %zu)%s",
+               workspace_bytes, plan.total,
+               plan.agg ? " (walk aggregation: size it with dw_sgns_walks_workspace_bytes)" : "");
     if (do1) {
         a.rec_key = ws.k0;
         a.rec_val = ws.v0;
+        a.coef_pos = plan.coef_pos;
+        a.agg = plan.agg_rows;
         int32_t fl = 0;
         rc = exact_of(a.g_in, a.V * a.d, &a.fx_in, &fl, "dw_sgns pass 1");
         if (rc != DW_OK) return rc;
         rc = launch_pass1_g16<FROM_WALKS>(a, st);
-        if (rc == DW_E_UNSUPPORTED) rc = launch_pass1<FROM_WALKS, true>(a, st);
+        if (rc == DW_E_UNSUPPORTED && !plan.agg) rc = launch_pass1<FROM_WALKS, true>(a, st);
         if (rc != DW_OK) return rc;
+        if (plan.agg) {
+            rc = launch_walk_agg(a, plan, st);
+            if (rc != DW_OK) return rc;
+        }
         if (a.fx_in.acc && !(fl & (DW_EXACT_DEFER | DW_EXACT_ADAM))) {
             int64_t cb = (a.batch + WAVES_PER_BLOCK - 1) / WAVES_PER_BLOCK;
             if (cb > grid_cap(8)) cb = grid_cap(8);
@@ -1684,7 +1890,7 @@
     }
     g_timer.mark(2, st);
     return launch_pass2(kb.current(), vb.current(), n_rec, a.w_in, a.g_out, a.d, oa, a.V, st,
-                        nullptr, 1.0, a.status);
+                        nullptr, 1.0, a.status, plan.agg_rows);
 }
 
 __global__ void k_piece_bounds(const uint32_t *__restrict__ keys, int64_t n_rec, int32_t n_pieces,
@@ -1719,13 +1925,14 @@
                n_pieces, (long long)piece_rows, (long long)a.V);
     const int64_t T = (int64_t)a.C * (1 + a.K);
     DW_REQUIRE(T <= TMAX && a.V <= 0x7FFFFFFF, "dw_sgns_walks_phase2_piece: records mode limits");
-    const int64_t n_rec = a.batch * T;
-    DW_REQUIRE(n_rec < 0x7FFFFFFF, "dw_sgns_walks_phase2_piece: too many records");
-    Workspace ws;
-    int rc = plan_workspace(n_rec > 0 ? n_rec : 1, a.V, workspace, &ws, st);
+    DW_REQUIRE(a.batch * T < 0x7FFFFFFF, "dw_sgns_walks_phase2_piece: too many records");
+    WalkPlan plan;
+    int rc = plan_walks_for(a, workspace, &plan, st);
     if (rc != DW_OK) return rc;
-    DW_REQUIRE(workspace_bytes >= ws.total, "dw_sgns: workspace too small (%zu < %zu)",
-               workspace_bytes, ws.total);
+    const Workspace &ws = plan.ws;
+    const int64_t n_rec = a.batch > 0 ? plan.n_rec : 0;
+    DW_REQUIRE(workspace_bytes >= plan.total, "dw_sgns: workspace too small (%zu < %zu)",
+               workspace_bytes, plan.total);
     if (piece == -1) {
         bool in_k1 = false;
         if (n_rec > 0) {
@@ -1760,7 +1967,8 @@
     }
     if (n_rec > 0) {
         rc = launch_pass2(in_k1 ? ws.k1 : ws.k0, in_k1 ? ws.v1 : ws.v0, n_rec, a.w_in, a.g_out,
-                          a.d, nullptr, a.V, st, ws.bounds + piece, 2.0 / n_pieces);
+                          a.d, nullptr, a.V, st, ws.bounds + piece, 2.0 / n_pieces, nullptr,
+                          plan.agg_rows);
         if (rc != DW_OK) return rc;
     }
     if (piece == n_pieces - 1) g_timer.mark(3, st);
@@ -2702,6 +2910,46 @@
     if (rc != DW_OK) return rc;
     *bytes = ws.total;
     return DW_OK;
+}
+
+int dw_sgns_walks_workspace_bytes(int64_t n_walks, int32_t walk_length, int32_t context_radius,
+                                  int32_t neg_samples, int64_t vocab_size, int32_t dim,
+                                  size_t *bytes) {
+    DW_REQUIRE(bytes, "dw_sgns_walks_workspace_bytes: bytes is null");
+    DW_REQUIRE(n_walks >= 0 && context_radius >= 1 && walk_length >= 2 * context_radius + 1 &&
+                   neg_samples >= 0 && vocab_size >= 1 && dim >= 1,
+               "dw_sgns_walks_workspace_bytes: bad sizes");
+    const int64_t n_rec = n_walks * (walk_length - 2 * context_radius) * 2 * context_radius *
+                          (1 + (int64_t)neg_samples);
+    DW_REQUIRE(n_rec < 0x7FFFFFFF, "dw_sgns_walks_workspace_bytes: too many records");
+    WalkPlan p;
+    char dummy;
+    int rc = plan_walks(n_walks, walk_length, context_radius, neg_samples, vocab_size, dim, false,
+                        &dummy, &p, nullptr);
+    if (rc != DW_OK) return rc;
+    size_t need = p.total;
+    if (walk_agg_shape_ok(n_walks, walk_length, context_radius, neg_samples, dim)) {
+        rc = plan_walks(n_walks, walk_length, context_radius, neg_samples, vocab_size, dim, true,
+                        &dummy, &p, nullptr);
+        if (rc != DW_OK) return rc;
+        need = p.total > need ? p.total : need;
+    }
+    *bytes = need;
+    return DW_OK;
+}
+
+int dw_sgns_set_walk_agg(int32_t mode) {
+    DW_REQUIRE(mode >= -1 && mode <= 1, "dw_sgns_set_walk_agg: mode must be -1, 0 or 1");
+    g_walk_agg_mode.store(mode);
+    return DW_OK;
+}
+
+int dw_sgns_walk_agg_active(int64_t n_walks, int32_t walk_length, int32_t context_radius,
+                            int32_t neg_samples, int32_t dim) {
+    DW_REQUIRE(n_walks >= 0 && context_radius >= 1 && walk_length >= 2 * context_radius + 1 &&
+                   neg_samples >= 0 && dim >= 1,
+               "dw_sgns_walk_agg_active: bad sizes");
+    return walk_agg_active(n_walks, walk_length, context_radius, neg_samples, dim, false) ? 1 : 0;
 }
 
 namespace {
diff --git a/deepwalk-and-node2vec_amd/shallow_encoders/_native.py b/deepwalk-and-node2vec_amd/shallow_encoders/_native.py
--- a/deepwalk-and-node2vec_amd/shallow_encoders/_native.py
+++ b/deepwalk-and-node2vec_amd/shallow_encoders/_native.py
@@ -28,7 +28,7 @@
 DW_METHOD_DEEPWALK = 0
 DW_METHOD_NODE2VEC = 1
 
-ABI_VERSION = 29
+ABI_VERSION = 30
 
 _p = ctypes.c_void_p
 _i32 = ctypes.c_int32
@@ -121,6 +121,9 @@
     'dw_sgns_pairs': (ctypes.c_int, [_p, _p, _i64, _i32, _i32, _i64, _i32, _p, _p, _p, _p,
                                      _p, _u64, _u64, _f32, _p, _p, _p, ctypes.c_size_t, _p]),
     'dw_sgns_workspace_bytes': (ctypes.c_int, [_i64, _i32, _i32, _i64, _szp]),
+    'dw_sgns_walks_workspace_bytes': (ctypes.c_int, [_i64, _i32, _i32, _i32, _i64, _i32, _szp]),
+    'dw_sgns_set_walk_agg': (ctypes.c_int, [_i32]),
+    'dw_sgns_walk_agg_active': (ctypes.c_int, [_i64, _i32, _i32, _i32, _i32]),
     'dw_sgns_pooled_pairs': (ctypes.c_int, [_p, _i32, _p, _i64, _i32, _i32, _i64, _i32, _p, _p,
                                             _p, _p, _p, _u64, _u64, _f32, _p, _p, _p]),
     'dw_sgns_noise': (ctypes.c_int, [_i64, _i32, _i32, _i64, _u64, _u64, _p, _p]),
diff --git a/deepwalk-and-node2vec_amd/shallow_encoders/word2vec/graphed.py b/deepwalk-and-node2vec_amd/shallow_encoders/word2vec/graphed.py
--- a/deepwalk-and-node2vec_amd/shallow_encoders/word2vec/graphed.py
+++ b/deepwalk-and-node2vec_amd/shallow_encoders/word2vec/graphed.py
@@ -73,7 +73,8 @@
         walker._next_walk_id = next_wid
         from shallow_encoders.word2vec.sgns import _use_records, workspace_for
         if scatter == 'sorted' and _use_records(scatter, 2 * R, K, tables.V):
-            workspace_for(self.centres, 2 * R, K, tables.V, dev)
+            workspace_for(self.centres, 2 * R, K, tables.V, dev, n_walks=self.B, walk_length=L,
+                          dim=int(tables.w_in.shape[1]))
         torch.cuda.synchronize(dev)
         self._flips = tables.overlap_in and self.unroll % 2 == 1
         n_graphs = 2 if self._flips else 1
diff --git a/deepwalk-and-node2vec_amd/shallow_encoders/word2vec/sgns.py b/deepwalk-and-node2vec_amd/shallow_encoders/word2vec/sgns.py
--- a/deepwalk-and-node2vec_amd/shallow_encoders/word2vec/sgns.py
+++ b/deepwalk-and-node2vec_amd/shallow_encoders/word2vec/sgns.py
@@ -32,10 +32,17 @@
 
 def workspace_for(n_centres: int, n_ctx: int, neg_samples: int, vocab_size: int,
                   device: torch.device, local_rows: Optional[int] = None,
-                  slot: int = 0) -> torch.Tensor:
+                  slot: int = 0, *, n_walks: Optional[int] = None,
+                  walk_length: Optional[int] = None, dim: Optional[int] = None) -> torch.Tensor:
     import ctypes
     nbytes = ctypes.c_size_t(0)
-    if local_rows is None:
+    if local_rows is None and n_walks is not None:
+        if walk_length is None or dim is None:
+            raise ValueError('workspace_for: n_walks needs walk_length and dim')
+        _native.call('dw_sgns_walks_workspace_bytes', int(n_walks), int(walk_length),
+                     int(n_ctx) // 2, int(neg_samples), int(vocab_size), int(dim),
+                     ctypes.byref(nbytes))
+    elif local_rows is None:
         _native.call('dw_sgns_workspace_bytes', int(n_centres), int(n_ctx), int(neg_samples),
                      int(vocab_size), ctypes.byref(nbytes))
     else:
@@ -84,7 +91,7 @@
             if noise is not None and noise.numel() != n_centres * C * K:
                 raise ValueError('noise must have B\' * 2R * K entries')
             scale = 1.0 / max(n_centres * C, 1) if grad_scale is None else grad_scale
-            ws = workspace_for(n_centres, C, K, V, dev) \
+            ws = workspace_for(n_centres, C, K, V, dev, n_walks=n, walk_length=L, dim=d) \
                 if _use_records(scatter, C, K, V) else None
             if out_adam is not None:
                 if phase != 2 or ws is None:
@@ -153,7 +160,7 @@
         return
     if status is None:
         status = torch.zeros(1, dtype=torch.int32, device=dev)
-    ws = workspace_for(n * (L - 2 * R), C, K, V, dev)
+    ws = workspace_for(n * (L - 2 * R), C, K, V, dev, n_walks=n, walk_length=L, dim=d)
     with torch.cuda.device(dev):
         for p in range(-1, n_pieces):
             _native.call('dw_sgns_walks_phase2_piece', p, int(n_pieces), int(piece_rows),
@@ -298,6 +305,19 @@
         _native.check_status(st, 'embedding renorm')
 
 
+def set_walk_agg(mode: int) -> None:
+    _native.call('dw_sgns_set_walk_agg', int(mode))
+
+
+def walk_agg_active(n_walks: int, L: int, R: int, K: int, d: int) -> bool:
+    if n_walks < 0 or R < 1 or L < 2 * R + 1 or K < 0 or d < 1:
+        return False
+    rc = _native.load().dw_sgns_walk_agg_active(int(n_walks), int(L), int(R), int(K), int(d))
+    if rc < 0:
+        raise _native.DWError('dw_sgns_walk_agg_active failed')
+    return rc == 1
+
+
 def sgns_phase_bytes(n_walks: int, L: int, R: int, K: int, d: int, V: int, scatter: str,
                      fused: bool = False) -> Dict[str, float]:
     centres = n_walks * (L - 2 * R)
@@ -308,6 +328,15 @@
                 'sort': 0, 'pass2': 0}
     bits = max(1, math.ceil(math.log2(V)))
     touched = V * (1.0 - math.exp(-n_rec / V))
+    if walk_agg_active(n_walks, L, R, K, d):
+        C = 2 * R
+        n_agg = n_walks * L
+        n_rec = centres * C * K + n_agg
+        return {'pass1': centres * (4 * d * (1 + T) + 8 * d + 12 * C * K + 4 * C)
+                + n_walks * L * 4
+                + centres * (4 * d + 4 * C) + n_agg * (4 * d + 12) + n_walks * L * 4,
+                'sort': n_rec * (4 + 24 * math.ceil(bits / 11)),
+                'pass2': n_rec * (12 + 4 * d) + (V * d * 24 if fused else touched * 8 * d)}
     return {'pass1': centres * (4 * d * (1 + T) + 8 * d + 12 * T) + n_walks * L * 4,
             'sort': n_rec * (4 + 24 * math.ceil(bits / 11)),
             'pass2': n_rec * (12 + 4 * d) + (V * d * 24 if fused else touched * 8 * d)}
diff --git a/include/dw_hip.h b/include/dw_hip.h
--- a/include/dw_hip.h
+++ b/include/dw_hip.h
@@ -328,6 +328,13 @@
 int dw_sgns_workspace_bytes(int64_t n_centres, int32_t n_ctx, int32_t neg_samples,
                             int64_t vocab_size, size_t *bytes);
 
+int dw_sgns_walks_workspace_bytes(int64_t n_walks, int32_t walk_length, int32_t context_radius,
+                                  int32_t neg_samples, int64_t vocab_size, int32_t dim,
+                                  size_t *bytes);
+int dw_sgns_set_walk_agg(int32_t mode);
+int dw_sgns_walk_agg_active(int64_t n_walks, int32_t walk_length, int32_t context_radius,
+                            int32_t neg_samples, int32_t dim);
+
 int dw_sgns_timing(int32_t enable);
 int dw_sgns_phase_ms(double *ms, int64_t *n_calls);
 
```
